# iden3/circom-witnesscalc

Measured on AMD Instinct MI355X. Metric: witnesses/sec, higher is better.
Workload: dtype u32

## Files before the change

### circom-witnesscalc_amd/csrc/fr_gfx950.hpp

```cpp
#pragma once
#include <stdint.h>

#if defined(__HIPCC__)
#define FRD __host__ __device__ __forceinline__
#else
#define FRD inline
#endif

namespace cwc {

struct Fr {
    uint32_t v[8];
};

#define CWC_P0 0xf0000001u
#define CWC_P1 0x43e1f593u
#define CWC_P2 0x79b97091u
#define CWC_P3 0x2833e848u
#define CWC_P4 0x8181585du
#define CWC_P5 0xb85045b6u
#define CWC_P6 0xe131a029u
#define CWC_P7 0x30644e72u
#define CWC_INV32 0xefffffffu

FRD Fr fr_p() { return Fr{{CWC_P0, CWC_P1, CWC_P2, CWC_P3, CWC_P4, CWC_P5, CWC_P6, CWC_P7}}; }
FRD Fr fr_one() { return Fr{{0x4ffffffbu, 0xac96341cu, 0x9f60cd29u, 0x36fc7695u, 0x7879462eu, 0x666ea36fu, 0x9a07df2fu, 0x0e0a77c1u}}; }
FRD Fr fr_r2() { return Fr{{0xae216da7u, 0x1bb8e645u, 0xe35c59e3u, 0x53fe3ab1u, 0x53bb8085u, 0x8c49833du, 0x7f4e44a5u, 0x0216d0b1u}}; }
FRD Fr fr_half() { return Fr{{0xf8000000u, 0xa1f0fac9u, 0x3cdcb848u, 0x9419f424u, 0x40c0ac2eu, 0xdc2822dbu, 0x7098d014u, 0x18322739u}}; }
FRD Fr fr_zero() { return Fr{{0, 0, 0, 0, 0, 0, 0, 0}}; }

FRD bool both(bool a, bool b) { return ((uint32_t)a & (uint32_t)b) != 0u; }
FRD bool either(bool a, bool b) { return ((uint32_t)a | (uint32_t)b) != 0u; }

FRD bool u256_is_zero(const Fr& a) {
    uint32_t o = 0;
#pragma unroll
    for (int i = 0; i < 8; ++i) o |= a.v[i];
    return o == 0;
}
FRD bool u256_eq(const Fr& a, const Fr& b) {
    uint32_t o = 0;
#pragma unroll
    for (int i = 0; i < 8; ++i) o |= a.v[i] ^ b.v[i];
    return o == 0;
}
FRD uint32_t adc32(uint32_t a, uint32_t b, uint32_t& carry) {
#if defined(__clang__)
    unsigned c = carry;
    const uint32_t r = __builtin_addc(a, b, c, &c);
    carry = c;
    return r;
#else
    const uint64_t t = (uint64_t)a + b + carry;
    carry = (uint32_t)(t >> 32);
    return (uint32_t)t;
#endif
}
FRD uint32_t sbb32(uint32_t a, uint32_t b, uint32_t& borrow) {
#if defined(__clang__)
    unsigned c = borrow;
    const uint32_t r = __builtin_subc(a, b, c, &c);
    borrow = c;
    return r;
#else
    const uint64_t t = (uint64_t)a - b - borrow;
    borrow = (uint32_t)(t >> 63);
    return (uint32_t)t;
#endif
}
FRD uint32_t u256_add(Fr& r, const Fr& a, const Fr& b) {
#if defined(__clang__)
    unsigned c = 0;
#pragma unroll
    for (int i = 0; i < 8; ++i) r.v[i] = __builtin_addc(a.v[i], b.v[i], c, &c);
    return c;
#else
    uint64_t c = 0;
#pragma unroll
    for (int i = 0; i < 8; ++i) {
        c += (uint64_t)a.v[i] + b.v[i];
        r.v[i] = (uint32_t)c;
        c >>= 32;
    }
    return (uint32_t)c;
#endif
}
FRD uint32_t u256_sub(Fr& r, const Fr& a, const Fr& b) {
#if defined(__clang__)
    unsigned br = 0;
#pragma unroll
    for (int i = 0; i < 8; ++i) r.v[i] = __builtin_subc(a.v[i], b.v[i], br, &br);
    return br;
#else
    int64_t c = 0;
#pragma unroll
    for (int i = 0; i < 8; ++i) {
        c += (int64_t)a.v[i] - (int64_t)b.v[i];
        r.v[i] = (uint32_t)c;
        c >>= 32;
    }
    return (uint32_t)(c & 1);
#endif
}
FRD bool u256_lt(const Fr& a, const Fr& b) {
    Fr t;
    return u256_sub(t, a, b) != 0;
}
FRD Fr u256_select(bool c, const Fr& a, const Fr& b) {
    Fr r;
#pragma unroll
    for (int i = 0; i < 8; ++i) r.v[i] = c ? a.v[i] : b.v[i];
    return r;
}

FRD Fr fr_add(const Fr& a, const Fr& b) {
    Fr s, t;
    u256_add(s, a, b);
    uint32_t br = u256_sub(t, s, fr_p());
    return u256_select(br != 0, s, t);
}
FRD Fr fr_sub(const Fr& a, const Fr& b) {
    Fr d, t;
    uint32_t br = u256_sub(d, a, b);
    u256_add(t, d, fr_p());
    return u256_select(br != 0, t, d);
}
#if defined(__HIPCC__)
__device__ __forceinline__ Fr fr_add_wave(const Fr& a, const Fr& b, const Fr& pv) {
#if defined(__HIP_DEVICE_COMPILE__)
#include "fr_add_gfx950.inc"
#else
    (void)pv;
    return fr_add(a, b);
#endif
}
__device__ __forceinline__ Fr fr_sub_wave(const Fr& a, const Fr& b, const Fr& pv) {
#if defined(__HIP_DEVICE_COMPILE__)
#include "fr_sub_gfx950.inc"
#else
    (void)pv;
    return fr_sub(a, b);
#endif
}
#endif
FRD Fr fr_neg(const Fr& a) {
    Fr t;
    u256_sub(t, fr_p(), a);
    return u256_select(u256_is_zero(a), a, t);
}

FRD Fr fr_mul(const Fr& a, const Fr& b) {
#if defined(__HIP_DEVICE_COMPILE__) && !defined(CWC_PORTABLE_FR_MUL)
#include "fr_mul_gfx950.inc"
#else
    const uint32_t p[8] = {CWC_P0, CWC_P1, CWC_P2, CWC_P3, CWC_P4, CWC_P5, CWC_P6, CWC_P7};
    uint32_t t[9];
#pragma unroll
    for (int i = 0; i < 9; ++i) t[i] = 0;
#pragma unroll
    for (int i = 0; i < 8; ++i) {
        uint64_t c = 0;
#pragma unroll
        for (int j = 0; j < 8; ++j) {
            c += (uint64_t)a.v[i] * b.v[j] + t[j];
            t[j] = (uint32_t)c;
            c >>= 32;
        }
        t[8] = (uint32_t)c;
        uint32_t m = t[0] * CWC_INV32;
        c = (uint64_t)m * p[0] + t[0];
        c >>= 32;
#pragma unroll
        for (int j = 1; j < 8; ++j) {
            c += (uint64_t)m * p[j] + t[j];
            t[j - 1] = (uint32_t)c;
            c >>= 32;
        }
        c += t[8];
        t[7] = (uint32_t)c;
    }
    Fr r, s;
#pragma unroll
    for (int i = 0; i < 8; ++i) r.v[i] = t[i];
    uint32_t br = u256_sub(s, r, fr_p());
    return u256_select(br != 0, r, s);
#endif
}
#if defined(__HIPCC__)
__device__ __forceinline__ Fr fr_addsub_wave(const Fr& a, const Fr& b, const Fr& pv, uint32_t m, unsigned long long subm,
                                             unsigned long long addm) {
#if defined(__HIP_DEVICE_COMPILE__)
#include "fr_addsub_gfx950.inc"
#else
    (void)pv; (void)subm; (void)addm;
    return m ? fr_sub(a, b) : fr_add(a, b);
#endif
}
__device__ __forceinline__ Fr fr_mul_wave(const Fr& a, const Fr& b, const Fr& pv) {
#if defined(__HIP_DEVICE_COMPILE__)
#include "fr_mul_block_gfx950.inc"
#else
    (void)pv;
    return fr_mul(a, b);
#endif
}
__device__ __forceinline__ void fr_mul_coop4(const Fr& a, uint32_t b0, uint32_t b1, uint32_t n0, uint32_t n1, uint32_t* out) {
#if defined(__HIP_DEVICE_COMPILE__)
#include "fr_mul_coop4_gfx950.inc"
#else
    (void)a; (void)b0; (void)b1; (void)n0; (void)n1;
    out[0] = out[1] = 0;
#endif
}
__device__ __forceinline__ void fr_mul_coop4r(const Fr& a, uint32_t aq0, uint32_t aq1, uint32_t b0, uint32_t b1, uint32_t n0, uint32_t n1, uint32_t sub,
                                              uint32_t* out) {
#if defined(__HIP_DEVICE_COMPILE__)
#include "fr_mul_coop4r_gfx950.inc"
#else
    (void)a; (void)aq0; (void)aq1; (void)b0; (void)b1; (void)n0; (void)n1; (void)sub;
    out[0] = out[1] = 0;
#endif
}
__device__ __forceinline__ void fr_addsub_coop4(uint32_t aq0, uint32_t aq1, uint32_t b0, uint32_t b1, uint32_t n0, uint32_t n1, uint32_t sub, uint32_t* out) {
#if defined(__HIP_DEVICE_COMPILE__)
#include "fr_addsub_coop4_gfx950.inc"
#else
    (void)aq0; (void)aq1; (void)b0; (void)b1; (void)n0; (void)n1; (void)sub;
    out[0] = out[1] = 0;
#endif
}
#endif
FRD Fr fr_sqr(const Fr& a) { return fr_mul(a, a); }

FRD Fr fr_to_mont(const Fr& x) { return fr_mul(x, fr_r2()); }
FRD Fr fr_from_mont(const Fr& x) {
#if defined(__HIP_DEVICE_COMPILE__) && !defined(CWC_PORTABLE_FR_MUL)
#include "fr_from_mont_gfx950.inc"
#else
    const uint32_t p[8] = {CWC_P0, CWC_P1, CWC_P2, CWC_P3, CWC_P4, CWC_P5, CWC_P6, CWC_P7};
    uint32_t t[8];
#pragma unroll
    for (int i = 0; i < 8; ++i) t[i] = x.v[i];
#pragma unroll
    for (int i = 0; i < 8; ++i) {
        uint32_t m = t[0] * CWC_INV32;
        uint64_t c = (uint64_t)m * p[0] + t[0];
        c >>= 32;
#pragma unroll
        for (int j = 1; j < 8; ++j) {
            c += (uint64_t)m * p[j] + t[j];
            t[j - 1] = (uint32_t)c;
            c >>= 32;
        }
        t[7] = (uint32_t)c;
    }
    Fr r, s;
#pragma unroll
    for (int i = 0; i < 8; ++i) r.v[i] = t[i];
    uint32_t br = u256_sub(s, r, fr_p());
    return u256_select(br != 0, r, s);
#endif
}

FRD Fr fr_inv_fermat(const Fr& a) {
    const uint32_t e[8] = {CWC_P7, CWC_P6, CWC_P5, CWC_P4, CWC_P3, CWC_P2, CWC_P1, CWC_P0 - 2u};
    Fr acc = fr_one();
    for (int w = 0; w < 8; ++w) {
        for (int bit = 31; bit >= 0; --bit) {
            acc = fr_sqr(acc);
            if ((e[w] >> bit) & 1u) acc = fr_mul(acc, a);
        }
    }
    return acc;
}

struct S30 {
    int32_t v[9];
};
struct Trans2x2 {
    int32_t u, v, q, r;
};

FRD int32_t sgcd_divsteps_30(int32_t zeta, uint32_t f0, uint32_t g0, Trans2x2& t) {
    uint32_t u = 1, v = 0, q = 0, r = 1;
    uint32_t f = f0, g = g0;
    for (int i = 0; i < 30; ++i) {
        uint32_t c1 = (uint32_t)(zeta >> 31);
        uint32_t c2 = 0u - (g & 1u);
        uint32_t x = (f ^ c1) - c1, y = (u ^ c1) - c1, z = (v ^ c1) - c1;
        g += x & c2;
        q += y & c2;
        r += z & c2;
        c1 &= c2;
        zeta = (int32_t)(((uint32_t)zeta ^ c1) - 1u);
        f += g & c1;
        u += q & c1;
        v += r & c1;
        g >>= 1;
        u <<= 1;
        v <<= 1;
    }
    t.u = (int32_t)u;
    t.v = (int32_t)v;
    t.q = (int32_t)q;
    t.r = (int32_t)r;
    return zeta;
}

FRD int64_t mad_i64(int32_t a, int32_t b, int64_t c) {
#if defined(__HIP_DEVICE_COMPILE__)
    int64_t d;
    unsigned long long cy;
    asm volatile("v_mad_i64_i32 %0, %1, %2, %3, %4" : "=v"(d), "=s"(cy) : "v"(a), "v"(b), "v"(c));
    return d;
#else
    return (int64_t)a * b + c;
#endif
}

FRD void sgcd_update_fg(S30& f, S30& g, const Trans2x2& t) {
    const int32_t M30 = 0x3fffffff;
    int64_t cf = mad_i64(t.u, f.v[0], mad_i64(t.v, g.v[0], 0));
    int64_t cg = mad_i64(t.q, f.v[0], mad_i64(t.r, g.v[0], 0));
    cf >>= 30;
    cg >>= 30;
#pragma unroll
    for (int i = 1; i < 9; ++i) {
        cf = mad_i64(t.u, f.v[i], mad_i64(t.v, g.v[i], cf));
        cg = mad_i64(t.q, f.v[i], mad_i64(t.r, g.v[i], cg));
        f.v[i - 1] = (int32_t)cf & M30;
        cf >>= 30;
        g.v[i - 1] = (int32_t)cg & M30;
        cg >>= 30;
    }
    f.v[8] = (int32_t)cf;
    g.v[8] = (int32_t)cg;
}

FRD void sgcd_update_de(S30& d, S30& e, const Trans2x2& t) {
    const int32_t M30 = 0x3fffffff;
    const int32_t p30[9] = {0x30000001, 0x0f87d64f, 0x1b970914, 0x0cfa121e, 0x01585d28, 0x0116da06, 0x1a029b85, 0x139cb84c, 0x3064};
    const uint32_t pinv30 = 0x10000001u;
    const int32_t sd = d.v[8] >> 31, se = e.v[8] >> 31;
    int32_t md = (t.u & sd) + (t.v & se);
    int32_t me = (t.q & sd) + (t.r & se);
    int64_t cd = mad_i64(t.u, d.v[0], mad_i64(t.v, e.v[0], 0));
    int64_t ce = mad_i64(t.q, d.v[0], mad_i64(t.r, e.v[0], 0));
    md -= (int32_t)((pinv30 * (uint32_t)cd + (uint32_t)md) & (uint32_t)M30);
    me -= (int32_t)((pinv30 * (uint32_t)ce + (uint32_t)me) & (uint32_t)M30);
    cd = mad_i64(p30[0], md, cd);
    ce = mad_i64(p30[0], me, ce);
    cd >>= 30;
    ce >>= 30;
#pragma unroll
    for (int i = 1; i < 9; ++i) {
        cd = mad_i64(t.u, d.v[i], mad_i64(t.v, e.v[i], cd));
        ce = mad_i64(t.q, d.v[i], mad_i64(t.r, e.v[i], ce));
        cd = mad_i64(p30[i], md, cd);
        ce = mad_i64(p30[i], me, ce);
        d.v[i - 1] = (int32_t)cd & M30;
        cd >>= 30;
        e.v[i - 1] = (int32_t)ce & M30;
        ce >>= 30;
    }
    d.v[8] = (int32_t)cd;
    e.v[8] = (int32_t)ce;
}

FRD int64_t sgcd_sar30(int64_t c) {
#if defined(__HIP_DEVICE_COMPILE__) && !defined(CWC_SGCD_SHIFT64)
    const uint32_t lo = (uint32_t)c, hi = (uint32_t)((uint64_t)c >> 32);
    const uint32_t nlo = __builtin_amdgcn_alignbit(hi, lo, 30);
    const int32_t nhi = (int32_t)hi >> 30;
    return (int64_t)(((uint64_t)(uint32_t)nhi << 32) | nlo);
#else
    return c >> 30;
#endif
}
FRD void sgcd_update_all(S30& d, S30& e, S30& f, S30& g, const Trans2x2& t) {
#if defined(__HIP_DEVICE_COMPILE__) && !defined(CWC_SGCD_CXX_UPDATE)
#if defined(CWC_SGCD_UPDATE_INC)
#include CWC_SGCD_UPDATE_INC
#else
#include "sgcd_update_gfx950.inc"
#endif
    return;
#endif
    const int32_t M30 = 0x3fffffff;
    const int32_t p30[9] = {0x30000001, 0x0f87d64f, 0x1b970914, 0x0cfa121e, 0x01585d28, 0x0116da06, 0x1a029b85, 0x139cb84c, 0x3064};
    const uint32_t pinv30 = 0x10000001u;
    const int32_t sd = d.v[8] >> 31, se = e.v[8] >> 31;
    int32_t md = (t.u & sd) + (t.v & se);
    int32_t me = (t.q & sd) + (t.r & se);
    int64_t cd = mad_i64(t.u, d.v[0], 0);
    int64_t ce = mad_i64(t.q, d.v[0], 0);
    int64_t cf = mad_i64(t.u, f.v[0], 0);
    int64_t cg = mad_i64(t.q, f.v[0], 0);
    cd = mad_i64(t.v, e.v[0], cd);
    ce = mad_i64(t.r, e.v[0], ce);
    cf = mad_i64(t.v, g.v[0], cf);
    cg = mad_i64(t.r, g.v[0], cg);
    md -= (int32_t)((pinv30 * (uint32_t)cd + (uint32_t)md) & (uint32_t)M30);
    me -= (int32_t)((pinv30 * (uint32_t)ce + (uint32_t)me) & (uint32_t)M30);
    cf = sgcd_sar30(cf);
    cg = sgcd_sar30(cg);
    cd = mad_i64(p30[0], md, cd);
    ce = mad_i64(p30[0], me, ce);
    cd = sgcd_sar30(cd);
    ce = sgcd_sar30(ce);
#pragma unroll
    for (int i = 1; i < 9; ++i) {
        const int32_t di = d.v[i], ei = e.v[i], fi = f.v[i], gi = g.v[i];
        cd = mad_i64(t.u, di, cd);
        ce = mad_i64(t.q, di, ce);
        cf = mad_i64(t.u, fi, cf);
        cg = mad_i64(t.q, fi, cg);
        cd = mad_i64(t.v, ei, cd);
        ce = mad_i64(t.r, ei, ce);
        cf = mad_i64(t.v, gi, cf);
        cg = mad_i64(t.r, gi, cg);
        cd = mad_i64(p30[i], md, cd);
        ce = mad_i64(p30[i], me, ce);
        f.v[i - 1] = (int32_t)cf & M30;
        g.v[i - 1] = (int32_t)cg & M30;
        cf = sgcd_sar30(cf);
        cg = sgcd_sar30(cg);
        d.v[i - 1] = (int32_t)cd & M30;
        e.v[i - 1] = (int32_t)ce & M30;
        cd = sgcd_sar30(cd);
        ce = sgcd_sar30(ce);
    }
    d.v[8] = (int32_t)cd;
    e.v[8] = (int32_t)ce;
    f.v[8] = (int32_t)cf;
    g.v[8] = (int32_t)cg;
}

FRD uint32_t sgcd_mul24(uint32_t a, uint32_t b) {
#if defined(__HIP_DEVICE_COMPILE__)
    uint32_t d;
    asm("v_mul_u32_u24 %0, %1, %2" : "=v"(d) : "v"(a), "v"(b));
    return d;
#else
    return (a & 0xffffffu) * (b & 0xffffffu);
#endif
}
FRD bool sgcd_any_lane(bool p) {
#if defined(__HIP_DEVICE_COMPILE__)
    return __ballot(p) != 0ull;
#else
    return p;
#endif
}
FRD int32_t sgcd_divsteps_30_var(int32_t eta, uint32_t f0, uint32_t g0, Trans2x2& t) {
    uint32_t u = 1, v = 0, q = 0, r = 1;
    uint32_t f = f0, g = g0;
    int32_t i = 30;
    do {
#pragma unroll
        for (int rep = 0; rep < 2; ++rep) {
            const int32_t zeros = (int32_t)__builtin_ctz(g | (0xffffffffu << i));
            g >>= zeros;
            u <<= zeros;
            v <<= zeros;
            eta -= zeros;
            i -= zeros;
            const bool sw = eta < 0 && i != 0;
            const uint32_t nf = 0u - f, nu = 0u - u, nv = 0u - v;
            eta = sw ? -eta : eta;
            const uint32_t f2 = sw ? g : f, g2 = sw ? nf : g;
            const uint32_t u2 = sw ? q : u, q2 = sw ? nu : q;
            const uint32_t v2 = sw ? r : v, r2 = sw ? nv : r;
            f = f2; g = g2; u = u2; q = q2; v = v2; r = r2;
            int32_t limit = eta + 1 < i ? eta + 1 : i;
            limit = limit < 6 ? limit : 6;
            limit = limit < 0 ? 0 : limit;
            const uint32_t w = sgcd_mul24(sgcd_mul24(g, f), sgcd_mul24(f, f) - 2u) & ((1u << limit) - 1u);
            g += f * w;
            q += u * w;
            r += v * w;
        }
    } while (sgcd_any_lane(i != 0));
    t.u = (int32_t)u;
    t.v = (int32_t)v;
    t.q = (int32_t)q;
    t.r = (int32_t)r;
    return eta;
}

FRD Fr u256_inv_mod_r(const Fr& x) {
    const int32_t M30 = 0x3fffffff;
    const int32_t p30[9] = {0x30000001, 0x0f87d64f, 0x1b970914, 0x0cfa121e, 0x01585d28, 0x0116da06, 0x1a029b85, 0x139cb84c, 0x3064};
    S30 d, e, f, g;
#pragma unroll
    for (int i = 0; i < 9; ++i) {
        d.v[i] = 0;
        e.v[i] = 0;
        f.v[i] = p30[i];
        const int lo = (30 * i) >> 5, sh = (30 * i) & 31;
        uint64_t w = x.v[lo];
        if (lo + 1 < 8) w |= (uint64_t)x.v[lo + 1] << 32;
        g.v[i] = (int32_t)((uint32_t)(w >> sh) & (uint32_t)M30);
    }
    e.v[0] = 1;
#if defined(CWC_CONSTANT_TIME_INVERSE)
    int32_t zeta = -1;
    for (int it = 0; it < 20; ++it) {
        Trans2x2 t;
        zeta = sgcd_divsteps_30(zeta, (uint32_t)f.v[0], (uint32_t)g.v[0], t);
        sgcd_update_de(d, e, t);
        sgcd_update_fg(f, g, t);
    }
#else
    int32_t eta = -1;
    for (int it = 0; it < 25; ++it) {
        Trans2x2 t;
        eta = sgcd_divsteps_30_var(eta, (uint32_t)f.v[0], (uint32_t)g.v[0], t);
        sgcd_update_all(d, e, f, g, t);
        int32_t gz = 0;
#pragma unroll
        for (int i = 0; i < 9; ++i) gz |= g.v[i];
#if defined(__HIP_DEVICE_COMPILE__)
        if (__ballot(gz != 0) == 0ull) break;
#else
        if (gz == 0) break;
#endif
    }
#endif
    const int32_t sign = f.v[8] >> 31;
    int32_t cond_add = d.v[8] >> 31;
#pragma unroll
    for (int i = 0; i < 9; ++i) d.v[i] += p30[i] & cond_add;
#pragma unroll
    for (int i = 0; i < 9; ++i) d.v[i] = (d.v[i] ^ sign) - sign;
#pragma unroll
    for (int i = 0; i < 8; ++i) {
        d.v[i + 1] += d.v[i] >> 30;
        d.v[i] &= M30;
    }
    cond_add = d.v[8] >> 31;
#pragma unroll
    for (int i = 0; i < 9; ++i) d.v[i] += p30[i] & cond_add;
#pragma unroll
    for (int i = 0; i < 8; ++i) {
        d.v[i + 1] += d.v[i] >> 30;
        d.v[i] &= M30;
    }
    Fr out;
#pragma unroll
    for (int k = 0; k < 8; ++k) {
        const int li = (32 * k) / 30, off = (32 * k) % 30;
        uint64_t w = (uint64_t)(uint32_t)d.v[li] >> off;
        w |= (uint64_t)(uint32_t)d.v[li + 1] << (30 - off);
        if (li + 2 < 9) w |= (uint64_t)(uint32_t)d.v[li + 2] << (60 - off);
        out.v[k] = (uint32_t)w;
    }
    return out;
}

FRD Fr fr_inv(const Fr& a) {
    const Fr r3 = Fr{{0xb4bf0040u, 0x5e94d8e1u, 0x1cfbb6b8u, 0x2a489cbeu, 0xa19fcfedu, 0x893cc664u, 0x7fcc657cu, 0x0cf8594bu}};
    return fr_mul(u256_inv_mod_r(a), r3);
}

FRD Fr u256_shr(const Fr& x, uint32_t n) {
    Fr a = x;
    const uint32_t w = n >> 5, s = n & 31;
    const bool w4 = (w & 4u) != 0u, w2 = (w & 2u) != 0u, w1 = (w & 1u) != 0u;
#pragma unroll
    for (int i = 0; i < 8; ++i) a.v[i] = w4 ? ((i + 4 < 8) ? a.v[i + 4 < 8 ? i + 4 : 0] : 0u) : a.v[i];
#pragma unroll
    for (int i = 0; i < 8; ++i) a.v[i] = w2 ? ((i + 2 < 8) ? a.v[i + 2 < 8 ? i + 2 : 0] : 0u) : a.v[i];
#pragma unroll
    for (int i = 0; i < 8; ++i) a.v[i] = w1 ? ((i + 1 < 8) ? a.v[i + 1 < 8 ? i + 1 : 0] : 0u) : a.v[i];
    Fr r;
#pragma unroll
    for (int i = 0; i < 8; ++i) {
        uint64_t pair = ((uint64_t)(i + 1 < 8 ? a.v[i + 1] : 0) << 32) | a.v[i];
        r.v[i] = (uint32_t)(pair >> s);
    }
    return r;
}
FRD Fr u256_shl(const Fr& x, uint32_t n) {
    Fr a = x;
    const uint32_t w = n >> 5, s = n & 31;
    const bool w4 = (w & 4u) != 0u, w2 = (w & 2u) != 0u, w1 = (w & 1u) != 0u;
#pragma unroll
    for (int i = 7; i >= 0; --i) a.v[i] = w4 ? ((i - 4 >= 0) ? a.v[i - 4 >= 0 ? i - 4 : 0] : 0u) : a.v[i];
#pragma unroll
    for (int i = 7; i >= 0; --i) a.v[i] = w2 ? ((i - 2 >= 0) ? a.v[i - 2 >= 0 ? i - 2 : 0] : 0u) : a.v[i];
#pragma unroll
    for (int i = 7; i >= 0; --i) a.v[i] = w1 ? ((i - 1 >= 0) ? a.v[i - 1 >= 0 ? i - 1 : 0] : 0u) : a.v[i];
    Fr r;
#pragma unroll
    for (int i = 7; i >= 0; --i) {
        uint64_t pair = ((uint64_t)a.v[i] << 32) | (i - 1 >= 0 ? a.v[i - 1] : 0);
        r.v[i] = (uint32_t)((pair << s) >> 32);
    }
    return r;
}

#if defined(__HIPCC__)
#endif

FRD uint32_t u256_bitlen(const Fr& a) {
    uint32_t n = 0;
#pragma unroll
    for (int i = 0; i < 8; ++i)
        if (a.v[i]) n = 32u * i + (32u - (uint32_t)__builtin_clz(a.v[i]));
    return n;
}

FRD void u256_divrem(Fr& q, Fr& rem, const Fr& a, const Fr& b, uint32_t top) {
    Fr num = top ? u256_shl(a, 256u - top) : fr_zero();
    rem = top >= 256u ? fr_zero() : u256_shr(a, top);
    q = fr_zero();
    for (uint32_t i = 0; i < top; ++i) {
        uint32_t carry = num.v[7] >> 31;
#pragma unroll
        for (int k = 7; k > 0; --k) num.v[k] = (num.v[k] << 1) | (num.v[k - 1] >> 31);
        num.v[0] <<= 1;
        uint32_t ov = rem.v[7] >> 31;
#pragma unroll
        for (int k = 7; k > 0; --k) rem.v[k] = (rem.v[k] << 1) | (rem.v[k - 1] >> 31);
        rem.v[0] = (rem.v[0] << 1) | carry;
        Fr t;
        uint32_t br = u256_sub(t, rem, b);
        bool ge = (br == 0) || ov;
        rem = u256_select(ge, t, rem);
#pragma unroll
        for (int k = 7; k > 0; --k) q.v[k] = (q.v[k] << 1) | (q.v[k - 1] >> 31);
        q.v[0] = (q.v[0] << 1) | (ge ? 1u : 0u);
    }
}

FRD void u256_divrem_digits(Fr& q, Fr& rem, const Fr& a, const Fr& b, uint32_t digits, uint32_t bitlen_b = 0) {
    const uint32_t L = bitlen_b ? bitlen_b : u256_bitlen(b);
    const uint32_t sh = 256u - L;
    const Fr bn = u256_shl(b, sh);
    Fr lo = u256_shl(a, sh);
    uint32_t R[9];
    {
        const Fr hi = u256_select(sh != 0u, u256_shr(a, L & 255u), fr_zero());
#pragma unroll
        for (int i = 0; i < 8; ++i) R[i] = hi.v[i];
        R[8] = 0;
    }
    q = fr_zero();
#pragma unroll
    for (int j = 7; j >= 0; --j) {
#pragma unroll
        for (int i = 8; i > 0; --i) R[i] = R[i - 1];
        R[0] = lo.v[j];
        if ((uint32_t)j >= digits) continue;
        const uint32_t d = bn.v[7];
        uint32_t qhat;
        {
            const uint64_t n64 = ((uint64_t)R[8] << 32) | R[7];
            const double n = (double)R[8] * 4294967296.0 + (double)R[7];
            double e = n / (double)d;
            e = e < 4294967295.0 ? e : 4294967295.0;
            uint32_t est = (uint32_t)e;
#if defined(CWC_TEST_PERTURB_QHAT)
            if ((CWC_TEST_PERTURB_QHAT) > 0 ? est != 0xffffffffu : est != 0u) est += (uint32_t)(CWC_TEST_PERTURB_QHAT);
#endif
            const int64_t r = (int64_t)(n64 - (uint64_t)est * d);
            est = r < 0 ? est - 1u : ((uint64_t)r >= d ? est + 1u : est);
            qhat = R[8] >= d ? 0xffffffffu : est;
        }
        uint32_t P[9];
        {
            uint64_t c = 0;
#pragma unroll
            for (int i = 0; i < 8; ++i) {
                c += (uint64_t)qhat * bn.v[i];
                P[i] = (uint32_t)c;
                c >>= 32;
            }
            P[8] = (uint32_t)c;
        }
        uint32_t borrow = 0;
#pragma unroll
        for (int i = 0; i < 9; ++i) R[i] = sbb32(R[i], P[i], borrow);
#pragma unroll
        for (int fix = 0; fix < 2; ++fix) {
            const bool neg = borrow != 0;
            uint32_t carry = 0;
#pragma unroll
            for (int i = 0; i < 9; ++i) R[i] = adc32(R[i], neg ? (i < 8 ? bn.v[i] : 0u) : 0u, carry);
            borrow = neg && !carry ? 1u : 0u;
            qhat -= neg ? 1u : 0u;
        }
        q.v[j] = qhat;
    }
    Fr r8;
#pragma unroll
    for (int i = 0; i < 8; ++i) r8.v[i] = R[i];
    rem = u256_shr(r8, sh);
}

FRD void u128_divrem_64(Fr& q, Fr& rem, const Fr& a, const Fr& b) {
    const uint64_t bv = ((uint64_t)b.v[1] << 32) | b.v[0];
    const uint32_t s = (uint32_t)(b.v[1] ? __builtin_clz(b.v[1]) : 32 + __builtin_clz(b.v[0] | 1u));
    const uint64_t bn = bv << s;
    const uint32_t bn1 = (uint32_t)(bn >> 32), bn0 = (uint32_t)bn;
    uint32_t A[6];
    {
        const uint64_t a_lo = ((uint64_t)a.v[1] << 32) | a.v[0], a_hi = ((uint64_t)a.v[3] << 32) | a.v[2];
        const uint64_t w0 = a_lo << s;
        const uint64_t w1 = (a_hi << s) | (s ? a_lo >> (64 - s) : 0);
        const uint64_t w2 = s ? a_hi >> (64 - s) : 0;
        A[0] = (uint32_t)w0; A[1] = (uint32_t)(w0 >> 32); A[2] = (uint32_t)w1; A[3] = (uint32_t)(w1 >> 32);
        A[4] = (uint32_t)w2; A[5] = (uint32_t)(w2 >> 32);
    }
    uint32_t R2 = 0, R1 = A[5], R0 = A[4];
    q = fr_zero();
#pragma unroll
    for (int j = 3; j >= 0; --j) {
        R2 = R1; R1 = R0; R0 = A[j];
        uint32_t qhat;
        {
            const uint64_t n64 = ((uint64_t)R2 << 32) | R1;
            const double n = (double)R2 * 4294967296.0 + (double)R1;
            double e = n / (double)bn1;
            e = e < 4294967295.0 ? e : 4294967295.0;
            uint32_t est = (uint32_t)e;
#if defined(CWC_TEST_PERTURB_QHAT)
            if ((CWC_TEST_PERTURB_QHAT) > 0 ? est != 0xffffffffu : est != 0u) est += (uint32_t)(CWC_TEST_PERTURB_QHAT);
#endif
            const int64_t r = (int64_t)(n64 - (uint64_t)est * bn1);
            est = r < 0 ? est - 1u : ((uint64_t)r >= bn1 ? est + 1u : est);
            qhat = R2 >= bn1 ? 0xffffffffu : est;
        }
        const uint64_t p0 = (uint64_t)qhat * bn0;
        const uint64_t p1 = (uint64_t)qhat * bn1 + (p0 >> 32);
        uint32_t borrow = 0;
        R0 = sbb32(R0, (uint32_t)p0, borrow);
        R1 = sbb32(R1, (uint32_t)p1, borrow);
        R2 = sbb32(R2, (uint32_t)(p1 >> 32), borrow);
#pragma unroll
        for (int fix = 0; fix < 2; ++fix) {
            const bool neg = borrow != 0;
            uint32_t carry = 0;
            R0 = adc32(R0, neg ? bn0 : 0u, carry);
            R1 = adc32(R1, neg ? bn1 : 0u, carry);
            R2 = adc32(R2, 0u, carry);
            borrow = neg && !carry ? 1u : 0u;
            qhat -= neg ? 1u : 0u;
        }
        q.v[j] = qhat;
    }
    const uint64_t r64 = (((uint64_t)R1 << 32) | R0) >> s;
    rem = fr_zero();
    rem.v[0] = (uint32_t)r64;
    rem.v[1] = (uint32_t)(r64 >> 32);
}

FRD uint64_t mulhi64(uint64_t a, uint64_t b) {
#if defined(__HIP_DEVICE_COMPILE__)
    return __umul64hi(a, b);
#else
    return (uint64_t)(((unsigned __int128)a * b) >> 64);
#endif
}
FRD uint32_t clz64_nonzero(uint64_t x) {
    const uint32_t hi = (uint32_t)(x >> 32), lo = (uint32_t)x;
    const uint32_t c_hi = (uint32_t)__builtin_clz(hi | 1u), c_lo = 32u + (uint32_t)__builtin_clz(lo | 1u);
    return hi ? c_hi : c_lo;
}
FRD uint64_t recip64(uint64_t dn) {
    const uint64_t d0 = dn & 1ull, d40 = (dn >> 24) + 1ull, d63 = (dn >> 1) + d0;
    const uint32_t d9 = (uint32_t)(dn >> 55);
    uint32_t v0 = (uint32_t)(523520.0f / (float)d9);
    v0 -= v0 * d9 > 523520u ? 1u : 0u;
    v0 += (v0 + 1u) * d9 <= 523520u ? 1u : 0u;
    const uint64_t v1 = ((uint64_t)v0 << 11) - (((uint64_t)(v0 * v0) * d40) >> 40) - 1ull;
    const uint64_t v2 = (v1 << 13) + ((v1 * ((1ull << 60) - v1 * d40)) >> 47);
    const uint64_t e = (0ull - v2 * d63) + ((v2 >> 1) & (0ull - d0));
    const uint64_t v3 = (v2 << 31) + (mulhi64(v2, e) >> 1);
    const uint64_t lo = v3 * dn, hi = mulhi64(v3, dn);
    const uint64_t lo2 = lo + dn;
    return v3 - (hi + dn + (lo2 < lo ? 1ull : 0ull));
}
FRD void div2by1(uint64_t u1, uint64_t u0, uint64_t dn, uint64_t v, uint64_t& q, uint64_t& r) {
    const uint64_t lo = v * u1, hi = mulhi64(v, u1);
    const uint64_t q0 = lo + u0;
    uint64_t q1 = hi + u1 + (q0 < lo ? 1ull : 0ull) + 1ull;
    uint64_t rr = u0 - q1 * dn;
    if (rr > q0) {
        --q1;
        rr += dn;
    }
    if (rr >= dn) {
        ++q1;
        rr -= dn;
    }
    q = q1;
    r = rr;
}
FRD void u128_divrem_64_recip(uint64_t th, uint64_t tl, uint64_t d, uint32_t s, uint64_t dn, uint64_t v, bool high, uint64_t& qh, uint64_t& ql, uint64_t& rem) {
    uint64_t rh = th;
    qh = 0;
    if (high) {
        uint64_t rn;
        div2by1((th >> 1) >> (63u - s), th << s, dn, v, qh, rn);
        rh = rn >> s;
    }
    (void)d;
    uint64_t rn;
    div2by1((rh << s) | ((tl >> 1) >> (63u - s)), tl << s, dn, v, ql, rn);
    rem = rn >> s;
}

FRD uint64_t recip64_3by2(uint64_t d1, uint64_t d0) {
    uint64_t v = recip64(d1);
    uint64_t p = d1 * v + d0;
    const bool c1 = p < d0, c2 = both(c1, p >= d1);
    v -= (c1 ? 1ull : 0ull) + (c2 ? 1ull : 0ull);
    p -= (c2 ? d1 : 0ull);
    p -= (c1 ? d1 : 0ull);
    const uint64_t t1 = mulhi64(v, d0), t0 = v * d0;
    p += t1;
    const bool c3 = p < t1, c4 = both(c3, either(p > d1, both(p == d1, t0 >= d0)));
    v -= (c3 ? 1ull : 0ull) + (c4 ? 1ull : 0ull);
    return v;
}
FRD void div3by2(uint64_t u2, uint64_t u1, uint64_t u0, uint64_t d1, uint64_t d0, uint64_t v, uint64_t& q, uint64_t& r1, uint64_t& r0) {
    uint64_t q0 = v * u2, q1 = mulhi64(v, u2);
    q0 += u1;
    q1 += u2 + (q0 < u1 ? 1ull : 0ull);
    uint64_t a1 = u1 - q1 * d1;
    const uint64_t t1 = mulhi64(d0, q1), t0 = d0 * q1;
    uint64_t a0 = u0 - t0;
    a1 -= t1 + (u0 < t0 ? 1ull : 0ull);
    const uint64_t b0 = a0 - d0;
    a1 -= d1 + (a0 < d0 ? 1ull : 0ull);
    a0 = b0;
    ++q1;
    {
        const bool f = a1 >= q0;
        q1 -= f ? 1ull : 0ull;
        const uint64_t c0 = a0 + d0, c1 = a1 + d1 + (c0 < a0 ? 1ull : 0ull);
        a1 = f ? c1 : a1;
        a0 = f ? c0 : a0;
    }
    {
        const bool f = either(a1 > d1, both(a1 == d1, a0 >= d0));
        q1 += f ? 1ull : 0ull;
        const uint64_t c0 = a0 - d0, c1 = a1 - (d1 + (a0 < d0 ? 1ull : 0ull));
        a1 = f ? c1 : a1;
        a0 = f ? c0 : a0;
    }
    q = q1;
    r1 = a1;
    r0 = a0;
}
FRD void u256_divrem_128(Fr& q, Fr& rem, const Fr& a, const Fr& b) {
    const uint64_t bh = ((uint64_t)b.v[3] << 32) | b.v[2], bl = ((uint64_t)b.v[1] << 32) | b.v[0];
    const uint32_t s = clz64_nonzero(bh);
    const uint64_t d1 = (bh << s) | ((bl >> 1) >> (63u - s)), d0 = bl << s;
    const uint64_t v = recip64_3by2(d1, d0);
    uint64_t aw[4];
#pragma unroll
    for (int k = 0; k < 4; ++k) aw[k] = ((uint64_t)a.v[2 * k + 1] << 32) | a.v[2 * k];
    uint64_t u[5];
    u[0] = aw[0] << s;
#pragma unroll
    for (int k = 1; k < 4; ++k) u[k] = (aw[k] << s) | ((aw[k - 1] >> 1) >> (63u - s));
    u[4] = (aw[3] >> 1) >> (63u - s);
    uint64_t qw[3];
#pragma unroll
    for (int j = 2; j >= 0; --j) {
        uint64_t r1, r0;
        div3by2(u[j + 2], u[j + 1], u[j], d1, d0, v, qw[j], r1, r0);
        u[j + 1] = r1;
        u[j] = r0;
    }
    q = fr_zero();
    rem = fr_zero();
#pragma unroll
    for (int j = 0; j < 3; ++j) {
        q.v[2 * j] = (uint32_t)qw[j];
        q.v[2 * j + 1] = (uint32_t)(qw[j] >> 32);
    }
    const uint64_t rl = (u[0] >> s) | ((u[1] << 1) << (63u - s)), rh = u[1] >> s;
    rem.v[0] = (uint32_t)rl;
    rem.v[1] = (uint32_t)(rl >> 32);
    rem.v[2] = (uint32_t)rh;
    rem.v[3] = (uint32_t)(rh >> 32);
}

}
```

### circom-witnesscalc_amd/csrc/kernels.hip

```cpp
#include <hip/hip_runtime.h>
#include <stdlib.h>

#include "fr_gfx950.hpp"
#include "scan_gfx950.hpp"
#include "program_dev.h"

namespace cwc {

__device__ __forceinline__ Fr fr_from_u4(const uint4& lo, const uint4& hi) {
    return Fr{{lo.x, lo.y, lo.z, lo.w, hi.x, hi.y, hi.z, hi.w}};
}

__device__ __forceinline__ bool wave_any(bool p) { return __ballot(p) != 0ull; }

struct InterpDims {
    uint32_t n_bundles, n_slots, n_inputs, batch, n_const, n_div_requests, trash_off;
    const uint32_t* div_lanes;
    uint32_t n_streams, stream_first[MAX_STREAMS], stream_count[MAX_STREAMS], stream_div_requests[MAX_STREAMS], stream_cref_first[MAX_STREAMS];
    uint4* pack_out;
    const uint2* pack_entries;
    const uint32_t* pack_ready;
    uint32_t n_inline, pack_mont, n_witness;
};
static const uint32_t ST_DIVIDER_TIMEOUT = 0x80000000u;
static const uint32_t ST_SYNC_TIMEOUT = 0x40000000u;

__device__ __forceinline__ bool mbox_wait(const volatile uint32_t* seq, uint32_t need) {
    for (uint32_t spins = 0; spins < (1u << 22); ++spins) {
        if (*seq >= need) return true;
        __builtin_amdgcn_s_sleep(8);
    }
    return false;
}
__device__ __noinline__ bool post_wait(uint32_t* word, uint32_t need) {
#pragma nounroll
    for (uint32_t spins = 0; spins < (1u << 22); ++spins) {
        if (__hip_atomic_load(word, __ATOMIC_ACQUIRE, __HIP_MEMORY_SCOPE_AGENT) >= need) return true;
        __builtin_amdgcn_s_sleep(8);
    }
    return false;
}
typedef uint32_t u32x4 __attribute__((ext_vector_type(4)));
typedef int i32x4 __attribute__((ext_vector_type(4)));
typedef __attribute__((address_space(3))) char lds_char;

__device__ __forceinline__ void dma16(uint32_t lds_addr, uint32_t voff, const i32x4& rsrc, uint32_t soff) {
    asm volatile("s_mov_b32 m0, %0\n\ts_nop 0\n\tbuffer_load_dwordx4 %1, %2, %3 offen lds"
                 :: "s"(lds_addr), "v"(voff), "s"(rsrc), "s"(soff) : "memory");
}
__device__ __forceinline__ i32x4 make_rsrc_words(const void* base, uint32_t bytes) {
    const uint64_t a = (uint64_t)base;
    return i32x4{(int)(uint32_t)a, (int)((uint32_t)(a >> 32) & 0xffffu), (int)bytes, 0x00020000};
}

template <int T, bool PROF, int W, int PACK, int MODE = 0>
__global__ __launch_bounds__((W > 0 ? (W + 1) * PACK : PACK) * 64) void interp_kernel(const uint32_t* __restrict__ hdr, const uint4* __restrict__ recs,
                                                    const uint32_t* __restrict__ crefs, InterpDims p, WsTable wst,
                                                    const uint4* __restrict__ inputs, uint32_t* __restrict__ status,
                                                    unsigned long long* __restrict__ prof) {
    constexpr int G = 64 / T;
    constexpr bool M2 = MODE == 2 || MODE == 3, WIDE = MODE == 3;
    constexpr uint32_t HI = 16u * T;
    constexpr bool DIVIDER = W > 0;
    constexpr uint32_t NW = (W > 0 ? (uint32_t)W : 1u) * (uint32_t)PACK;
    constexpr uint32_t WD = W > 0 ? (uint32_t)W : 1u;
    constexpr uint32_t AREA = lds_area_bytes((uint32_t)W, LDS_BYTES);
    constexpr uint32_t ML = mbox_lanes((uint32_t)W), MB = mbox_bytes((uint32_t)W);
    const uint32_t batch = p.batch;
    const uint32_t lane = threadIdx.x & 63u;
    const uint32_t wave = (uint32_t)__builtin_amdgcn_readfirstlane((int)(threadIdx.x >> 6));
    const uint32_t n_tiles = (batch + T - 1) / T;
    const uint32_t t = lane % T;
    const uint32_t j = (G == 1) ? 0u : lane / T;
    const uint32_t NS = p.n_streams;
    const uint32_t stream = wave < NW ? wave % NS : 0u;
    const uint32_t tile_raw = blockIdx.x * (NW / NS) + (wave < NW ? wave : 0u) / NS;
    const uint32_t tile = tile_raw < n_tiles ? tile_raw : n_tiles - 1;
    const uint32_t set = tile * T + t;
    const uint32_t set_c = set < batch ? set : batch - 1;
    [[maybe_unused]] auto census_slot = [&]() -> unsigned long long* {
        const uint32_t wv = blockIdx.x * (blockDim.x >> 6) + wave;
        return lane == 0 && wv < CENSUS_MAX_WAVES ? prof + PROF_WORDS + CENSUS_WORDS * wv : nullptr;
    };
    if constexpr (PROF) {
        if (unsigned long long* c = census_slot()) {
            const uint32_t w_of = wave < NW ? wave : (wave - NW) * WD;
            const uint32_t has_tile = blockIdx.x * (NW / NS) + w_of / NS < n_tiles ? 1u : 0u;
            const unsigned long long role = (wave >= NW ? 1u : 0u) | (w_of % NS) << 1 | has_tile << 4 | (blockDim.x >> 6) << 8;
            constexpr int HWREG_HW_ID = 4 | 31 << 11, HWREG_XCC_ID = 20 | 31 << 11;
            c[0] = (unsigned long long)__builtin_amdgcn_s_getreg(HWREG_HW_ID) | (unsigned long long)(__builtin_amdgcn_s_getreg(HWREG_XCC_ID) & 15u) << 32 | role << 40;
            c[1] = __builtin_amdgcn_s_memtime();
        }
    }
    const uint64_t tile_bytes = ws_tile_bytes(p.n_const, p.n_slots, T);
    const uint32_t chunk = tile / wst.tiles_per_chunk, tile_in_chunk = tile % wst.tiles_per_chunk;
    char* tile_base = reinterpret_cast<char*>(wst.base[chunk]) + (uint64_t)tile_in_chunk * tile_bytes;
    const __amdgpu_buffer_rsrc_t rsrc = __builtin_amdgcn_make_buffer_rsrc(tile_base, 0, (int)(uint32_t)tile_bytes, 0x00020000);
    const i32x4 rsrc_rec = make_rsrc_words(recs, (p.n_bundles + REC_AHEAD) * (uint32_t)G * 16u);
    uint32_t* const sync_words = reinterpret_cast<uint32_t*>(tile_base + ws_sync_offset(p.n_const, p.n_slots, T));
    static_assert(NW + PACK <= 16, "sequence words: 64 bytes");
    __shared__ uint4 lds[(NW * AREA + (DIVIDER ? NW * MB + 64u : 0u)) / 16];
    const uint32_t area = wave * AREA;
    const uint32_t lds0 = (uint32_t)(uintptr_t)(lds_char*)(char*)lds + area;
    const uint32_t t16 = 16u * t, lane16 = 16u * lane, j16 = 16u * j;
    char* const ldsb = reinterpret_cast<char*>(lds) + area;
    char* const mbox_all = reinterpret_cast<char*>(lds) + NW * AREA;
    char* const mbox = mbox_all + (wave < NW ? wave : 0u) * MB;
    volatile uint32_t* const seq = reinterpret_cast<volatile uint32_t*>(mbox_all + NW * MB);
    if (DIVIDER || NW > 1) {
        if (DIVIDER && threadIdx.x < NW + (uint32_t)PACK) seq[threadIdx.x] = 0;
        if (NS > 1 && wave < NW && stream == 0 && lane < MAX_STREAMS && tile_raw < n_tiles) {
            __hip_atomic_store(sync_words + lane, 0u, __ATOMIC_RELAXED, __HIP_MEMORY_SCOPE_AGENT);
            __builtin_amdgcn_fence(__ATOMIC_RELEASE, "agent");
        }
        if (wave < NW && stream == 0 && j == 0 && tile_raw < n_tiles && set < batch) status[set] = 0;
        __syncthreads();
    } else {
        if (j == 0 && tile_raw < n_tiles && set < batch) status[set] = 0;
    }
    if (DIVIDER) {
        if (wave >= NW) {
            const uint32_t first_w = (wave - NW) * WD, first_tile = blockIdx.x * (NW / NS) + first_w / NS;
            if (first_tile >= n_tiles) return;
            const uint32_t n_active = NS > 1 ? 1u : n_tiles - first_tile < WD ? n_tiles - first_tile : WD;
            char* const mbox_d = mbox_all + first_w * MB;
            const uint32_t n_requests = NS > 1 ? p.stream_div_requests[first_w % NS] : p.n_div_requests;
            uint32_t div_lanes_base = 0;
            for (uint32_t q = 0; NS > 1 && q < first_w % NS; ++q) div_lanes_base += p.stream_div_requests[q];
            [[maybe_unused]] uint32_t pk_next = 0;
            [[maybe_unused]] uint2 pk_e0 = make_uint2(0u, 0u), pk_e1 = pk_e0;
            [[maybe_unused]] unsigned long long pk_cycles = 0, pk_passes = 0;
            const bool inl = W == 1 && NS == 1 && p.n_inline > 0;
            const char* const pk_tile = reinterpret_cast<const char*>(wst.base[first_tile / wst.tiles_per_chunk]) + (uint64_t)(first_tile % wst.tiles_per_chunk) * tile_bytes;
            const uint32_t pk_set = first_tile * T + t;
            auto pk_load = [&](const uint2& e, uint4& lo, uint4& hi) {
                const uint32_t ref = e.y & ~REF_CANON;
                const uint32_t slot = (ref & REF_CONST) ? (ref & ~REF_CONST) : p.n_const + ref;
                const uint4* q = reinterpret_cast<const uint4*>(pk_tile) + (size_t)slot * (2 * T);
                lo = q[t];
                hi = q[T + t];
            };
            auto pk_store = [&](const uint2& e, const uint4& lo, const uint4& hi, uint32_t limit) {
                const bool valid = pk_next + j < limit && pk_set < batch, canon = (e.y & REF_CANON) != 0;
                const Fr v = fr_from_u4(lo, hi);
                Fr c = v;
                if (p.pack_mont) {
                    if (wave_any(both(valid, canon))) c = u256_select(canon, fr_mul(v, fr_r2()), v);
                } else {
                    if (wave_any(both(valid, !canon))) c = u256_select(canon, v, fr_from_mont(v));
                }
                if (valid) {
                    uint4* o = p.pack_out + ((size_t)pk_set * p.n_witness + e.x) * 2;
                    o[0] = make_uint4(c.v[0], c.v[1], c.v[2], c.v[3]);
                    o[1] = make_uint4(c.v[4], c.v[5], c.v[6], c.v[7]);
                }
            };
            auto pk_run = [&](uint32_t limit, uint32_t need) {
                if (pk_next >= limit) return;
                unsigned long long t0 = 0;
                if (PROF) t0 = __builtin_amdgcn_s_memtime();
                uint4 lo, hi;
                pk_load(pk_e0, lo, hi);
                for (;;) {
                    const uint32_t nb = pk_next + (uint32_t)G;
                    const bool more = nb < limit && seq[first_w] < need;
                    uint4 lo1 = lo, hi1 = hi;
                    if (more) pk_load(pk_e1, lo1, hi1);
                    const uint2 e2 = p.pack_entries[nb + (uint32_t)G + j];
                    pk_store(pk_e0, lo, hi, limit);
                    pk_next = nb;
                    pk_e0 = pk_e1;
                    pk_e1 = e2;
                    if (PROF) ++pk_passes;
                    if (!more) break;
                    lo = lo1;
                    hi = hi1;
                }
                if (PROF) pk_cycles += __builtin_amdgcn_s_memtime() - t0;
            };
            if constexpr (W == 1) {
                if (inl) {
                    pk_e0 = p.pack_entries[j];
                    pk_e1 = p.pack_entries[(uint32_t)G + j];
                }
            }
            for (uint32_t k = 0; k < n_requests; ++k) {
                if constexpr (W == 1) {
                    if (inl) {
                        const uint32_t lim = p.pack_ready[k] < p.n_inline ? p.pack_ready[k] : p.n_inline;
                        pk_run(lim / (uint32_t)G * (uint32_t)G, k + 1);
                    }
                }
                bool ok = true;
                for (uint32_t w = 0; w < n_active; ++w) ok = ok && mbox_wait(seq + first_w + w, k + 1);
                if (!ok) {
                    if (first_tile * T + t < batch) atomicOr(&status[first_tile * T + t], ST_DIVIDER_TIMEOUT);
                    break;
                }
                __builtin_amdgcn_fence(__ATOMIC_ACQUIRE, "workgroup");
                const uint32_t lanes_k = p.div_lanes[div_lanes_base + k];
                const uint32_t total = n_active * lanes_k;
                for (uint32_t g0 = 0; g0 < total; g0 += 64u) {
                    const uint32_t g = g0 + lane;
                    const bool valid = g < total;
                    const uint32_t w = valid ? g / lanes_k : 0u, i = valid ? g % lanes_k : 0u;
                    char* mb = mbox_d + w * MB + 16u * i;
                    const uint4* qa = reinterpret_cast<const uint4*>(mb);
                    const uint4* qb = reinterpret_cast<const uint4*>(mb + 32u * ML);
                    Fr a = fr_from_u4(qa[0], qa[ML]), b = fr_from_u4(qb[0], qb[ML]);
                    if (!valid) b = fr_zero();
                    const Fr inv = fr_inv(b);
                    const Fr r = u256_select(u256_is_zero(b), fr_zero(), fr_mul(a, inv));
                    if (valid) {
                        uint4* qr = reinterpret_cast<uint4*>(mb);
                        qr[0] = make_uint4(r.v[0], r.v[1], r.v[2], r.v[3]);
                        qr[ML] = make_uint4(r.v[4], r.v[5], r.v[6], r.v[7]);
                    }
                }
                __builtin_amdgcn_fence(__ATOMIC_RELEASE, "workgroup");
                if (lane == 0) seq[wave] = k + 1;
            }
            if constexpr (W == 1) {
                if (inl) {
                    pk_run(p.pack_ready[n_requests] < p.n_inline ? p.pack_ready[n_requests] : p.n_inline, 0xffffffffu);
                    if (PROF && lane == 0 && first_tile % 64u == 0) {
                        atomicAdd(&prof[94], pk_cycles);
                        atomicAdd(&prof[95], pk_passes);
                    }
                }
            }
            if constexpr (PROF) {
                if (unsigned long long* c = census_slot()) c[2] = __builtin_amdgcn_s_memtime();
            }
            return;
        }
    }
    if (tile_raw >= n_tiles) return;
    uint32_t div_seq = 0;
    uint32_t n_posts = 0, n_waits = 0;
    uint32_t cref_row = p.stream_cref_first[stream];

    auto ld = [&](uint32_t off) -> Fr {
        const u32x4 lo = __builtin_amdgcn_raw_buffer_load_b128(rsrc, (int)off, 0, 0);
        const u32x4 hi = __builtin_amdgcn_raw_buffer_load_b128(rsrc, (int)off + (int)HI, 0, 0);
        return Fr{{lo.x, lo.y, lo.z, lo.w, hi.x, hi.y, hi.z, hi.w}};
    };
    auto ld_lds = [&](uint32_t addr) -> Fr {
        const uint4* q = reinterpret_cast<const uint4*>(ldsb + addr);
        const uint4 lo = q[0], hi = q[LDS_HALF_BYTES / 16];
        return fr_from_u4(lo, hi);
    };
    auto ld_rec2 = [&](uint32_t bundle, uint32_t half) -> uint2 {
        return *reinterpret_cast<const uint2*>(ldsb + LDS_REC_OFF + (bundle % REC_AHEAD) * REC_BYTES + lane16 + 8u * half);
    };
    const uint32_t B0 = p.stream_first[stream], NBND = B0 + p.stream_count[stream];
    if (NBND == B0) return;
    auto clampb = [&](uint32_t b) { return b < NBND ? b : NBND - 1; };
    auto stage_rec = [&](uint32_t bundle) {
        dma16(lds0 + LDS_REC_OFF + (bundle % REC_AHEAD) * REC_BYTES, j16, rsrc_rec, bundle * (uint32_t)G * 16u);
    };
    constexpr uint32_t DMA_BIAS = 3u * LDS_HALF_BYTES;
    const i32x4 rsrc_dma = make_rsrc_words(tile_base - DMA_BIAS, (uint32_t)tile_bytes + DMA_BIAS);
    const uint32_t dma_soff0 = DMA_BIAS, dma_soff1 = DMA_BIAS + HI - LDS_HALF_BYTES, dma_soff2 = DMA_BIAS - 2u * LDS_HALF_BYTES,
                   dma_soff3 = DMA_BIAS + HI - 3u * LDS_HALF_BYTES;
    static_assert(LDS_HALF_BYTES == 1024, "instruction offsets below are written out");
    auto stage_operands = [&](uint32_t bundle, const uint2& offs) {
        const uint32_t s = lds0 + LDS_STAGE_OFF + (bundle % OPND_AHEAD) * STAGE_BYTES;
        const uint32_t ao = offs.x + t16, bo = offs.y + t16;
        asm volatile("s_mov_b32 m0, %0\n\ts_nop 0\n\t"
                     "buffer_load_dwordx4 %1, %3, %4 offen lds\n\t"
                     "buffer_load_dwordx4 %1, %3, %5 offen offset:1024 lds\n\t"
                     "buffer_load_dwordx4 %2, %3, %6 offen offset:2048 lds\n\t"
                     "buffer_load_dwordx4 %2, %3, %7 offen offset:3072 lds"
                     :: "s"(s), "v"(ao), "v"(bo), "s"(rsrc_dma), "s"(dma_soff0), "s"(dma_soff1), "s"(dma_soff2), "s"(dma_soff3) : "memory");
    };
    uint32_t err_bits = 0;
    Fr pv = fr_p();
#pragma unroll
    for (int i = 0; i < 8; ++i) asm volatile("" : "+v"(pv.v[i]));
    constexpr bool COOP = (uint32_t)T <= COOP_MAX_T;
    const uint32_t cq = lane & 3u, cv = lane >> 2;
    const uint32_t t16c = 16u * (cv % T);
    const uint32_t coop_chunk = (cq >> 1) * LDS_HALF_BYTES + (cq & 1u) * 8u;
    const uint32_t coop_ring_off = 16u * cv + coop_chunk;
    const uint32_t coop_dst_off = t16c + (cq >> 1) * HI + (cq & 1u) * 8u;
    uint32_t nq0 = cq == 0 ? CWC_P0 : cq == 1 ? CWC_P2 : cq == 2 ? CWC_P4 : CWC_P6;
    uint32_t nq1 = cq == 0 ? CWC_P1 : cq == 1 ? CWC_P3 : cq == 2 ? CWC_P5 : CWC_P7;
    asm volatile("" : "+v"(nq0), "+v"(nq1));
    const uint32_t trash_doff = p.trash_off | t16;
    constexpr int C_PROF = 12;
    unsigned long long pf[C_PROF][2], psec[2][7] = {{0, 0, 0, 0, 0, 0, 0}, {0, 0, 0, 0, 0, 0, 0}};
    unsigned long long pf_fused[2] = {0, 0};
    unsigned long long pf_scan[5][2] = {{0, 0}, {0, 0}, {0, 0}, {0, 0}, {0, 0}};
    if (PROF) {
#pragma unroll
        for (int c = 0; c < C_PROF; ++c) pf[c][0] = pf[c][1] = 0;
    }
#define CWC_STAMP(var) unsigned long long var = 0; if (PROF) asm volatile("s_memtime %0\n\ts_waitcnt lgkmcnt(0)" : "=s"(var)::"memory")
#define CWC_SHADOW_ISSUE()                                                                                                                  \
    stage_rec(b + 4);                                                                                                                       \
    __builtin_amdgcn_raw_buffer_store_b128(u32x4{r_prev.v[0], r_prev.v[1], r_prev.v[2], r_prev.v[3]}, rsrc, (int)doff_prev, 0, 0);          \
    __builtin_amdgcn_raw_buffer_store_b128(u32x4{r_prev.v[4], r_prev.v[5], r_prev.v[6], r_prev.v[7]}, rsrc, (int)doff_prev + (int)HI, 0, 0)
#define CWC_NEXT_HEADER(var)                                                                                                                 \
    asm volatile("s_mov_b32 %0, xnack_mask_lo\n\ts_load_dword xnack_mask_lo, %1, %2" : "=&s"(var) : "s"(hdr), "s"(hdr_off_n2) : "memory"); \
    hdr_off_n2 += 4u

    static_assert(OPND_AHEAD == 2 && REC_AHEAD == 4, "the counted waits below are written for this pipeline depth");
#pragma unroll
    for (uint32_t q = 0; q < REC_AHEAD; ++q) stage_rec(B0 + q);
    asm volatile("s_waitcnt vmcnt(0)" ::: "memory");
    stage_operands(B0, ld_rec2(B0, 0));
    stage_operands(B0 + 1, ld_rec2(B0 + 1, 0));
    uint2 rec_hi = ld_rec2(B0, 1);
    uint2 rec_hi_n1 = ld_rec2(B0 + 1, 1);
    uint32_t h_cur = hdr[B0], h_n1 = hdr[clampb(B0 + 1)];
    asm volatile("s_waitcnt vmcnt(0)" ::: "memory");
    const unsigned long long t_wave0 = PROF ? __builtin_amdgcn_s_memtime() : 0ull;
    asm volatile("s_load_dword xnack_mask_lo, %0, %1\n\ts_waitcnt lgkmcnt(0)" :: "s"(hdr), "s"(4u * B0 + 8u) : "memory");
    uint32_t hdr_off_n2 = 4u * B0 + 12u;
    Fr r_prev = fr_zero();
    uint32_t doff_prev = trash_doff;
    for (uint32_t b = B0; b < NBND; ++b) {
        CWC_STAMP(st0);
        const uint32_t h = h_cur;
        asm volatile("s_waitcnt vmcnt(7)" ::: "memory");
        CWC_STAMP(st1);
        if constexpr (COOP) {
            uint32_t cls_q = h & HDR_CLASS_MASK;
            asm volatile("" : "+s"(cls_q));
            static_assert(C_MULQ == 11 && C_SYNC == 12 && C_MULF == 13 && C_SCAN == 14 && C_COUNT == 15, "one compare (class >= C_MULQ) leads to the narrow classes");
            const bool narrow_cls = MODE == 1 ? cls_q >= C_MULQ : cls_q == C_MULQ;
            if (M2 ? __builtin_expect(narrow_cls, 0) : narrow_cls) {
            if (MODE != 1 || cls_q == C_MULQ) {
                const uint32_t la = rec_hi.y + (t16c | (t16c << 16));
                const Fr a_op = ld_lds(la & 0xffffu);
                const uint2 bq = *reinterpret_cast<const uint2*>(ldsb + (la >> 16) + coop_chunk);
                const uint2 aq = *reinterpret_cast<const uint2*>(ldsb + (la & 0xffffu) + coop_chunk);
                const uint4 rec_full_n2 = *reinterpret_cast<const uint4*>(ldsb + LDS_REC_OFF + ((b + 2) % REC_AHEAD) * REC_BYTES + lane16);
                const uint2 rec_n2 = make_uint2(rec_full_n2.x, rec_full_n2.y), rec_hi_n2 = make_uint2(rec_full_n2.z, rec_full_n2.w);
                CWC_SHADOW_ISSUE();
                asm volatile("s_waitcnt lgkmcnt(0)" :: "v"(a_op.v[0]), "v"(a_op.v[4]), "v"(bq.x), "v"(aq.x), "v"(rec_n2.x), "v"(rec_hi_n2.x) : "memory");
                uint32_t h_n2;
                CWC_NEXT_HEADER(h_n2);
                CWC_STAMP(st2);
                stage_operands(b + 2, rec_n2);
                CWC_STAMP(st3);
                uint32_t out[2];
                if (h & (HDR_LIN_ADD | HDR_LIN_SUB)) {
                    fr_mul_coop4r(a_op, aq.x, aq.y, bq.x, bq.y, nq0, nq1, rec_hi.x & CTRL_SUB_MASK, out);
                } else {
                    fr_mul_coop4(a_op, bq.x, bq.y, nq0, nq1, out);
                }
                CWC_STAMP(st4);
                *reinterpret_cast<uint2*>(ldsb + LDS_RING_OFF + (b % RING_BUNDLES) * RING_SLOT_BYTES + coop_ring_off) = make_uint2(out[0], out[1]);
                {
                    typedef uint32_t u32x2 __attribute__((ext_vector_type(2)));
                    __builtin_amdgcn_raw_buffer_store_b64(u32x2{out[0], out[1]}, rsrc, (int)((rec_hi.x & ~CTRL_MASK) + coop_dst_off), 0, 0);
                }
                doff_prev = trash_doff;
                rec_hi = rec_hi_n1;
                rec_hi_n1 = rec_hi_n2;
                h_cur = h_n1;
                h_n1 = h_n2;
                __builtin_amdgcn_fence(__ATOMIC_ACQ_REL, "wavefront");
                if (PROF) {
                    asm volatile("s_waitcnt lgkmcnt(0)" ::: "memory");
                    const unsigned long long t_now = __builtin_amdgcn_s_memtime();
                    pf[C_MULQ][0] += t_now - st0;
                    pf[C_MULQ][1] += 1;
                    (void)st2; (void)st3; (void)st4;
                }
                continue;
            }
            if constexpr (MODE == 1 && (uint32_t)T <= COOP_FUSE_MAX_T) {
            if (cls_q == C_MULF) {
                constexpr int QP_MAIN = T == 1 ? 0xA0  : 0x00 , QP_EXTRA = T == 1 ? 0xF5  : 0xAA ;
                const uint32_t mx = (uint32_t)__builtin_amdgcn_mov_dpp((int)rec_hi.x, QP_MAIN, 0xf, 0xf, false);
                const uint32_t my = (uint32_t)__builtin_amdgcn_mov_dpp((int)rec_hi.y, QP_MAIN, 0xf, 0xf, false);
                const uint32_t xx = (uint32_t)__builtin_amdgcn_mov_dpp((int)rec_hi.x, QP_EXTRA, 0xf, 0xf, false);
                const uint32_t xy = (uint32_t)__builtin_amdgcn_mov_dpp((int)rec_hi.y, QP_EXTRA, 0xf, 0xf, false);
                const uint32_t la = my + (t16c | (t16c << 16)), lx = xy + (t16c | (t16c << 16));
                const Fr a_op = ld_lds(la & 0xffffu);
                const uint2 bq = *reinterpret_cast<const uint2*>(ldsb + (la >> 16) + coop_chunk);
                const Fr x2_full = ld_lds(lx & 0xffffu);
                const uint2 x2q = *reinterpret_cast<const uint2*>(ldsb + (lx & 0xffffu) + coop_chunk);
                const uint2 x3q = *reinterpret_cast<const uint2*>(ldsb + (lx >> 16) + coop_chunk);
                const uint4 rec_full_n2 = *reinterpret_cast<const uint4*>(ldsb + LDS_REC_OFF + ((b + 2) % REC_AHEAD) * REC_BYTES + lane16);
                const uint2 rec_n2 = make_uint2(rec_full_n2.x, rec_full_n2.y), rec_hi_n2 = make_uint2(rec_full_n2.z, rec_full_n2.w);
                CWC_SHADOW_ISSUE();
                asm volatile("s_waitcnt lgkmcnt(0)" :: "v"(a_op.v[0]), "v"(a_op.v[4]), "v"(bq.x), "v"(x2_full.v[0]), "v"(x2_full.v[4]), "v"(x2q.x), "v"(x3q.x), "v"(rec_n2.x), "v"(rec_hi_n2.x) : "memory");
                uint32_t h_n2;
                CWC_NEXT_HEADER(h_n2);
                stage_operands(b + 2, rec_n2);
                uint32_t out[2];
                fr_mul_coop4(a_op, bq.x, bq.y, nq0, nq1, out);
                const uint32_t op2 = mx & CTRL_SUB_MASK, op3 = xx & CTRL_SUB_MASK;
                if (h & HDR_F_S2MUL) {
                    uint32_t o2[2];
                    fr_mul_coop4(x2_full, out[0], out[1], nq0, nq1, o2);
                    out[0] = op2 == FOP_MUL ? o2[0] : out[0];
                    out[1] = op2 == FOP_MUL ? o2[1] : out[1];
                }
                auto lin_stage = [&](uint32_t op, const uint2& xq) {
                    const bool rs = op == FOP_RSUB;
                    uint32_t o[2];
                    fr_addsub_coop4(rs ? xq.x : out[0], rs ? xq.y : out[1], rs ? out[0] : xq.x, rs ? out[1] : xq.y, nq0, nq1, op == FOP_ADD ? 0u : 1u, o);
                    out[0] = op >= FOP_ADD ? o[0] : out[0];
                    out[1] = op >= FOP_ADD ? o[1] : out[1];
                };
                if (h & HDR_F_S2LIN) lin_stage(op2, x2q);
                if (h & HDR_F_S3LIN) lin_stage(op3, x3q);
                *reinterpret_cast<uint2*>(ldsb + LDS_RING_OFF + (b % RING_BUNDLES) * RING_SLOT_BYTES + coop_ring_off) = make_uint2(out[0], out[1]);
                {
                    typedef uint32_t u32x2 __attribute__((ext_vector_type(2)));
                    __builtin_amdgcn_raw_buffer_store_b64(u32x2{out[0], out[1]}, rsrc, (int)((mx & ~CTRL_MASK) + coop_dst_off), 0, 0);
                }
                doff_prev = trash_doff;
                rec_hi = rec_hi_n1;
                rec_hi_n1 = rec_hi_n2;
                h_cur = h_n1;
                h_n1 = h_n2;
                __builtin_amdgcn_fence(__ATOMIC_ACQ_REL, "wavefront");
                if (PROF) {
                    asm volatile("s_waitcnt lgkmcnt(0)" ::: "memory");
                    const unsigned long long t_now = __builtin_amdgcn_s_memtime();
                    pf_fused[0] += t_now - st0;
                    pf_fused[1] += 1;
                }
                continue;
            }
            }
            }
        }
        const uint32_t ctrl = rec_hi.x & CTRL_MASK;
        const uint32_t doff = (rec_hi.x & ~CTRL_MASK) | t16;
        const uint32_t la = rec_hi.y + (t16 | (t16 << 16));
        const Fr a_op = ld_lds(la & 0xffffu), b_op = ld_lds(la >> 16);
        const uint4 rec_full_n2 = *reinterpret_cast<const uint4*>(ldsb + LDS_REC_OFF + ((b + 2) % REC_AHEAD) * REC_BYTES + lane16);
        const uint2 rec_n2 = make_uint2(rec_full_n2.x, rec_full_n2.y), rec_hi_n2 = make_uint2(rec_full_n2.z, rec_full_n2.w);
        CWC_SHADOW_ISSUE();
        unsigned long long st_iss = 0;
        if (PROF) st_iss = __builtin_amdgcn_s_memtime();
        uint32_t h_n2;
        unsigned long long st2 = 0, st3 = 0;
        auto wait_and_stage = [&]() {
            asm volatile("s_waitcnt lgkmcnt(0)" :: "v"(a_op.v[0]), "v"(a_op.v[4]), "v"(b_op.v[0]), "v"(b_op.v[4]), "v"(rec_n2.x), "v"(rec_hi_n2.x) : "memory");
            CWC_NEXT_HEADER(h_n2);
            if (PROF) asm volatile("s_memtime %0\n\ts_waitcnt lgkmcnt(0)" : "=s"(st2)::"memory");
            stage_operands(b + 2, rec_n2);
            if (PROF) asm volatile("s_memtime %0\n\ts_waitcnt lgkmcnt(0)" : "=s"(st3)::"memory");
        };

        const uint32_t cls = h & HDR_CLASS_MASK;
        uint32_t cls_hot = cls, cls_hot2 = cls;
        asm volatile("" : "+s"(cls_hot));
        asm volatile("" : "+s"(cls_hot2));
        const bool active = (ctrl & CTRL_ACTIVE) != 0;
        const uint32_t sub = ctrl & CTRL_SUB_MASK;
        auto finish = [&](const Fr& r) {
            CWC_STAMP(st4);
            r_prev = r;
            doff_prev = doff;
            {
                uint4* q = reinterpret_cast<uint4*>(ldsb + LDS_RING_OFF + (b % RING_BUNDLES) * RING_SLOT_BYTES + lane16);
                q[0] = make_uint4(r.v[0], r.v[1], r.v[2], r.v[3]);
                q[LDS_HALF_BYTES / 16] = make_uint4(r.v[4], r.v[5], r.v[6], r.v[7]);
            }
            rec_hi = rec_hi_n1;
            rec_hi_n1 = rec_hi_n2;
            h_cur = h_n1;
            h_n1 = h_n2;
            __builtin_amdgcn_fence(__ATOMIC_ACQ_REL, "wavefront");
            if (PROF) {
                asm volatile("s_waitcnt lgkmcnt(0)" ::: "memory");
                const unsigned long long t_now = __builtin_amdgcn_s_memtime();
    #pragma unroll
                for (int c = 0; c < C_PROF; ++c)
                    if (cls == (uint32_t)c) {
                        pf[c][0] += t_now - st0;
                        pf[c][1] += 1;
                    }
                if (M2 && cls == C_SCAN) {
                    pf_fused[0] += t_now - st0;
                    pf_fused[1] += 1;
                    const int kind = (h & HDR_SCAN_CONV) ? 2 : (h & HDR_SCAN_BORROW) ? 3 : (h & HDR_SCAN_LEX) ? 4 : (h & HDR_SCAN_DIV) ? 1 : 0;
#pragma unroll
                    for (int q = 0; q < 5; ++q)
                        if (kind == q) {
                            pf_scan[q][0] += t_now - st0;
                            pf_scan[q][1] += 1;
                        }
                }
                if (cls == C_MUL || cls == C_LIN) {
                    unsigned long long* q = psec[cls == C_MUL ? 0 : 1];
                    q[0] += st1 - st0;
                    q[1] += st2 - st1;
                    q[2] += st3 - st2;
                    q[3] += st4 - st3;
                    q[4] += t_now - st4;
                    q[5] += 1;
                    q[6] += st_iss - st1;
                }
            }
        };
        Fr r;
        auto one_out = [&]() -> Fr { return (h & HDR_OUT_CANON) ? Fr{{1u, 0u, 0u, 0u, 0u, 0u, 0u, 0u}} : fr_one(); };
        if (cls_hot2 == C_LIN) {
            wait_and_stage();
            if (!(h & HDR_LIN_SUB)) {
                r = fr_add_wave(a_op, b_op, pv);
            } else if (!(h & HDR_LIN_ADD)) {
                r = fr_sub_wave(a_op, b_op, pv);
            } else {
                const unsigned long long subm = __ballot(sub == SUB_SUB);
                r = fr_addsub_wave(a_op, b_op, pv, sub == SUB_SUB ? ~0u : 0u, subm, ~subm);
            }
            finish(r);
            continue;
        }
        wait_and_stage();
        if (__builtin_expect(cls_hot == C_MUL, WIDE ? 0 : 1)) {
            if constexpr (M2) {
                if (h & HDR_MUL_CC) {
                    auto limb_product = [&](const Fr& x, const Fr& y) -> Fr {
                        const uint64_t p00 = (uint64_t)x.v[0] * y.v[0], p01 = (uint64_t)x.v[0] * y.v[1], p10 = (uint64_t)x.v[1] * y.v[0], p11 = (uint64_t)x.v[1] * y.v[1];
                        const uint64_t m1 = (p00 >> 32) + (uint32_t)p01 + (uint32_t)p10;
                        const uint64_t m2 = (m1 >> 32) + (p01 >> 32) + (p10 >> 32) + (uint32_t)p11;
                        Fr z = fr_zero();
                        z.v[0] = (uint32_t)p00;
                        z.v[1] = (uint32_t)m1;
                        z.v[2] = (uint32_t)m2;
                        z.v[3] = (uint32_t)((m2 >> 32) + (p11 >> 32));
                        return z;
                    };
                    const uint32_t hi_a = a_op.v[2] | a_op.v[3] | a_op.v[4] | a_op.v[5] | a_op.v[6] | a_op.v[7], hi_b = b_op.v[2] | b_op.v[3] | b_op.v[4] | b_op.v[5] | b_op.v[6] | b_op.v[7];
                    if (!wave_any((hi_a | hi_b) != 0u)) {
                        r = limb_product(a_op, b_op);
                    } else if (WIDE && !wave_any(((a_op.v[3] | b_op.v[3]) >> 30 | a_op.v[4] | a_op.v[5] | a_op.v[6] | a_op.v[7] | b_op.v[4] | b_op.v[5] | b_op.v[6] | b_op.v[7]) != 0u)) {
                        uint32_t z[8] = {0, 0, 0, 0, 0, 0, 0, 0};
#pragma unroll
                        for (int i = 0; i < 4; ++i) {
                            uint32_t carry = 0;
#pragma unroll
                            for (int jj = 0; jj < 4; ++jj) {
                                const uint64_t t = (uint64_t)a_op.v[i] * b_op.v[jj] + z[i + jj] + carry;
                                z[i + jj] = (uint32_t)t;
                                carry = (uint32_t)(t >> 32);
                            }
                            z[i + 4] = carry;
                        }
#pragma unroll
                        for (int k = 0; k < 8; ++k) r.v[k] = z[k];
                    } else {
                        Fr na, nb;
                        (void)u256_sub(na, fr_p(), a_op);
                        (void)u256_sub(nb, fr_p(), b_op);
                        const bool a_neg = hi_a != 0u, b_neg = hi_b != 0u;
                        const Fr ma = u256_select(a_neg, na, a_op), mb = u256_select(b_neg, nb, b_op);
                        if (!wave_any((ma.v[2] | ma.v[3] | ma.v[4] | ma.v[5] | ma.v[6] | ma.v[7] | mb.v[2] | mb.v[3] | mb.v[4] | mb.v[5] | mb.v[6] | mb.v[7]) != 0u)) {
                            const Fr z = limb_product(ma, mb);
                            Fr nz;
                            (void)u256_sub(nz, fr_p(), z);
                            r = u256_select(both(a_neg != b_neg, !u256_is_zero(z)), nz, z);
                        } else {
                            r = fr_mul_wave(fr_mul_wave(a_op, fr_r2(), pv), b_op, pv);
                        }
                    }
                    finish(r);
                    continue;
                }
            }
            r = fr_mul_wave(a_op, b_op, pv);
            if ((h & (HDR_LIN_ADD | HDR_LIN_SUB)) == (HDR_LIN_ADD | HDR_LIN_SUB)) {
                const unsigned long long subm = __ballot(sub == SUB_SUB);
                r = u256_select(sub <= SUB_SUB, fr_addsub_wave(a_op, b_op, pv, sub == SUB_SUB ? ~0u : 0u, subm, ~subm), r);
            } else if (h & HDR_LIN_ADD) {
                r = u256_select(sub == SUB_ADD, fr_add_wave(a_op, b_op, pv), r);
            } else if (h & HDR_LIN_SUB) {
                r = u256_select(sub == SUB_SUB, fr_sub_wave(a_op, b_op, pv), r);
            }
            finish(r);
            continue;
        }
        if constexpr (M2 && (uint32_t)T <= SCAN_MAX_T) {
            uint32_t cls_scan = cls;
            asm volatile("" : "+s"(cls_scan));
            if (WIDE ? __builtin_expect(cls_scan == C_SCAN, 1) : (cls_scan == C_SCAN)) {
                r = fr_zero();
                if constexpr (M2 && (uint32_t)T <= SCAN_MAX_T) {
                    if (h & HDR_SCAN_CONV) {
                        const uint32_t k = (h >> HDR_SCAN_ITER_SHIFT) + 1u;
                        const bool holds_y = active && lane < k * (uint32_t)T;
                        if (!wave_any(both(active, (a_op.v[2] | a_op.v[3] | a_op.v[4] | a_op.v[5] | a_op.v[6] | a_op.v[7] | b_op.v[2] | b_op.v[3] | b_op.v[4] | b_op.v[5] | b_op.v[6] | b_op.v[7]) != 0u))) {
                            uint32_t col[5];
                            conv_limb_columns<T>(k, lane, ((uint64_t)a_op.v[1] << 32) | a_op.v[0], holds_y ? (((uint64_t)b_op.v[1] << 32) | b_op.v[0]) : 0ull, col);
#pragma unroll
                            for (int w = 0; w < 5; ++w) r.v[w] = col[w];
                        } else {
                            Fr yy = u256_select(holds_y, b_op, fr_zero());
                            for (uint32_t i = 0; i < k; ++i) {
                                Fr xi;
#pragma unroll
                                for (int w = 0; w < 8; ++w) {
                                    if constexpr (T == 1) {
                                        xi.v[w] = (uint32_t)__builtin_amdgcn_readlane((int)a_op.v[w], (int)i);
                                    } else {
                                        const uint32_t e = (uint32_t)__builtin_amdgcn_readlane((int)a_op.v[w], (int)(2 * i)), o = (uint32_t)__builtin_amdgcn_readlane((int)a_op.v[w], (int)(2 * i + 1));
                                        xi.v[w] = (lane & 1u) ? o : e;
                                    }
                                }
                                r = fr_add_wave(r, fr_mul_wave(fr_mul_wave(xi, fr_r2(), pv), yy, pv), pv);
#pragma unroll
                                for (int w = 0; w < 8; ++w) yy.v[w] = wave_shr_lanes<T>(yy.v[w]);
                            }
                        }
                        finish(r);
                        continue;
                    }
                    constexpr int QP_OUT = T == 1 ? 0xA0  : 0x44 , QP_ACC = T == 1 ? 0xF5  : 0xEE ;
                    constexpr int D = 2 * T;
                    const uint32_t sh = (h >> HDR_SCAN_SHIFT_SHIFT) & 0xffu, iters = (h >> HDR_SCAN_ITER_SHIFT) + 1u;
                    const bool start = (sub & SCAN_START) != 0, role_acc = (sub & SCAN_ROLE_ACC) != 0;
                    const Fr x = fr_quad_perm<QP_OUT>(a_op), acc0 = fr_quad_perm<QP_OUT>(b_op);
                    if (WIDE && (h & (HDR_SCAN_BORROW | HDR_SCAN_LEX))) {
                        const Fr y = fr_quad_perm<QP_ACC>(a_op);
                        const bool seg = start || !active;
                        const uint32_t a0 = both(both(start, active), !u256_is_zero(acc0)) ? 1u : 0u;
                        auto less = [](const Fr& a, const Fr& b) {
                            Fr t;
                            const uint32_t borrow = u256_sub(t, a, b);
                            asm volatile("" ::"v"(t.v[7]));
                            return borrow != 0;
                        };
                        auto signed_lt = [&](const Fr& a, const Fr& b) {
                            const bool an = less(fr_half(), a), bn = less(fr_half(), b), ab = less(a, b);
                            return an == bn ? ab : an;
                        };
                        auto compare = [&](const Fr& a, const Fr& b, bool& lt, bool& gt) {
                            if (!wave_any(both(active, (a.v[4] | a.v[5] | a.v[6] | a.v[7] | b.v[4] | b.v[5] | b.v[6] | b.v[7]) != 0u))) {
                                uint32_t d[4], bw = 0;
#pragma unroll
                                for (int k = 0; k < 4; ++k) d[k] = sbb32(a.v[k], b.v[k], bw);
                                lt = bw != 0u;
                                gt = bw == 0u && (d[0] | d[1] | d[2] | d[3]) != 0u;
                            } else {
                                lt = signed_lt(a, b);
                                gt = signed_lt(b, a);
                            }
                        };
                        if ((h & (HDR_SCAN_BORROW | HDR_SCAN_LEX)) == (HDR_SCAN_BORROW | HDR_SCAN_LEX)) {
                            const Fr q_arm = fr_quad_perm<QP_ACC>(b_op);
                            const uint32_t code = sh & 7u;
                            bool cond;
                            if (code == SEL_NEZ) {
                                cond = !u256_is_zero(x);
                            } else {
                                bool lt, gt;
                                compare(x, acc0, lt, gt);
                                cond = code == SEL_LT ? lt : code == SEL_GT ? gt : code == SEL_LEQ ? !gt : !lt;
                            }
                            const Fr one_out = (sh & SEL_OUT_MONT) ? fr_one() : Fr{{1u, 0u, 0u, 0u, 0u, 0u, 0u, 0u}};
                            r = u256_select(cond, u256_select(role_acc, y, one_out), u256_select(role_acc, q_arm, fr_zero()));
                        } else if (h & HDR_SCAN_LEX) {
                            const uint32_t kg = (h & HDR_SCAN_KG) ? 1u : 0u, kl = (h & HDR_SCAN_KL) ? 1u : 0u;
                            bool lt, gt;
                            compare(x, y, lt, gt);
                            lt = both(lt, active);
                            gt = both(gt, active);
                            const bool gen = either(both(gt, kg != 0u), both(lt, kl != 0u)), prop = both(active, !either(gt, lt));
                            const uint32_t cin = scan_bit_lookahead<T>(seg, either(gen, both(both(seg, prop), a0 != 0u)), prop, lane);
                            const uint32_t bin = seg ? a0 : cin;
                            const bool res = role_acc ? either(gen, both(prop, bin != 0u)) : bin != 0u;
                            r = u256_select(res, sh ? fr_one() : Fr{{1u, 0u, 0u, 0u, 0u, 0u, 0u, 0u}}, fr_zero());
                        } else {
                            const uint32_t m[4] = {mask_word(sh, 0), mask_word(sh, 1), mask_word(sh, 2), mask_word(sh, 3)};
                            const uint32_t above = (x.v[0] & ~m[0]) | (x.v[1] & ~m[1]) | (x.v[2] & ~m[2]) | (x.v[3] & ~m[3]) | x.v[4] | x.v[5] | x.v[6] | x.v[7] |
                                                   (y.v[0] & ~m[0]) | (y.v[1] & ~m[1]) | (y.v[2] & ~m[2]) | (y.v[3] & ~m[3]) | y.v[4] | y.v[5] | y.v[6] | y.v[7];
                            if (sh <= 126u && !wave_any(both(active, above != 0u))) {
                                uint32_t d[4], bw = 0;
#pragma unroll
                                for (int k = 0; k < 4; ++k) d[k] = sbb32(x.v[k], y.v[k], bw);
                                const bool gen = both(active, bw != 0u), prop = both(active, (d[0] | d[1] | d[2] | d[3]) == 0u);
                                const uint32_t cin = scan_bit_lookahead<T>(seg, either(gen, both(both(seg, prop), a0 != 0u)), prop, lane);
                                const uint32_t bin = seg ? a0 : cin;
                                const bool bout = either(gen, both(prop, bin != 0u));
                                uint32_t e[4], b2 = 0;
                                e[0] = sbb32(d[0], bin, b2);
#pragma unroll
                                for (int k = 1; k < 4; ++k) e[k] = sbb32(d[k], 0u, b2);
                                uint32_t cy = 0;
#pragma unroll
                                for (int k = 0; k < 4; ++k) {
                                    const uint32_t add = (bout && (sh >> 5) == (uint32_t)k) ? (1u << (sh & 31u)) : 0u;
                                    e[k] = adc32(e[k], add, cy);
                                }
#pragma unroll
                                for (int k = 0; k < 4; ++k) r.v[k] = role_acc ? (k == 0 && bout ? 1u : 0u) : e[k];
                            } else {
                                Fr pw = fr_zero();
#pragma unroll
                                for (int k = 0; k < 8; ++k) pw.v[k] = (sh >> 5) == (uint32_t)k ? (1u << (sh & 31u)) : 0u;
                                uint32_t bo = 0;
                                Fr diff = fr_zero();
                                const Fr xy = fr_sub_wave(x, y, pv);
                                for (uint32_t it = 0; it < iters; ++it) {
                                    const uint32_t sft = wave_shr_lanes<D>(bo);
                                    Fr in = fr_zero();
                                    in.v[0] = start ? a0 : sft;
                                    const bool c = !signed_lt(x, fr_add_wave(y, in, pv));
                                    const Fr d0 = fr_sub_wave(xy, in, pv);
                                    diff = u256_select(c, d0, fr_add_wave(d0, pw, pv));
                                    bo = c ? 0u : 1u;
                                }
                                r = u256_select(role_acc, Fr{{bo, 0u, 0u, 0u, 0u, 0u, 0u, 0u}}, diff);
                            }
                        }
                    } else if (!(h & HDR_SCAN_DIV)) {
                        const bool small = !wave_any((x.v[4] | x.v[5] | x.v[6] | x.v[7] | acc0.v[4] | acc0.v[5] | acc0.v[6] | acc0.v[7]) != 0u) && sh >= 1u && sh <= 128u;
                        const bool seg = start || !active;
                        uint32_t xp[8];
                        {
                            uint32_t cy = 0;
#pragma unroll
                            for (int k = 0; k < 8; ++k) xp[k] = adc32(active ? x.v[k] : 0u, start && active ? acc0.v[k] : 0u, cy);
                            xp[7] |= cy << 31;
                        }
                        bool wide_ok = WIDE && sh != 64u && sh >= 32u && sh <= 126u && iters > 2u;
                        if (wide_ok) {
                            const Fr xpf = Fr{{xp[0], xp[1], xp[2], xp[3], xp[4], xp[5], xp[6], xp[7]}};
                            if (3u * sh >= 252u) {
                                wide_ok = !wave_any((xp[7] >> 28) != 0u);
                            } else {
                                const uint32_t top = 3u * sh;
                                uint32_t hi_or = 0;
#pragma unroll
                                for (int k = 0; k < 8; ++k) hi_or |= xp[k] & ~(top >= 32u * (k + 1) ? 0xffffffffu : top > 32u * k ? (1u << (top - 32u * k)) - 1u : 0u);
                                wide_ok = !wave_any(hi_or != 0u);
                            }
                            if (wide_ok) {
                                Fr limb, carry;
                                if (sh >= 96u) scan_carry_parallel_wide<T, 3>(seg, lane, sh, xpf, limb, carry);
                                else if (sh >= 64u) scan_carry_parallel_wide<T, 2>(seg, lane, sh, xpf, limb, carry);
                                else scan_carry_parallel_wide<T, 1>(seg, lane, sh, xpf, limb, carry);
                                r = u256_select(role_acc, carry, limb);
                            }
                        }
                        if (wide_ok) {
                        } else if (sh == 64u && iters > 2u && !wave_any((xp[6] | xp[7]) != 0u)) {
                            const uint32_t xw[6] = {xp[0], xp[1], xp[2], xp[3], xp[4], xp[5]};
                            uint32_t limb[2], carry[6];
                            scan_carry_parallel<T>(seg, lane, xw, limb, carry);
#pragma unroll
                            for (int k = 0; k < 6; ++k) r.v[k] = role_acc ? carry[k] : (k < 2 ? limb[k] : 0u);
                        } else if (small) {
                            const uint32_t m[4] = {mask_word(sh, 0), mask_word(sh, 1), mask_word(sh, 2), mask_word(sh, 3)};
                            const uint32_t xs[4] = {x.v[0], x.v[1], x.v[2], x.v[3]}, as[4] = {acc0.v[0], acc0.v[1], acc0.v[2], acc0.v[3]};
                            uint32_t limb[4], carry[4];
                            const uint32_t bs = sh & 31u;
                            switch (sh >> 5) {
                                case 0: scan_carry_rounds<0, D>(iters, bs, m, start, xs, as, limb, carry); break;
                                case 1: scan_carry_rounds<1, D>(iters, bs, m, start, xs, as, limb, carry); break;
                                case 2: scan_carry_rounds<2, D>(iters, bs, m, start, xs, as, limb, carry); break;
                                case 3: scan_carry_rounds<3, D>(iters, bs, m, start, xs, as, limb, carry); break;
                                default: scan_carry_rounds<4, D>(iters, bs, m, start, xs, as, limb, carry); break;
                            }
#pragma unroll
                            for (int k = 0; k < 4; ++k) r.v[k] = role_acc ? carry[k] : limb[k];
                        } else {
                            Fr c = fr_zero(), limb = fr_zero();
                            for (uint32_t it = 0; it < iters; ++it) {
                                Fr in;
#pragma unroll
                                for (int k = 0; k < 8; ++k) {
                                    const uint32_t sft = wave_shr_lanes<D>(c.v[k]);
                                    in.v[k] = start ? acc0.v[k] : sft;
                                }
                                const Fr t = fr_add_wave(x, in, pv);
#pragma unroll
                                for (int k = 0; k < 8; ++k) limb.v[k] = t.v[k] & mask_word(sh, (uint32_t)k);
                                c = u256_shr(t, sh);
                            }
                            r = u256_select(role_acc, c, limb);
                        }
                    } else {
                        const Fr d = fr_quad_perm<QP_ACC>(a_op), bm = fr_quad_perm<QP_ACC>(b_op);
                        const bool dz = u256_is_zero(d);
                        Fr ds = d;
                        ds.v[0] |= dz ? 1u : 0u;
                        const bool small = !wave_any((x.v[2] | x.v[3] | x.v[4] | x.v[5] | x.v[6] | x.v[7] | acc0.v[2] | acc0.v[3] | acc0.v[4] | acc0.v[5] | acc0.v[6] | acc0.v[7] |
                                                      d.v[2] | d.v[3] | d.v[4] | d.v[5] | d.v[6] | d.v[7]) != 0u) && sh >= 1u && sh <= 64u;
                        Fr quo = fr_zero(), rem = fr_zero();
                        if (small) {
                            const uint64_t dv = ((uint64_t)ds.v[1] << 32) | ds.v[0];
                            const uint32_t s = clz64_nonzero(dv);
                            const uint64_t dn = dv << s, rv = recip64(dn);
                            const uint64_t xl = ((uint64_t)x.v[1] << 32) | x.v[0];
                            const uint64_t a0 = ((uint64_t)acc0.v[1] << 32) | acc0.v[0];
                            uint64_t r64 = 0, qh = 0, ql = 0;
                            const bool seg = start || !active;
                            const uint64_t d_prev = ((uint64_t)wave_shr_lanes<D>((uint32_t)(dv >> 32)) << 32) | wave_shr_lanes<D>((uint32_t)dv);
                            if (sh == 64u && iters > 2u && !wave_any(both(active, either(dz, start ? a0 >= dv : dv != d_prev)))) {
                                scan_div_parallel<T>(seg, lane, iters, active ? dv : 1ull, active ? xl : 0ull, active ? a0 : 0ull, ql, r64);
                            } else if (sh == 64u) {
                                const uint64_t xn = xl << s, xh = (xl >> 1) >> (63u - s);
                                for (uint32_t it = 0; it < iters; ++it) {
                                    const uint32_t s0 = wave_shr_lanes<D>((uint32_t)r64), s1 = wave_shr_lanes<D>((uint32_t)(r64 >> 32));
                                    const uint64_t in = start ? a0 : (((uint64_t)s1 << 32) | s0);
                                    uint64_t q_h = 0, q_l, rr;
                                    if (wave_any(in >= dv)) {
                                        u128_divrem_64_recip(in, xl, dv, s, dn, rv, true, q_h, q_l, rr);
                                    } else {
                                        uint64_t rn;
                                        div2by1((in << s) | xh, xn, dn, rv, q_l, rn);
                                        rr = rn >> s;
                                    }
                                    qh = dz ? 0ull : q_h;
                                    ql = dz ? 0ull : q_l;
                                    r64 = dz ? 0ull : rr;
                                }
                            } else {
                                for (uint32_t it = 0; it < iters; ++it) {
                                    const uint32_t s0 = wave_shr_lanes<D>((uint32_t)r64), s1 = wave_shr_lanes<D>((uint32_t)(r64 >> 32));
                                    const uint64_t in = start ? a0 : (((uint64_t)s1 << 32) | s0);
                                    const uint64_t lo = in << sh, hi = (in >> 1) >> (63u - sh);
                                    const uint64_t tl = lo + xl, th = hi + (tl < lo ? 1ull : 0ull);
                                    uint64_t q_h, q_l, rr;
                                    u128_divrem_64_recip(th, tl, dv, s, dn, rv, wave_any(th >= dv), q_h, q_l, rr);
                                    qh = dz ? 0ull : q_h;
                                    ql = dz ? 0ull : q_l;
                                    r64 = dz ? 0ull : rr;
                                }
                            }
                            quo.v[0] = (uint32_t)ql; quo.v[1] = (uint32_t)(ql >> 32); quo.v[2] = (uint32_t)qh; quo.v[3] = (uint32_t)(qh >> 32);
                            rem.v[0] = (uint32_t)r64; rem.v[1] = (uint32_t)(r64 >> 32);
                        } else {
                            for (uint32_t it = 0; it < iters; ++it) {
                                Fr in;
#pragma unroll
                                for (int k = 0; k < 8; ++k) {
                                    const uint32_t sft = wave_shr_lanes<D>(rem.v[k]);
                                    in.v[k] = start ? acc0.v[k] : sft;
                                }
                                const Fr t = fr_add_wave(fr_mul_wave(in, bm, pv), x, pv);
                                const uint32_t lx = u256_bitlen(t), ly = u256_bitlen(ds);
                                const uint32_t my_dig = lx >= ly ? (lx - ly + 32u) >> 5 : 0u;
                                uint32_t dig = 0;
#pragma unroll
                                for (uint32_t dd = 1; dd <= 8; ++dd) dig = wave_any(my_dig >= dd) ? dd : dig;
                                Fr q1, r1;
                                u256_divrem_digits(q1, r1, t, ds, dig, ly);
                                quo = u256_select(dz, fr_zero(), q1);
                                rem = u256_select(dz, fr_zero(), r1);
                            }
                        }
                        r = u256_select(role_acc, rem, quo);
                    }
                }
                finish(r);
                continue;
            }
        }
        switch (cls) {
            case C_INPUT: {
                const uint32_t idx = crefs[(size_t)cref_row * G + j];
                ++cref_row;
                const uint4* q = inputs + ((size_t)set_c * p.n_inputs + idx) * 2;
                r = fr_mul_wave(fr_from_u4(q[0], q[1]), (h & HDR_OUT_CANON) ? fr_one() : fr_r2(), pv);
                break;
            }
            case C_DIVREQ: {
                if (DIVIDER) {
                    if (lane < ML) {
                        uint4* qa = reinterpret_cast<uint4*>(mbox + lane16);
                        uint4* qb = reinterpret_cast<uint4*>(mbox + 32u * ML + lane16);
                        qa[0] = make_uint4(a_op.v[0], a_op.v[1], a_op.v[2], a_op.v[3]);
                        qa[ML] = make_uint4(a_op.v[4], a_op.v[5], a_op.v[6], a_op.v[7]);
                        qb[0] = make_uint4(b_op.v[0], b_op.v[1], b_op.v[2], b_op.v[3]);
                        qb[ML] = make_uint4(b_op.v[4], b_op.v[5], b_op.v[6], b_op.v[7]);
                    }
                    __builtin_amdgcn_fence(__ATOMIC_RELEASE, "workgroup");
                    if (lane == 0) seq[wave] = div_seq + 1;
                }
                r = fr_zero();
                break;
            }
            case C_DIVGET: {
                r = fr_zero();
                if (DIVIDER) {
                    ++div_seq;
                    if (!mbox_wait(seq + NW + wave / WD, div_seq)) err_bits |= ST_DIVIDER_TIMEOUT;
                    __builtin_amdgcn_fence(__ATOMIC_ACQUIRE, "workgroup");
                    if (lane < ML) {
                        const uint4* qr = reinterpret_cast<const uint4*>(mbox + lane16);
                        r = fr_from_u4(qr[0], qr[ML]);
                    }
                }
                break;
            }
            case C_DIV: {
                const Fr inv = fr_inv(b_op);
                r = u256_select(u256_is_zero(b_op), fr_zero(), fr_mul(a_op, inv));
                break;
            }
            case C_CMPZ: {
                const bool az = u256_is_zero(a_op), cz = u256_is_zero(b_op), eq = u256_eq(a_op, b_op);
                const bool v = either(either(both(sub == SUB_EQ, eq), both(sub == SUB_NEQ, !eq)), either(both(sub == SUB_LAND, !either(az, cz)), both(both(sub != SUB_EQ, both(sub != SUB_NEQ, sub != SUB_LAND)), !both(az, cz))));
                r = u256_select(v, one_out(), fr_zero());
                break;
            }
            case C_CMPS: {
                const Fr x = (h & HDR_A_CANON) ? a_op : fr_from_mont(a_op), y = (h & HDR_B_CANON) ? b_op : fr_from_mont(b_op);
                auto less = [](const Fr& a, const Fr& b) {
                    Fr t;
                    const uint32_t borrow = u256_sub(t, a, b);
                    if constexpr (M2) asm volatile("" ::"v"(t.v[7]));
                    return borrow != 0;
                };
                bool lt, gt;
                bool limb_sized = false;
                if constexpr (M2) limb_sized = !wave_any(both(active, (x.v[4] | x.v[5] | x.v[6] | x.v[7] | y.v[4] | y.v[5] | y.v[6] | y.v[7]) != 0u));
                if (M2 && limb_sized) {
                    uint32_t d[4], bw = 0;
#pragma unroll
                    for (int k = 0; k < 4; ++k) d[k] = sbb32(x.v[k], y.v[k], bw);
                    lt = bw != 0u;
                    gt = both(bw == 0u, (d[0] | d[1] | d[2] | d[3]) != 0u);
                } else {
                    const bool xn = less(fr_half(), x), yn = less(fr_half(), y);
                    const bool same = xn == yn, xy = less(x, y), yx = less(y, x);
                    lt = same ? xy : xn;
                    gt = same ? yx : yn;
                }
                const bool v = either(either(both(sub == SUB_LT, lt), both(sub == SUB_GT, gt)), either(both(sub == SUB_LEQ, !gt), both(both(sub != SUB_LT, both(sub != SUB_GT, sub != SUB_LEQ)), !lt)));
                r = u256_select(v, one_out(), fr_zero());
                break;
            }
            case C_BIT: {
                const Fr x = (h & HDR_A_CANON) ? a_op : fr_from_mont(a_op);
                const uint32_t kx = rec_hi.y >> 20;
                const bool is_x = sub == SUB_BITX;
                if (h & HDR_BITX_ALL) {
                    const Fr e = u256_shr(x, kx);
                    r = u256_select((e.v[0] & 1u) != 0u, one_out(), fr_zero());
                    break;
                }
                const Fr y = (h & HDR_B_CANON) ? b_op : fr_from_mont(b_op);
                auto bit_result = [&](const Fr& d) -> Fr {
                    if (h & HDR_OUT_CANON) return d;
                    const bool small = both(d.v[0] < 2u, (d.v[1] | d.v[2] | d.v[3] | d.v[4] | d.v[5] | d.v[6] | d.v[7]) == 0u);
                    if (wave_any(!small)) return fr_mul_wave(d, fr_r2(), pv);
                    return u256_select(d.v[0] != 0u, fr_one(), fr_zero());
                };
                if (h & (HDR_BIT_ALL_SHR | HDR_BIT_ALL_BAND)) {
                    Fr d;
#pragma unroll
                    for (int i = 0; i < 8; ++i) d.v[i] = x.v[i] & y.v[i];
                    if (h & HDR_BIT_ALL_SHR) {
                        const bool big = either((y.v[1] | y.v[2] | y.v[3] | y.v[4] | y.v[5] | y.v[6] | y.v[7]) != 0u, y.v[0] >= 254u);
                        const Fr sh = u256_select(big, fr_zero(), u256_shr(x, big ? 0u : y.v[0]));
                        d = u256_select(sub == SUB_SHR, sh, d);
                    }
                    r = bit_result(d);
                    break;
                }
                uint32_t hi_or = 0;
#pragma unroll
                for (int i = 1; i < 8; ++i) hi_or |= y.v[i];
                const bool big = either(hi_or != 0u, y.v[0] >= 254u);
                const uint32_t n = is_x ? kx : big ? 0u : y.v[0];
                const bool shifts = either(either(sub == SUB_SHL, sub == SUB_SHR), is_x);
                Fr d = u256_shr(x, n);
                if (wave_any(sub == SUB_SHL)) d = u256_select(sub == SUB_SHL, u256_shl(x, n), d);
                d = u256_select(both(big, !is_x), fr_zero(), d);
                d.v[0] &= is_x ? 1u : 0xffffffffu;
#pragma unroll
                for (int i = 1; i < 8; ++i) d.v[i] = is_x ? 0u : d.v[i];
                {
                    const bool over = both(sub == SUB_SHL, !u256_lt(d, fr_p()));
                    err_bits |= both(over, active) ? ST_SHL_OVERFLOW : 0u;
                    d = u256_select(over, fr_zero(), d);
                }
                {
                    const uint32_t m_and = sub == SUB_BAND ? 0xffffffffu : 0u, m_or = sub == SUB_BAND ? 0u : 0xffffffffu, m_xor = (sub == SUB_BAND || sub == SUB_BOR) ? 0u : 0xffffffffu;
                    Fr e;
#pragma unroll
                    for (int i = 0; i < 8; ++i) {
                        const uint32_t a = x.v[i] & y.v[i], o = x.v[i] | y.v[i];
                        e.v[i] = (a & m_and) | ((o & m_or) & ~(a & m_xor));
                    }
                    Fr em;
                    const uint32_t br = u256_sub(em, e, fr_p());
                    err_bits |= both(both(br == 0u, u256_is_zero(em)), both(active, !shifts)) ? ST_BITOP_EQ_R : 0u;
                    e = u256_select(br == 0u, em, e);
                    d = u256_select(shifts, d, e);
                }
                r = bit_result(d);
                break;
            }
            case C_IDIVMOD: {
                const Fr x = (h & HDR_A_CANON) ? a_op : fr_from_mont(a_op), y = (h & HDR_B_CANON) ? b_op : fr_from_mont(b_op);
                const bool yz = u256_is_zero(y);
                Fr ys = y;
                ys.v[0] |= yz ? 1u : 0u;
                Fr q, rem;
                bool two_words = false;
                if constexpr (WIDE) two_words = !wave_any(both(both(active, !yz), either((ys.v[2] | ys.v[3]) == 0u, (ys.v[4] | ys.v[5] | ys.v[6] | ys.v[7]) != 0u)));
                if (!wave_any((x.v[4] | x.v[5] | x.v[6] | x.v[7] | ys.v[2] | ys.v[3] | ys.v[4] | ys.v[5] | ys.v[6] | ys.v[7]) != 0u)) {
                    u128_divrem_64(q, rem, x, ys);
                } else if (WIDE && two_words) {
                    const bool sub = either(yz, !active);
                    Fr yy = ys;
                    yy.v[0] = sub ? 0u : ys.v[0];
                    yy.v[1] = sub ? 0u : ys.v[1];
                    yy.v[2] = sub ? 1u : ys.v[2];
                    yy.v[3] = sub ? 0u : ys.v[3];
#pragma unroll
                    for (int k = 4; k < 8; ++k) yy.v[k] = 0u;
                    u256_divrem_128(q, rem, x, yy);
                } else {
                    const uint32_t lx = u256_bitlen(x), ly = u256_bitlen(ys);
                    const uint32_t my_dig = lx >= ly ? (lx - ly + 32u) >> 5 : 0u;
                    uint32_t dig = 0;
#pragma unroll
                    for (uint32_t dd = 1; dd <= 8; ++dd) dig = wave_any(my_dig >= dd) ? dd : dig;
                    u256_divrem_digits(q, rem, x, ys, dig, ly);
                }
                const Fr d = u256_select(yz, fr_zero(), u256_select(sub == SUB_IDIV, q, rem));
                r = (h & HDR_OUT_CANON) ? d : fr_mul_wave(d, fr_r2(), pv);
                break;
            }
            case C_TERN: {
                const uint32_t cr = crefs[(size_t)cref_row * G + j];
                ++cref_row;
                const Fr y = ld(cr + t16);
                r = u256_select(u256_is_zero(a_op), y, b_op);
                break;
            }
            case C_SYNC: {
                r = fr_zero();
                if (h & HDR_POST) {
                    asm volatile("s_waitcnt vmcnt(0)" ::: "memory");
                    ++n_posts;
                    if (lane == 0) __hip_atomic_store(sync_words + stream, n_posts, __ATOMIC_RELEASE, __HIP_MEMORY_SCOPE_AGENT);
                }
                if (h & HDR_WAIT) {
                    ++n_waits;
                    if (!post_wait(sync_words, n_waits)) err_bits |= ST_SYNC_TIMEOUT;
                }
                break;
            }
            case C_SCAN: r = fr_zero(); break;
            default: r = fr_zero(); break;
        }
        finish(r);
    }
    __builtin_amdgcn_raw_buffer_store_b128(u32x4{r_prev.v[0], r_prev.v[1], r_prev.v[2], r_prev.v[3]}, rsrc, (int)doff_prev, 0, 0);
    __builtin_amdgcn_raw_buffer_store_b128(u32x4{r_prev.v[4], r_prev.v[5], r_prev.v[6], r_prev.v[7]}, rsrc, (int)doff_prev + (int)HI, 0, 0);
    if (PROF && lane == 0) {
        const unsigned long long cyc = __builtin_amdgcn_s_memtime() - t_wave0;
        atomicMax(&prof[54], cyc);
        atomicMax(&prof[55], (1ull << 40) - cyc);
        atomicAdd(&prof[62], cyc);
        atomicAdd(&prof[63], 1ull);
    }
    if constexpr (PROF) {
        if (unsigned long long* c = census_slot()) c[2] = __builtin_amdgcn_s_memtime();
    }
    if (PROF && lane == 0 && (tile % 64u) == 0u) {
#pragma unroll
        for (int c = 0; c < C_PROF; ++c) {
            atomicAdd(&prof[c * 4 + 0], pf[c][0]);
            atomicAdd(&prof[c * 4 + 3], pf[c][1]);
        }
        atomicAdd(&prof[M2 ? 68 : 64], pf_fused[0]);
        atomicAdd(&prof[M2 ? 71 : 67], pf_fused[1]);
        if (M2) {
#pragma unroll
            for (int q = 0; q < 5; ++q) {
                atomicAdd(&prof[72 + 4 * q], pf_scan[q][0]);
                atomicAdd(&prof[75 + 4 * q], pf_scan[q][1]);
            }
        }
#pragma unroll
        for (int k = 0; k < 2; ++k)
#pragma unroll
            for (int q = 0; q < 6; ++q) atomicAdd(&prof[48 + 8 * k + q], psec[k][q]);
        atomicAdd(&prof[92], psec[0][6]);
        atomicAdd(&prof[93], psec[1][6]);
    }
    if (err_bits && set < batch) atomicOr(&status[set], err_bits);
}

__global__ __launch_bounds__(256) void fill_consts_kernel(ProgramDev p, WsTable wst, uint32_t n_tiles, uint32_t T) {
    const uint32_t e = blockIdx.x * 256u + threadIdx.x;
    const uint32_t pieces = p.n_const * 2u * T;
    if (e >= pieces) return;
    const uint4 v = reinterpret_cast<const uint4*>(p.consts)[(size_t)(e / (2u * T)) * 2u + (e / T) % 2u];
    const uint64_t tile_bytes = ws_tile_bytes(p.n_const, p.n_slots, T);
    for (uint32_t tile = blockIdx.y; tile < n_tiles; tile += gridDim.y) {
        char* tb = reinterpret_cast<char*>(wst.base[tile / wst.tiles_per_chunk]) + (uint64_t)(tile % wst.tiles_per_chunk) * tile_bytes;
        reinterpret_cast<uint4*>(tb)[e] = v;
    }
}

template <bool MONT>
__device__ __forceinline__ Fr pack_form(const Fr& v, bool canon) {
    if (MONT) return canon ? fr_mul(v, fr_r2()) : v;
    return canon ? v : fr_from_mont(v);
}

template <bool MONT, int TT>
__global__ __launch_bounds__(256) void pack_kernel(ProgramDev p, WsTable wst, uint4* __restrict__ out, uint32_t batch, uint32_t T_, uint32_t first) {
    const uint32_t T = TT ? (uint32_t)TT : T_;
    const uint32_t wi = first + blockIdx.x * 256u + threadIdx.x;
    if (wi >= p.n_witness) return;
    const uint32_t w = first ? p.pack_order[wi] : wi;
    const uint32_t ref_raw = p.witness_refs[w];
    const bool canon = (ref_raw & REF_CANON) != 0;
    const uint32_t ref = ref_raw & ~REF_CANON;
    const uint32_t n_tiles = (batch + T - 1) / T;
    const uint64_t tile_bytes = ws_tile_bytes(p.n_const, p.n_slots, T);
    const uint32_t slot = (ref & REF_CONST) ? (ref & ~REF_CONST) : p.n_const + ref;
    for (uint32_t tile = blockIdx.y; tile < n_tiles; tile += gridDim.y) {
        const char* tb = reinterpret_cast<const char*>(wst.base[tile / wst.tiles_per_chunk]) + (uint64_t)(tile % wst.tiles_per_chunk) * tile_bytes;
        const uint4* q = reinterpret_cast<const uint4*>(tb) + (size_t)slot * (2 * T);
        if (TT != 0 && TT <= 4) {
            uint4 lo[TT ? TT : 1], hi[TT ? TT : 1];
#pragma unroll
            for (int t = 0; t < TT; ++t) {
                lo[t] = q[t];
                hi[t] = q[TT + t];
            }
#pragma unroll
            for (int t = 0; t < TT; ++t) {
                const uint32_t set = tile * TT + t;
                if (set >= batch) break;
                const Fr c = pack_form<MONT>(fr_from_u4(lo[t], hi[t]), canon);
                uint4* o = out + ((size_t)set * p.n_witness + w) * 2;
                o[0] = make_uint4(c.v[0], c.v[1], c.v[2], c.v[3]);
                o[1] = make_uint4(c.v[4], c.v[5], c.v[6], c.v[7]);
            }
        } else {
            for (uint32_t t = 0; t < T; ++t) {
                const uint32_t set = tile * T + t;
                if (set >= batch) break;
                const Fr c = pack_form<MONT>(fr_from_u4(q[t], q[T + t]), canon);
                uint4* o = out + ((size_t)set * p.n_witness + w) * 2;
                o[0] = make_uint4(c.v[0], c.v[1], c.v[2], c.v[3]);
                o[1] = make_uint4(c.v[4], c.v[5], c.v[6], c.v[7]);
            }
        }
    }
}

template <bool MONT, int TT>
__global__ __launch_bounds__(256) void pack_kernel_v3(ProgramDev p, WsTable wst, uint4* __restrict__ out, uint32_t batch, uint32_t first) {
    constexpr uint32_t T = TT, WPB = 256u / T;
    const uint32_t t = threadIdx.x % T, wi = first + blockIdx.x * WPB + threadIdx.x / T;
    if (wi >= p.n_witness) return;
    const uint32_t w = first ? p.pack_order[wi] : wi;
    const uint32_t ref_raw = p.witness_refs[w];
    const bool canon = (ref_raw & REF_CANON) != 0;
    const uint32_t ref = ref_raw & ~REF_CANON;
    const uint32_t n_tiles = (batch + T - 1) / T;
    const uint64_t tile_bytes = ws_tile_bytes(p.n_const, p.n_slots, T);
    const uint32_t slot = (ref & REF_CONST) ? (ref & ~REF_CONST) : p.n_const + ref;
    for (uint32_t tile = blockIdx.y; tile < n_tiles; tile += gridDim.y) {
        const uint32_t set = tile * T + t;
        if (set >= batch) continue;
        const char* tb = reinterpret_cast<const char*>(wst.base[tile / wst.tiles_per_chunk]) + (uint64_t)(tile % wst.tiles_per_chunk) * tile_bytes;
        const uint4* q = reinterpret_cast<const uint4*>(tb) + (size_t)slot * (2 * T);
        const Fr c = pack_form<MONT>(fr_from_u4(q[t], q[T + t]), canon);
        uint4* o = out + ((size_t)set * p.n_witness + w) * 2;
        o[0] = make_uint4(c.v[0], c.v[1], c.v[2], c.v[3]);
        o[1] = make_uint4(c.v[4], c.v[5], c.v[6], c.v[7]);
    }
}

template <bool MONT>
__global__ __launch_bounds__(256) void pack_kernel_v1(ProgramDev p, WsTable wst, uint4* __restrict__ out, uint32_t batch, uint32_t T, uint32_t first) {
    const uint32_t wi = first + blockIdx.x * 64u + threadIdx.x;
    if (wi >= p.n_witness) return;
    const uint32_t w = first ? p.pack_order[wi] : wi;
    const uint32_t ref_raw = p.witness_refs[w];
    const bool canon = (ref_raw & REF_CANON) != 0;
    const uint32_t ref = ref_raw & ~REF_CANON;
    const uint32_t n_tiles = (batch + T - 1) / T;
    const uint64_t tile_bytes = ws_tile_bytes(p.n_const, p.n_slots, T);
    const uint32_t slot = (ref & REF_CONST) ? (ref & ~REF_CONST) : p.n_const + ref;
    for (uint32_t tile = blockIdx.y; tile < n_tiles; tile += gridDim.y) {
        const char* tb = reinterpret_cast<const char*>(wst.base[tile / wst.tiles_per_chunk]) + (uint64_t)(tile % wst.tiles_per_chunk) * tile_bytes;
        const uint4* q0 = reinterpret_cast<const uint4*>(tb) + (size_t)slot * (2 * T);
        for (uint32_t t = threadIdx.y; t < T; t += blockDim.y) {
            const uint32_t set = tile * T + t;
            if (set >= batch) break;
            const uint4* q = q0 + t;
            const Fr c = pack_form<MONT>(fr_from_u4(q[0], q[T]), canon);
            uint4* o = out + ((size_t)set * p.n_witness + w) * 2;
            o[0] = make_uint4(c.v[0], c.v[1], c.v[2], c.v[3]);
            o[1] = make_uint4(c.v[4], c.v[5], c.v[6], c.v[7]);
        }
    }
}

hipError_t launch_interp(uint32_t T, uint32_t W, uint32_t pack, uint32_t n_div_requests, const uint32_t* div_lanes, const ProgramDev& p,
                         const WsTable& wst, const void* inputs, uint32_t* status, uint32_t batch, hipStream_t stream, unsigned long long* prof,
                         void* out, uint32_t n_inline, bool montgomery) {
    const uint32_t tiles = (batch + T - 1) / T, nw = (W ? W : 1u) * pack, ns = p.n_streams ? p.n_streams : 1u;
    if (nw == 0 || nw % ns != 0 || (ns > 1 && W > 1)) return hipErrorInvalidValue;
    const uint32_t tiles_per_wg = nw / ns;
    dim3 grid((tiles + tiles_per_wg - 1) / tiles_per_wg), block((W ? (W + 1) * pack : pack) * 64);
    const uint4* in = (const uint4*)inputs;
    InterpDims dims{p.n_bundles, p.n_slots, p.n_inputs, batch, p.n_const, n_div_requests, p.trash_off, div_lanes, ns, {0, 0, 0, 0}, {0, 0, 0, 0}, {0, 0, 0, 0}, {0, 0, 0, 0},
                    (uint4*)out, reinterpret_cast<const uint2*>(p.pack_entries), p.pack_ready, 0u, montgomery ? 1u : 0u, p.n_witness};
    if (W == 1 && ns == 1 && out && p.pack_entries && p.pack_ready) dims.n_inline = n_inline < p.n_ready_last ? n_inline : p.n_ready_last;
    for (uint32_t s = 0; s < MAX_STREAMS; ++s) {
        dims.stream_first[s] = p.stream_first[s];
        dims.stream_count[s] = p.stream_count[s];
        dims.stream_div_requests[s] = p.stream_div_requests[s];
        dims.stream_cref_first[s] = p.stream_cref_first[s];
    }
    if (ns == 1) {
        dims.stream_first[0] = 0;
        dims.stream_count[0] = p.n_bundles;
        dims.stream_div_requests[0] = n_div_requests;
    }
    const uint4* recs = reinterpret_cast<const uint4*>(p.recs);
    const uint32_t mode = p.has_fused;
    static_assert(SCAN_MAX_T == COOP_FUSE_MAX_T, "the instances with a MODE are made for tile widths up to COOP_FUSE_MAX_T");
    if (mode > 3 || (mode && (T > COOP_FUSE_MAX_T || W > 1))) return hipErrorInvalidValue;
#define CWC_LAUNCH3(TT, PP, WW, KK)                                                                                                     \
    do {                                                                                                                                \
        if constexpr ((uint32_t)(TT) <= COOP_FUSE_MAX_T && (WW) <= 1) {                                                                 \
            if (mode == 3) interp_kernel<TT, PP, WW, KK, 3><<<grid, block, 0, stream>>>(p.hdr, recs, p.crefs, dims, wst, in, status, prof); \
            else if (mode == 2) interp_kernel<TT, PP, WW, KK, 2><<<grid, block, 0, stream>>>(p.hdr, recs, p.crefs, dims, wst, in, status, prof); \
            else if (mode == 1) interp_kernel<TT, PP, WW, KK, 1><<<grid, block, 0, stream>>>(p.hdr, recs, p.crefs, dims, wst, in, status, prof); \
            else interp_kernel<TT, PP, WW, KK, 0><<<grid, block, 0, stream>>>(p.hdr, recs, p.crefs, dims, wst, in, status, prof);     \
        } else {                                                                                                                        \
            interp_kernel<TT, PP, WW, KK, 0><<<grid, block, 0, stream>>>(p.hdr, recs, p.crefs, dims, wst, in, status, prof);          \
        }                                                                                                                               \
    } while (0)
#define CWC_LAUNCH2(TT, PP)                                  \
    if (W == 0 && pack == 1) CWC_LAUNCH3(TT, PP, 0, 1);      \
    else if (W == 0 && pack == 4) CWC_LAUNCH3(TT, PP, 0, 4); \
    else if (W == 1 && pack == 1) CWC_LAUNCH3(TT, PP, 1, 1); \
    else if (W == 1 && pack == 2) CWC_LAUNCH3(TT, PP, 1, 2); \
    else if (W == 1 && pack == 4) CWC_LAUNCH3(TT, PP, 1, 4); \
    else if (W == 3 && pack == 1) CWC_LAUNCH3(TT, PP, 3, 1); \
    else if (W == 4 && pack == 1) CWC_LAUNCH3(TT, PP, 4, 1); \
    else return hipErrorInvalidValue;
#ifdef CWC_DIAG
#define CWC_LAUNCH_PROF(TT, WW, KK) CWC_LAUNCH3(TT, true, WW, KK)
#define CWC_LAUNCH2_PROF(TT) CWC_LAUNCH2(TT, true)
#else
#define CWC_LAUNCH_PROF(TT, WW, KK) return hipErrorNotSupported
#define CWC_LAUNCH2_PROF(TT) return hipErrorNotSupported;
#endif
#define CWC_LAUNCH(TT)                                    \
    case TT:                                              \
        if (prof) { CWC_LAUNCH2_PROF(TT) } else { CWC_LAUNCH2(TT, false) } \
        break;
    switch (T) {
        CWC_LAUNCH(1) CWC_LAUNCH(2) CWC_LAUNCH(4) CWC_LAUNCH(8) CWC_LAUNCH(16) CWC_LAUNCH(32)
        case 64:
            if (W != 0) return hipErrorInvalidValue;
            if (pack == 4) { if (prof) { CWC_LAUNCH_PROF(64, 0, 4); } else CWC_LAUNCH3(64, false, 0, 4); }
            else if (pack == 1) { if (prof) { CWC_LAUNCH_PROF(64, 0, 1); } else CWC_LAUNCH3(64, false, 0, 1); }
            else return hipErrorInvalidValue;
            break;
        default: return hipErrorInvalidValue;
    }
#undef CWC_LAUNCH_PROF
#undef CWC_LAUNCH2_PROF
#undef CWC_LAUNCH
#undef CWC_LAUNCH2
#undef CWC_LAUNCH3
    return hipGetLastError();
}

#ifndef CWC_KSRC_HASH
#define CWC_KSRC_HASH "unstamped"
#endif
extern "C" const char* gwb_kernel_source_hash() { return CWC_KSRC_HASH; }
extern "C" int gwb_kernels_have_diagnostics() {
#ifdef CWC_DIAG
    return 1;
#else
    return 0;
#endif
}

__global__ void warm_kernel() {}
hipError_t launch_warm(hipStream_t stream) {
    warm_kernel<<<1, 64, 0, stream>>>();
    return hipGetLastError();
}

hipError_t launch_fill_consts(uint32_t T, const ProgramDev& p, const WsTable& wst, uint32_t n_tiles, hipStream_t stream) {
    if (n_tiles == 0 || p.n_const == 0) return hipSuccess;
    dim3 grid((p.n_const * 2u * T + 255u) / 256u, n_tiles < 16384u ? n_tiles : 16384u), block(256);
    fill_consts_kernel<<<grid, block, 0, stream>>>(p, wst, n_tiles, T);
    return hipGetLastError();
}

hipError_t launch_pack(uint32_t T, const ProgramDev& p, const WsTable& wst, void* out, uint32_t batch, hipStream_t stream, bool montgomery, int pack_shape, uint32_t first) {
    if (p.n_witness == 0 || batch == 0 || first >= p.n_witness) return hipSuccess;
    const uint32_t count = p.n_witness - first;
    const uint32_t n_tiles = (batch + T - 1) / T;
    if (pack_shape == 1 || T > 4) {
        dim3 grid((count + 63) / 64, n_tiles < 32768u ? n_tiles : 32768u), block(64, T < 4 ? T : 4);
        if (montgomery) pack_kernel_v1<true><<<grid, block, 0, stream>>>(p, wst, (uint4*)out, batch, T, first);
        else pack_kernel_v1<false><<<grid, block, 0, stream>>>(p, wst, (uint4*)out, batch, T, first);
        return hipGetLastError();
    }
    if (pack_shape == 3 && T >= 2) {
        dim3 grid3((count + 256 / T - 1) / (256 / T), n_tiles < 32768u ? n_tiles : 32768u), block3(256);
#define CWC_PACK3(MM, TT) pack_kernel_v3<MM, TT><<<grid3, block3, 0, stream>>>(p, wst, (uint4*)out, batch, first)
        if (montgomery) {
            if (T == 2) CWC_PACK3(true, 2); else CWC_PACK3(true, 4);
        } else {
            if (T == 2) CWC_PACK3(false, 2); else CWC_PACK3(false, 4);
        }
#undef CWC_PACK3
        return hipGetLastError();
    }
    dim3 grid((count + 255) / 256, n_tiles < 32768u ? n_tiles : 32768u), block(256);
#define CWC_PACK(MM, TT) pack_kernel<MM, TT><<<grid, block, 0, stream>>>(p, wst, (uint4*)out, batch, T, first)
    if (montgomery) {
        if (T == 1) CWC_PACK(true, 1); else if (T == 2) CWC_PACK(true, 2); else CWC_PACK(true, 4);
    } else {
        if (T == 1) CWC_PACK(false, 1); else if (T == 2) CWC_PACK(false, 2); else CWC_PACK(false, 4);
    }
#undef CWC_PACK
    return hipGetLastError();
}

__global__ __launch_bounds__(1024) void modmul_ubench_kernel(uint32_t* sink, uint32_t iters) {
    Fr a = fr_r2(), b = fr_one();
    a.v[0] ^= threadIdx.x + blockIdx.x * 977u;
    for (uint32_t it = 0; it < iters; ++it) {
        a = fr_mul(a, b);
        b = fr_mul(b, a);
    }
    if (a.v[0] == 0x1234567u && b.v[3] == 7u) sink[0] = a.v[1];
}
__global__ __launch_bounds__(512) void modmul_block_ubench_kernel(uint32_t* sink, uint32_t iters) {
    Fr a = fr_r2(), b = fr_one(), pv = fr_p();
#pragma unroll
    for (int i = 0; i < 8; ++i) asm volatile("" : "+v"(pv.v[i]));
    a.v[0] ^= threadIdx.x + blockIdx.x * 977u;
    for (uint32_t it = 0; it < iters; ++it) {
        a = fr_mul_wave(a, b, pv);
        b = fr_mul_wave(b, a, pv);
    }
    if (a.v[0] == 0x1234567u && b.v[3] == 7u) sink[0] = a.v[1];
}
hipError_t launch_modmul_ubench(uint32_t n_cus, uint32_t waves_per_simd, uint32_t iters, uint32_t* sink, hipStream_t stream, bool block_multiplier) {
    if (block_multiplier) {
        if (waves_per_simd > 2) return hipErrorInvalidValue;
        modmul_block_ubench_kernel<<<n_cus, 256 * waves_per_simd, 0, stream>>>(sink, iters);
    } else {
        modmul_ubench_kernel<<<n_cus, 256 * waves_per_simd, 0, stream>>>(sink, iters);
    }
    return hipGetLastError();
}

}
```

Baseline: 94330.

## Use lazy Montgomery reduction in [0,2p) and canonicalize only at consumers

```diff
diff --git a/circom-witnesscalc_amd/csrc/fr_gfx950.hpp b/circom-witnesscalc_amd/csrc/fr_gfx950.hpp
--- a/circom-witnesscalc_amd/csrc/fr_gfx950.hpp
+++ b/circom-witnesscalc_amd/csrc/fr_gfx950.hpp
@@ -229,7 +229,38 @@
     out[0] = out[1] = 0;
 #endif
 }
-#endif
+__device__ __forceinline__ Fr fr_mul_wave_lazy(const Fr& a, const Fr& b) {
+#if defined(__HIP_DEVICE_COMPILE__)
+#include "fr_mul_block_lazy_gfx950.inc"
+#else
+    (void)a; (void)b;
+    return fr_zero();
+#endif
+}
+__device__ __forceinline__ void fr_mul_coop4_lazy(const Fr& a, uint32_t b0, uint32_t b1, uint32_t n0, uint32_t n1, uint32_t* out) {
+#if defined(__HIP_DEVICE_COMPILE__)
+#include "fr_mul_coop4_lazy_gfx950.inc"
+#else
+    (void)a; (void)b0; (void)b1; (void)n0; (void)n1;
+    out[0] = out[1] = 0;
+#endif
+}
+__device__ __forceinline__ void fr_mul_coop4r_lazy(const Fr& a, uint32_t aq0, uint32_t aq1, uint32_t b0, uint32_t b1, uint32_t n0, uint32_t n1,
+                                                   uint32_t nn0, uint32_t nn1, uint32_t sub, uint32_t* out) {
+#if defined(__HIP_DEVICE_COMPILE__)
+#include "fr_mul_coop4r_lazy_gfx950.inc"
+#else
+    (void)a; (void)aq0; (void)aq1; (void)b0; (void)b1; (void)n0; (void)n1; (void)nn0; (void)nn1; (void)sub;
+    out[0] = out[1] = 0;
+#endif
+}
+#endif
+FRD Fr fr_2p() { return Fr{{0xe0000002u, 0x87c3eb27u, 0xf372e122u, 0x5067d090u, 0x0302b0bau, 0x70a08b6du, 0xc2634053u, 0x60c89ce5u}}; }
+FRD Fr fr_canon(const Fr& v) {
+    Fr t;
+    const uint32_t br = u256_sub(t, v, fr_p());
+    return u256_select(br != 0, v, t);
+}
 FRD Fr fr_sqr(const Fr& a) { return fr_mul(a, a); }
 
 FRD Fr fr_to_mont(const Fr& x) { return fr_mul(x, fr_r2()); }
diff --git a/circom-witnesscalc_amd/csrc/fr_mul_block_lazy_gfx950.inc b/circom-witnesscalc_amd/csrc/fr_mul_block_lazy_gfx950.inc
--- /dev/null
+++ b/circom-witnesscalc_amd/csrc/fr_mul_block_lazy_gfx950.inc
@@ -0,0 +1,18 @@
+{
+    unsigned int t0, t1, t2, t3, t4, t5, t6, t7, m0, m1, m2, m3, m4, m5, m6, m7;
+    unsigned long long cA, cB, cC;
+    const unsigned int p0 = 0xf0000001u;
+    const unsigned int p1 = 0x43e1f593u;
+    const unsigned int p2 = 0x79b97091u;
+    const unsigned int p3 = 0x2833e848u;
+    const unsigned int p4 = 0x8181585du;
+    const unsigned int p5 = 0xb85045b6u;
+    const unsigned int p6 = 0xe131a029u;
+    const unsigned int p7 = 0x30644e72u;
+    const unsigned int inv32 = 0xefffffffu;
+    asm volatile("v_mad_u64_u32 v[160:161], %[cA], %[a0], %[b0], 0\n\ts_nop 1\n\ts_nop 0\n\tv_addc_co_u32_e64 v162, %[cA], 0, 0, %[cA]\n\tv_mul_lo_u32 %[m0], v160, %[inv]\n\tv_mad_u64_u32 v[160:161], %[cB], %[m0], %[p0], v[160:161]\n\ts_nop 1\n\ts_nop 0\n\tv_addc_co_u32_e64 v162, %[cB], 0, v162, %[cB]\n\tv_pk_mov_b32 v[164:165], v[160:161], v[162:163] op_sel:[1,0]\n\tv_mad_u64_u32 v[164:165], %[cA], %[a0], %[b1], v[164:165]\n\tv_mad_u64_u32 v[164:165], %[cB], %[a1], %[b0], v[164:165]\n\tv_mad_u64_u32 v[164:165], %[cC], %[m0], %[p1], v[164:165]\n\tv_addc_co_u32_e64 v166, %[cA], 0, 0, %[cA]\n\tv_addc_co_u32_e64 v166, %[cB], 0, v166, %[cB]\n\tv_addc_co_u32_e64 v166, %[cC], 0, v166, %[cC]\n\tv_mul_lo_u32 %[m1], v164, %[inv]\n\tv_mad_u64_u32 v[164:165], %[cA], %[m1], %[p0], v[164:165]\n\ts_nop 1\n\ts_nop 0\n\tv_addc_co_u32_e64 v166, %[cA], 0, v166, %[cA]\n\tv_pk_mov_b32 v[160:161], v[164:165], v[166:167] op_sel:[1,0]\n\tv_mad_u64_u32 v[160:161], %[cA], %[a0], %[b2], v[160:161]\n\tv_mad_u64_u32 v[160:161], %[cB], %[a1], %[b1], v[160:161]\n\tv_mad_u64_u32 v[160:161], %[cC], %[a2], %[b0], v[160:161]\n\tv_addc_co_u32_e64 v162, %[cA], 0, 0, %[cA]\n\tv_mad_u64_u32 v[160:161], %[cA], %[m0], %[p2], v[160:161]\n\tv_addc_co_u32_e64 v162, %[cB], 0, v162, %[cB]\n\tv_mad_u64_u32 v[160:161], %[cB], %[m1], %[p1], v[160:161]\n\tv_addc_co_u32_e64 v162, %[cC], 0, v162, %[cC]\n\tv_addc_co_u32_e64 v162, %[cA], 0, v162, %[cA]\n\tv_addc_co_u32_e64 v162, %[cB], 0, v162, %[cB]\n\tv_mul_lo_u32 %[m2], v160, %[inv]\n\tv_mad_u64_u32 v[160:161], %[cC], %[m2], %[p0], v[160:161]\n\ts_nop 1\n\ts_nop 0\n\tv_addc_co_u32_e64 v162, %[cC], 0, v162, %[cC]\n\tv_pk_mov_b32 v[164:165], v[160:161], v[162:163] op_sel:[1,0]\n\tv_mad_u64_u32 v[164:165], %[cA], %[a0], %[b3], v[164:165]\n\tv_mad_u64_u32 v[164:165], %[cB], %[a1], %[b2], v[164:165]\n\tv_mad_u64_u32 v[164:165], %[cC], %[a2], %[b1], v[164:165]\n\tv_addc_co_u32_e64 v166, %[cA], 0, 0, %[cA]\n\tv_mad_u64_u32 v[164:165], %[cA], %[a3], %[b0], v[164:165]\n\tv_addc_co_u32_e64 v166, %[cB], 0, v166, %[cB]\n\tv_mad_u64_u32 v[164:165], %[cB], %[m0], %[p3], v[164:165]\n\tv_addc_co_u32_e64 v166, %[cC], 0, v166, %[cC]\n\tv_mad_u64_u32 v[164:165], %[cC], %[m1], %[p2], v[164:165]\n\tv_addc_co_u32_e64 v166, %[cA], 0, v166, %[cA]\n\tv_mad_u64_u32 v[164:165], %[cA], %[m2], %[p1], v[164:165]\n\tv_addc_co_u32_e64 v166, %[cB], 0, v166, %[cB]\n\tv_addc_co_u32_e64 v166, %[cC], 0, v166, %[cC]\n\tv_addc_co_u32_e64 v166, %[cA], 0, v166, %[cA]\n\tv_mul_lo_u32 %[m3], v164, %[inv]\n\tv_mad_u64_u32 v[164:165], %[cB], %[m3], %[p0], v[164:165]\n\ts_nop 1\n\ts_nop 0\n\tv_addc_co_u32_e64 v166, %[cB], 0, v166, %[cB]\n\tv_pk_mov_b32 v[160:161], v[164:165], v[166:167] op_sel:[1,0]\n\tv_mad_u64_u32 v[160:161], %[cA], %[a0], %[b4], v[160:161]\n\tv_mad_u64_u32 v[160:161], %[cB], %[a1], %[b3], v[160:161]\n\tv_mad_u64_u32 v[160:161], %[cC], %[a2], %[b2], v[160:161]\n\tv_addc_co_u32_e64 v162, %[cA], 0, 0, %[cA]\n\tv_mad_u64_u32 v[160:161], %[cA], %[a3], %[b1], v[160:161]\n\tv_addc_co_u32_e64 v162, %[cB], 0, v162, %[cB]\n\tv_mad_u64_u32 v[160:161], %[cB], %[a4], %[b0], v[160:161]\n\tv_addc_co_u32_e64 v162, %[cC], 0, v162, %[cC]\n\tv_mad_u64_u32 v[160:161], %[cC], %[m0], %[p4], v[160:161]\n\tv_addc_co_u32_e64 v162, %[cA], 0, v162, %[cA]\n\tv_mad_u64_u32 v[160:161], %[cA], %[m1], %[p3], v[160:161]\n\tv_addc_co_u32_e64 v162, %[cB], 0, v162, %[cB]\n\tv_mad_u64_u32 v[160:161], %[cB], %[m2], %[p2], v[160:161]\n\tv_addc_co_u32_e64 v162, %[cC], 0, v162, %[cC]\n\tv_mad_u64_u32 v[160:161], %[cC], %[m3], %[p1], v[160:161]\n\tv_addc_co_u32_e64 v162, %[cA], 0, v162, %[cA]\n\tv_addc_co_u32_e64 v162, %[cB], 0, v162, %[cB]\n\tv_addc_co_u32_e64 v162, %[cC], 0, v162, %[cC]\n\tv_mul_lo_u32 %[m4], v160, %[inv]\n\tv_mad_u64_u32 v[160:161], %[cA], %[m4], %[p0], v[160:161]\n\ts_nop 1\n\ts_nop 0\n\tv_addc_co_u32_e64 v162, %[cA], 0, v162, %[cA]\n\tv_pk_mov_b32 v[164:165], v[160:161], v[162:163] op_sel:[1,0]\n\tv_mad_u64_u32 v[164:165], %[cA], %[a0], %[b5], v[164:165]\n\tv_mad_u64_u32 v[164:165], %[cB], %[a1], %[b4], v[164:165]\n\tv_mad_u64_u32 v[164:165], %[cC], %[a2], %[b3], v[164:165]\n\tv_addc_co_u32_e64 v166, %[cA], 0, 0, %[cA]\n\tv_mad_u64_u32 v[164:165], %[cA], %[a3], %[b2], v[164:165]\n\tv_addc_co_u32_e64 v166, %[cB], 0, v166, %[cB]\n\tv_mad_u64_u32 v[164:165], %[cB], %[a4], %[b1], v[164:165]\n\tv_addc_co_u32_e64 v166, %[cC], 0, v166, %[cC]\n\tv_mad_u64_u32 v[164:165], %[cC], %[a5], %[b0], v[164:165]\n\tv_addc_co_u32_e64 v166, %[cA], 0, v166, %[cA]\n\tv_mad_u64_u32 v[164:165], %[cA], %[m0], %[p5], v[164:165]\n\tv_addc_co_u32_e64 v166, %[cB], 0, v166, %[cB]\n\tv_mad_u64_u32 v[164:165], %[cB], %[m1], %[p4], v[164:165]\n\tv_addc_co_u32_e64 v166, %[cC], 0, v166, %[cC]\n\tv_mad_u64_u32 v[164:165], %[cC], %[m2], %[p3], v[164:165]\n\tv_addc_co_u32_e64 v166, %[cA], 0, v166, %[cA]\n\tv_mad_u64_u32 v[164:165], %[cA], %[m3], %[p2], v[164:165]\n\tv_addc_co_u32_e64 v166, %[cB], 0, v166, %[cB]\n\tv_mad_u64_u32 v[164:165], %[cB], %[m4], %[p1], v[164:165]\n\tv_addc_co_u32_e64 v166, %[cC], 0, v166, %[cC]\n\tv_addc_co_u32_e64 v166, %[cA], 0, v166, %[cA]\n\tv_addc_co_u32_e64 v166, %[cB], 0, v166, %[cB]\n\tv_mul_lo_u32 %[m5], v164, %[inv]\n\tv_mad_u64_u32 v[164:165], %[cC], %[m5], %[p0], v[164:165]\n\ts_nop 1\n\ts_nop 0\n\tv_addc_co_u32_e64 v166, %[cC], 0, v166, %[cC]\n\tv_pk_mov_b32 v[160:161], v[164:165], v[166:167] op_sel:[1,0]\n\tv_mad_u64_u32 v[160:161], %[cA], %[a0], %[b6], v[160:161]\n\tv_mad_u64_u32 v[160:161], %[cB], %[a1], %[b5], v[160:161]\n\tv_mad_u64_u32 v[160:161], %[cC], %[a2], %[b4], v[160:161]\n\tv_addc_co_u32_e64 v162, %[cA], 0, 0, %[cA]\n\tv_mad_u64_u32 v[160:161], %[cA], %[a3], %[b3], v[160:161]\n\tv_addc_co_u32_e64 v162, %[cB], 0, v162, %[cB]\n\tv_mad_u64_u32 v[160:161], %[cB], %[a4], %[b2], v[160:161]\n\tv_addc_co_u32_e64 v162, %[cC], 0, v162, %[cC]\n\tv_mad_u64_u32 v[160:161], %[cC], %[a5], %[b1], v[160:161]\n\tv_addc_co_u32_e64 v162, %[cA], 0, v162, %[cA]\n\tv_mad_u64_u32 v[160:161], %[cA], %[a6], %[b0], v[160:161]\n\tv_addc_co_u32_e64 v162, %[cB], 0, v162, %[cB]\n\tv_mad_u64_u32 v[160:161], %[cB], %[m0], %[p6], v[160:161]\n\tv_addc_co_u32_e64 v162, %[cC], 0, v162, %[cC]\n\tv_mad_u64_u32 v[160:161], %[cC], %[m1], %[p5], v[160:161]\n\tv_addc_co_u32_e64 v162, %[cA], 0, v162, %[cA]\n\tv_mad_u64_u32 v[160:161], %[cA], %[m2], %[p4], v[160:161]\n\tv_addc_co_u32_e64 v162, %[cB], 0, v162, %[cB]\n\tv_mad_u64_u32 v[160:161], %[cB], %[m3], %[p3], v[160:161]\n\tv_addc_co_u32_e64 v162, %[cC], 0, v162, %[cC]\n\tv_mad_u64_u32 v[160:161], %[cC], %[m4], %[p2], v[160:161]\n\tv_addc_co_u32_e64 v162, %[cA], 0, v162, %[cA]\n\tv_mad_u64_u32 v[160:161], %[cA], %[m5], %[p1], v[160:161]\n\tv_addc_co_u32_e64 v162, %[cB], 0, v162, %[cB]\n\tv_addc_co_u32_e64 v162, %[cC], 0, v162, %[cC]\n\tv_addc_co_u32_e64 v162, %[cA], 0, v162, %[cA]\n\tv_mul_lo_u32 %[m6], v160, %[inv]\n\tv_mad_u64_u32 v[160:161], %[cB], %[m6], %[p0], v[160:161]\n\ts_nop 1\n\ts_nop 0\n\tv_addc_co_u32_e64 v162, %[cB], 0, v162, %[cB]\n\tv_pk_mov_b32 v[164:165], v[160:161], v[162:163] op_sel:[1,0]\n\tv_mad_u64_u32 v[164:165], %[cA], %[a0], %[b7], v[164:165]\n\tv_mad_u64_u32 v[164:165], %[cB], %[a1], %[b6], v[164:165]\n\tv_mad_u64_u32 v[164:165], %[cC], %[a2], %[b5], v[164:165]\n\tv_addc_co_u32_e64 v166, %[cA], 0, 0, %[cA]\n\tv_mad_u64_u32 v[164:165], %[cA], %[a3], %[b4], v[164:165]\n\tv_addc_co_u32_e64 v166, %[cB], 0, v166, %[cB]\n\tv_mad_u64_u32 v[164:165], %[cB], %[a4], %[b3], v[164:165]\n\tv_addc_co_u32_e64 v166, %[cC], 0, v166, %[cC]\n\tv_mad_u64_u32 v[164:165], %[cC], %[a5], %[b2], v[164:165]\n\tv_addc_co_u32_e64 v166, %[cA], 0, v166, %[cA]\n\tv_mad_u64_u32 v[164:165], %[cA], %[a6], %[b1], v[164:165]\n\tv_addc_co_u32_e64 v166, %[cB], 0, v166, %[cB]\n\tv_mad_u64_u32 v[164:165], %[cB], %[a7], %[b0], v[164:165]\n\tv_addc_co_u32_e64 v166, %[cC], 0, v166, %[cC]\n\tv_mad_u64_u32 v[164:165], %[cC], %[m0], %[p7], v[164:165]\n\tv_addc_co_u32_e64 v166, %[cA], 0, v166, %[cA]\n\tv_mad_u64_u32 v[164:165], %[cA], %[m1], %[p6], v[164:165]\n\tv_addc_co_u32_e64 v166, %[cB], 0, v166, %[cB]\n\tv_mad_u64_u32 v[164:165], %[cB], %[m2], %[p5], v[164:165]\n\tv_addc_co_u32_e64 v166, %[cC], 0, v166, %[cC]\n\tv_mad_u64_u32 v[164:165], %[cC], %[m3], %[p4], v[164:165]\n\tv_addc_co_u32_e64 v166, %[cA], 0, v166, %[cA]\n\tv_mad_u64_u32 v[164:165], %[cA], %[m4], %[p3], v[164:165]\n\tv_addc_co_u32_e64 v166, %[cB], 0, v166, %[cB]\n\tv_mad_u64_u32 v[164:165], %[cB], %[m5], %[p2], v[164:165]\n\tv_addc_co_u32_e64 v166, %[cC], 0, v166, %[cC]\n\tv_mad_u64_u32 v[164:165], %[cC], %[m6], %[p1], v[164:165]\n\tv_addc_co_u32_e64 v166, %[cA], 0, v166, %[cA]\n\tv_addc_co_u32_e64 v166, %[cB], 0, v166, %[cB]\n\tv_addc_co_u32_e64 v166, %[cC], 0, v166, %[cC]\n\tv_mul_lo_u32 %[m7], v164, %[inv]\n\tv_mad_u64_u32 v[164:165], %[cA], %[m7], %[p0], v[164:165]\n\ts_nop 1\n\ts_nop 0\n\tv_addc_co_u32_e64 v166, %[cA], 0, v166, %[cA]\n\tv_pk_mov_b32 v[160:161], v[164:165], v[166:167] op_sel:[1,0]\n\tv_mad_u64_u32 v[160:161], %[cA], %[a1], %[b7], v[160:161]\n\tv_mad_u64_u32 v[160:161], %[cB], %[a2], %[b6], v[160:161]\n\tv_mad_u64_u32 v[160:161], %[cC], %[a3], %[b5], v[160:161]\n\tv_addc_co_u32_e64 v162, %[cA], 0, 0, %[cA]\n\tv_mad_u64_u32 v[160:161], %[cA], %[a4], %[b4], v[160:161]\n\tv_addc_co_u32_e64 v162, %[cB], 0, v162, %[cB]\n\tv_mad_u64_u32 v[160:161], %[cB], %[a5], %[b3], v[160:161]\n\tv_addc_co_u32_e64 v162, %[cC], 0, v162, %[cC]\n\tv_mad_u64_u32 v[160:161], %[cC], %[a6], %[b2], v[160:161]\n\tv_addc_co_u32_e64 v162, %[cA], 0, v162, %[cA]\n\tv_mad_u64_u32 v[160:161], %[cA], %[a7], %[b1], v[160:161]\n\tv_addc_co_u32_e64 v162, %[cB], 0, v162, %[cB]\n\tv_mad_u64_u32 v[160:161], %[cB], %[m1], %[p7], v[160:161]\n\tv_addc_co_u32_e64 v162, %[cC], 0, v162, %[cC]\n\tv_mad_u64_u32 v[160:161], %[cC], %[m2], %[p6], v[160:161]\n\tv_addc_co_u32_e64 v162, %[cA], 0, v162, %[cA]\n\tv_mad_u64_u32 v[160:161], %[cA], %[m3], %[p5], v[160:161]\n\tv_addc_co_u32_e64 v162, %[cB], 0, v162, %[cB]\n\tv_mad_u64_u32 v[160:161], %[cB], %[m4], %[p4], v[160:161]\n\tv_addc_co_u32_e64 v162, %[cC], 0, v162, %[cC]\n\tv_mad_u64_u32 v[160:161], %[cC], %[m5], %[p3], v[160:161]\n\tv_addc_co_u32_e64 v162, %[cA], 0, v162, %[cA]\n\tv_mad_u64_u32 v[160:161], %[cA], %[m6], %[p2], v[160:161]\n\tv_addc_co_u32_e64 v162, %[cB], 0, v162, %[cB]\n\tv_mad_u64_u32 v[160:161], %[cB], %[m7], %[p1], v[160:161]\n\tv_addc_co_u32_e64 v162, %[cC], 0, v162, %[cC]\n\tv_addc_co_u32_e64 v162, %[cA], 0, v162, %[cA]\n\tv_addc_co_u32_e64 v162, %[cB], 0, v162, %[cB]\n\tv_mov_b32 %[t0], v160\n\tv_pk_mov_b32 v[164:165], v[160:161], v[162:163] op_sel:[1,0]\n\tv_mad_u64_u32 v[164:165], %[cA], %[a2], %[b7], v[164:165]\n\tv_mad_u64_u32 v[164:165], %[cB], %[a3], %[b6], v[164:165]\n\tv_mad_u64_u32 v[164:165], %[cC], %[a4], %[b5], v[164:165]\n\tv_addc_co_u32_e64 v166, %[cA], 0, 0, %[cA]\n\tv_mad_u64_u32 v[164:165], %[cA], %[a5], %[b4], v[164:165]\n\tv_addc_co_u32_e64 v166, %[cB], 0, v166, %[cB]\n\tv_mad_u64_u32 v[164:165], %[cB], %[a6], %[b3], v[164:165]\n\tv_addc_co_u32_e64 v166, %[cC], 0, v166, %[cC]\n\tv_mad_u64_u32 v[164:165], %[cC], %[a7], %[b2], v[164:165]\n\tv_addc_co_u32_e64 v166, %[cA], 0, v166, %[cA]\n\tv_mad_u64_u32 v[164:165], %[cA], %[m2], %[p7], v[164:165]\n\tv_addc_co_u32_e64 v166, %[cB], 0, v166, %[cB]\n\tv_mad_u64_u32 v[164:165], %[cB], %[m3], %[p6], v[164:165]\n\tv_addc_co_u32_e64 v166, %[cC], 0, v166, %[cC]\n\tv_mad_u64_u32 v[164:165], %[cC], %[m4], %[p5], v[164:165]\n\tv_addc_co_u32_e64 v166, %[cA], 0, v166, %[cA]\n\tv_mad_u64_u32 v[164:165], %[cA], %[m5], %[p4], v[164:165]\n\tv_addc_co_u32_e64 v166, %[cB], 0, v166, %[cB]\n\tv_mad_u64_u32 v[164:165], %[cB], %[m6], %[p3], v[164:165]\n\tv_addc_co_u32_e64 v166, %[cC], 0, v166, %[cC]\n\tv_mad_u64_u32 v[164:165], %[cC], %[m7], %[p2], v[164:165]\n\tv_addc_co_u32_e64 v166, %[cA], 0, v166, %[cA]\n\tv_addc_co_u32_e64 v166, %[cB], 0, v166, %[cB]\n\tv_addc_co_u32_e64 v166, %[cC], 0, v166, %[cC]\n\tv_mov_b32 %[t1], v164\n\tv_pk_mov_b32 v[160:161], v[164:165], v[166:167] op_sel:[1,0]\n\tv_mad_u64_u32 v[160:161], %[cA], %[a3], %[b7], v[160:161]\n\tv_mad_u64_u32 v[160:161], %[cB], %[a4], %[b6], v[160:161]\n\tv_mad_u64_u32 v[160:161], %[cC], %[a5], %[b5], v[160:161]\n\tv_addc_co_u32_e64 v162, %[cA], 0, 0, %[cA]\n\tv_mad_u64_u32 v[160:161], %[cA], %[a6], %[b4], v[160:161]\n\tv_addc_co_u32_e64 v162, %[cB], 0, v162, %[cB]\n\tv_mad_u64_u32 v[160:161], %[cB], %[a7], %[b3], v[160:161]\n\tv_addc_co_u32_e64 v162, %[cC], 0, v162, %[cC]\n\tv_mad_u64_u32 v[160:161], %[cC], %[m3], %[p7], v[160:161]\n\tv_addc_co_u32_e64 v162, %[cA], 0, v162, %[cA]\n\tv_mad_u64_u32 v[160:161], %[cA], %[m4], %[p6], v[160:161]\n\tv_addc_co_u32_e64 v162, %[cB], 0, v162, %[cB]\n\tv_mad_u64_u32 v[160:161], %[cB], %[m5], %[p5], v[160:161]\n\tv_addc_co_u32_e64 v162, %[cC], 0, v162, %[cC]\n\tv_mad_u64_u32 v[160:161], %[cC], %[m6], %[p4], v[160:161]\n\tv_addc_co_u32_e64 v162, %[cA], 0, v162, %[cA]\n\tv_mad_u64_u32 v[160:161], %[cA], %[m7], %[p3], v[160:161]\n\tv_addc_co_u32_e64 v162, %[cB], 0, v162, %[cB]\n\tv_addc_co_u32_e64 v162, %[cC], 0, v162, %[cC]\n\tv_addc_co_u32_e64 v162, %[cA], 0, v162, %[cA]\n\tv_mov_b32 %[t2], v160\n\tv_pk_mov_b32 v[164:165], v[160:161], v[162:163] op_sel:[1,0]\n\tv_mad_u64_u32 v[164:165], %[cA], %[a4], %[b7], v[164:165]\n\tv_mad_u64_u32 v[164:165], %[cB], %[a5], %[b6], v[164:165]\n\tv_mad_u64_u32 v[164:165], %[cC], %[a6], %[b5], v[164:165]\n\tv_addc_co_u32_e64 v166, %[cA], 0, 0, %[cA]\n\tv_mad_u64_u32 v[164:165], %[cA], %[a7], %[b4], v[164:165]\n\tv_addc_co_u32_e64 v166, %[cB], 0, v166, %[cB]\n\tv_mad_u64_u32 v[164:165], %[cB], %[m4], %[p7], v[164:165]\n\tv_addc_co_u32_e64 v166, %[cC], 0, v166, %[cC]\n\tv_mad_u64_u32 v[164:165], %[cC], %[m5], %[p6], v[164:165]\n\tv_addc_co_u32_e64 v166, %[cA], 0, v166, %[cA]\n\tv_mad_u64_u32 v[164:165], %[cA], %[m6], %[p5], v[164:165]\n\tv_addc_co_u32_e64 v166, %[cB], 0, v166, %[cB]\n\tv_mad_u64_u32 v[164:165], %[cB], %[m7], %[p4], v[164:165]\n\tv_addc_co_u32_e64 v166, %[cC], 0, v166, %[cC]\n\tv_addc_co_u32_e64 v166, %[cA], 0, v166, %[cA]\n\tv_addc_co_u32_e64 v166, %[cB], 0, v166, %[cB]\n\tv_mov_b32 %[t3], v164\n\tv_pk_mov_b32 v[160:161], v[164:165], v[166:167] op_sel:[1,0]\n\tv_mad_u64_u32 v[160:161], %[cA], %[a5], %[b7], v[160:161]\n\tv_mad_u64_u32 v[160:161], %[cB], %[a6], %[b6], v[160:161]\n\tv_mad_u64_u32 v[160:161], %[cC], %[a7], %[b5], v[160:161]\n\tv_addc_co_u32_e64 v162, %[cA], 0, 0, %[cA]\n\tv_mad_u64_u32 v[160:161], %[cA], %[m5], %[p7], v[160:161]\n\tv_addc_co_u32_e64 v162, %[cB], 0, v162, %[cB]\n\tv_mad_u64_u32 v[160:161], %[cB], %[m6], %[p6], v[160:161]\n\tv_addc_co_u32_e64 v162, %[cC], 0, v162, %[cC]\n\tv_mad_u64_u32 v[160:161], %[cC], %[m7], %[p5], v[160:161]\n\tv_addc_co_u32_e64 v162, %[cA], 0, v162, %[cA]\n\tv_addc_co_u32_e64 v162, %[cB], 0, v162, %[cB]\n\tv_addc_co_u32_e64 v162, %[cC], 0, v162, %[cC]\n\tv_mov_b32 %[t4], v160\n\tv_pk_mov_b32 v[164:165], v[160:161], v[162:163] op_sel:[1,0]\n\tv_mad_u64_u32 v[164:165], %[cA], %[a6], %[b7], v[164:165]\n\tv_mad_u64_u32 v[164:165], %[cB], %[a7], %[b6], v[164:165]\n\tv_mad_u64_u32 v[164:165], %[cC], %[m6], %[p7], v[164:165]\n\tv_addc_co_u32_e64 v166, %[cA], 0, 0, %[cA]\n\tv_mad_u64_u32 v[164:165], %[cA], %[m7], %[p6], v[164:165]\n\tv_addc_co_u32_e64 v166, %[cB], 0, v166, %[cB]\n\tv_addc_co_u32_e64 v166, %[cC], 0, v166, %[cC]\n\tv_addc_co_u32_e64 v166, %[cA], 0, v166, %[cA]\n\tv_mov_b32 %[t5], v164\n\tv_pk_mov_b32 v[160:161], v[164:165], v[166:167] op_sel:[1,0]\n\tv_mad_u64_u32 v[160:161], %[cA], %[a7], %[b7], v[160:161]\n\tv_mad_u64_u32 v[160:161], %[cB], %[m7], %[p7], v[160:161]\n\tv_mov_b32 %[t6], v160\n\tv_addc_co_u32_e64 v162, %[cA], 0, 0, %[cA]\n\tv_addc_co_u32_e64 v162, %[cB], 0, v162, %[cB]\n\tv_pk_mov_b32 v[164:165], v[160:161], v[162:163] op_sel:[1,0]\n\tv_mov_b32 %[t7], v164"
+                 : [t0] "=&v"(t0), [t1] "=&v"(t1), [t2] "=&v"(t2), [t3] "=&v"(t3), [t4] "=&v"(t4), [t5] "=&v"(t5), [t6] "=&v"(t6), [t7] "=&v"(t7), [m0] "=&v"(m0), [m1] "=&v"(m1), [m2] "=&v"(m2), [m3] "=&v"(m3), [m4] "=&v"(m4), [m5] "=&v"(m5), [m6] "=&v"(m6), [m7] "=&v"(m7), [cA] "=&s"(cA), [cB] "=&s"(cB), [cC] "=&s"(cC)
+                 : [a0] "v"(a.v[0]), [a1] "v"(a.v[1]), [a2] "v"(a.v[2]), [a3] "v"(a.v[3]), [a4] "v"(a.v[4]), [a5] "v"(a.v[5]), [a6] "v"(a.v[6]), [a7] "v"(a.v[7]), [b0] "v"(b.v[0]), [b1] "v"(b.v[1]), [b2] "v"(b.v[2]), [b3] "v"(b.v[3]), [b4] "v"(b.v[4]), [b5] "v"(b.v[5]), [b6] "v"(b.v[6]), [b7] "v"(b.v[7]), [p0] "s"(p0), [p1] "s"(p1), [p2] "s"(p2), [p3] "s"(p3), [p4] "s"(p4), [p5] "s"(p5), [p6] "s"(p6), [p7] "s"(p7), [inv] "s"(inv32)
+                 : "v160", "v161", "v162", "v163", "v164", "v165", "v166", "v167");
+    return Fr{{t0, t1, t2, t3, t4, t5, t6, t7}};
+}
diff --git a/circom-witnesscalc_amd/csrc/fr_mul_coop4_lazy_gfx950.inc b/circom-witnesscalc_amd/csrc/fr_mul_coop4_lazy_gfx950.inc
--- /dev/null
+++ b/circom-witnesscalc_amd/csrc/fr_mul_coop4_lazy_gfx950.inc
@@ -0,0 +1,12 @@
+{
+    unsigned int r0, r1;
+    unsigned long long sc0, sc1, sc2, sc3, sp;
+    const unsigned int inv32 = 0xefffffffu;
+    const unsigned long long top = 0x8888888888888888ull, lane0 = 0x1111111111111111ull;
+    asm volatile("v_mad_u64_u32 v[172:173], %[sc0], %[a0], %[b0], 0\n\tv_mul_lo_u32 v170, v172, %[inv]\n\tv_mad_u64_u32 v[176:177], %[sc1], %[a0], %[b1], 0\n\tv_mov_b32_e32 v169, 0\n\tv_mov_b32_dpp v171, v170 quad_perm:[0,0,0,0] row_mask:0xf bank_mask:0xf bound_ctrl:0\n\tv_mad_u64_u32 v[172:173], %[sc2], v171, %[n0], v[172:173]\n\tv_mad_u64_u32 v[176:177], %[sc3], v171, %[n1], v[176:177]\n\tv_add_co_u32_e64 v176, %[sc0], v176, v173\n\tv_addc_co_u32_e64 v174, %[sc2], 0, 0, %[sc2]\n\tv_addc_co_u32_e64 v178, %[sc3], 0, 0, %[sc3]\n\tv_addc_co_u32_e64 v177, %[sc0], v177, v174, %[sc0]\n\tv_mad_u64_u32 v[176:177], %[sc1], %[a1], %[b0], v[176:177]\n\tv_mul_lo_u32 v170, v176, %[inv]\n\tv_mov_b32_dpp v168, v172 quad_perm:[1,2,3,0] row_mask:0xf bank_mask:0xf bound_ctrl:0\n\tv_addc_co_u32_e64 v178, %[sc0], v178, 0, %[sc0]\n\tv_mad_u64_u32 v[172:173], %[sc2], %[a1], %[b1], v[168:169]\n\tv_mov_b32_dpp v171, v170 quad_perm:[0,0,0,0] row_mask:0xf bank_mask:0xf bound_ctrl:0\n\tv_addc_co_u32_e64 v178, %[sc1], v178, 0, %[sc1]\n\tv_mad_u64_u32 v[176:177], %[sc3], v171, %[n0], v[176:177]\n\tv_mad_u64_u32 v[172:173], %[sc0], v171, %[n1], v[172:173]\n\tv_add_co_u32_e64 v172, %[sc1], v172, v177\n\tv_addc_co_u32_e64 v178, %[sc3], v178, 0, %[sc3]\n\tv_addc_co_u32_e64 v174, %[sc0], 0, 0, %[sc0]\n\tv_addc_co_u32_e64 v173, %[sc1], v173, v178, %[sc1]\n\tv_mad_u64_u32 v[172:173], %[sc2], %[a2], %[b0], v[172:173]\n\tv_mul_lo_u32 v170, v172, %[inv]\n\tv_mov_b32_dpp v168, v176 quad_perm:[1,2,3,0] row_mask:0xf bank_mask:0xf bound_ctrl:0\n\tv_addc_co_u32_e64 v174, %[sc1], v174, 0, %[sc1]\n\tv_mad_u64_u32 v[176:177], %[sc3], %[a2], %[b1], v[168:169]\n\tv_mov_b32_dpp v171, v170 quad_perm:[0,0,0,0] row_mask:0xf bank_mask:0xf bound_ctrl:0\n\tv_addc_co_u32_e64 v174, %[sc2], v174, 0, %[sc2]\n\tv_mad_u64_u32 v[172:173], %[sc0], v171, %[n0], v[172:173]\n\tv_mad_u64_u32 v[176:177], %[sc1], v171, %[n1], v[176:177]\n\tv_add_co_u32_e64 v176, %[sc2], v176, v173\n\tv_addc_co_u32_e64 v174, %[sc0], v174, 0, %[sc0]\n\tv_addc_co_u32_e64 v178, %[sc1], 0, 0, %[sc1]\n\tv_addc_co_u32_e64 v177, %[sc2], v177, v174, %[sc2]\n\tv_mad_u64_u32 v[176:177], %[sc3], %[a3], %[b0], v[176:177]\n\tv_mul_lo_u32 v170, v176, %[inv]\n\tv_mov_b32_dpp v168, v172 quad_perm:[1,2,3,0] row_mask:0xf bank_mask:0xf bound_ctrl:0\n\tv_addc_co_u32_e64 v178, %[sc2], v178, 0, %[sc2]\n\tv_mad_u64_u32 v[172:173], %[sc0], %[a3], %[b1], v[168:169]\n\tv_mov_b32_dpp v171, v170 quad_perm:[0,0,0,0] row_mask:0xf bank_mask:0xf bound_ctrl:0\n\tv_addc_co_u32_e64 v178, %[sc3], v178, 0, %[sc3]\n\tv_mad_u64_u32 v[176:177], %[sc1], v171, %[n0], v[176:177]\n\tv_mad_u64_u32 v[172:173], %[sc2], v171, %[n1], v[172:173]\n\tv_add_co_u32_e64 v172, %[sc3], v172, v177\n\tv_addc_co_u32_e64 v178, %[sc1], v178, 0, %[sc1]\n\tv_addc_co_u32_e64 v174, %[sc2], 0, 0, %[sc2]\n\tv_addc_co_u32_e64 v173, %[sc3], v173, v178, %[sc3]\n\tv_mad_u64_u32 v[172:173], %[sc0], %[a4], %[b0], v[172:173]\n\tv_mul_lo_u32 v170, v172, %[inv]\n\tv_mov_b32_dpp v168, v176 quad_perm:[1,2,3,0] row_mask:0xf bank_mask:0xf bound_ctrl:0\n\tv_addc_co_u32_e64 v174, %[sc3], v174, 0, %[sc3]\n\tv_mad_u64_u32 v[176:177], %[sc1], %[a4], %[b1], v[168:169]\n\tv_mov_b32_dpp v171, v170 quad_perm:[0,0,0,0] row_mask:0xf bank_mask:0xf bound_ctrl:0\n\tv_addc_co_u32_e64 v174, %[sc0], v174, 0, %[sc0]\n\tv_mad_u64_u32 v[172:173], %[sc2], v171, %[n0], v[172:173]\n\tv_mad_u64_u32 v[176:177], %[sc3], v171, %[n1], v[176:177]\n\tv_add_co_u32_e64 v176, %[sc0], v176, v173\n\tv_addc_co_u32_e64 v174, %[sc2], v174, 0, %[sc2]\n\tv_addc_co_u32_e64 v178, %[sc3], 0, 0, %[sc3]\n\tv_addc_co_u32_e64 v177, %[sc0], v177, v174, %[sc0]\n\tv_mad_u64_u32 v[176:177], %[sc1], %[a5], %[b0], v[176:177]\n\tv_mul_lo_u32 v170, v176, %[inv]\n\tv_mov_b32_dpp v168, v172 quad_perm:[1,2,3,0] row_mask:0xf bank_mask:0xf bound_ctrl:0\n\tv_addc_co_u32_e64 v178, %[sc0], v178, 0, %[sc0]\n\tv_mad_u64_u32 v[172:173], %[sc2], %[a5], %[b1], v[168:169]\n\tv_mov_b32_dpp v171, v170 quad_perm:[0,0,0,0] row_mask:0xf bank_mask:0xf bound_ctrl:0\n\tv_addc_co_u32_e64 v178, %[sc1], v178, 0, %[sc1]\n\tv_mad_u64_u32 v[176:177], %[sc3], v171, %[n0], v[176:177]\n\tv_mad_u64_u32 v[172:173], %[sc0], v171, %[n1], v[172:173]\n\tv_add_co_u32_e64 v172, %[sc1], v172, v177\n\tv_addc_co_u32_e64 v178, %[sc3], v178, 0, %[sc3]\n\tv_addc_co_u32_e64 v174, %[sc0], 0, 0, %[sc0]\n\tv_addc_co_u32_e64 v173, %[sc1], v173, v178, %[sc1]\n\tv_mad_u64_u32 v[172:173], %[sc2], %[a6], %[b0], v[172:173]\n\tv_mul_lo_u32 v170, v172, %[inv]\n\tv_mov_b32_dpp v168, v176 quad_perm:[1,2,3,0] row_mask:0xf bank_mask:0xf bound_ctrl:0\n\tv_addc_co_u32_e64 v174, %[sc1], v174, 0, %[sc1]\n\tv_mad_u64_u32 v[176:177], %[sc3], %[a6], %[b1], v[168:169]\n\tv_mov_b32_dpp v171, v170 quad_perm:[0,0,0,0] row_mask:0xf bank_mask:0xf bound_ctrl:0\n\tv_addc_co_u32_e64 v174, %[sc2], v174, 0, %[sc2]\n\tv_mad_u64_u32 v[172:173], %[sc0], v171, %[n0], v[172:173]\n\tv_mad_u64_u32 v[176:177], %[sc1], v171, %[n1], v[176:177]\n\tv_add_co_u32_e64 v176, %[sc2], v176, v173\n\tv_addc_co_u32_e64 v174, %[sc0], v174, 0, %[sc0]\n\tv_addc_co_u32_e64 v178, %[sc1], 0, 0, %[sc1]\n\tv_addc_co_u32_e64 v177, %[sc2], v177, v174, %[sc2]\n\tv_mad_u64_u32 v[176:177], %[sc3], %[a7], %[b0], v[176:177]\n\tv_mul_lo_u32 v170, v176, %[inv]\n\tv_mov_b32_dpp v168, v172 quad_perm:[1,2,3,0] row_mask:0xf bank_mask:0xf bound_ctrl:0\n\tv_addc_co_u32_e64 v178, %[sc2], v178, 0, %[sc2]\n\tv_mad_u64_u32 v[172:173], %[sc0], %[a7], %[b1], v[168:169]\n\tv_mov_b32_dpp v171, v170 quad_perm:[0,0,0,0] row_mask:0xf bank_mask:0xf bound_ctrl:0\n\tv_addc_co_u32_e64 v178, %[sc3], v178, 0, %[sc3]\n\tv_mad_u64_u32 v[176:177], %[sc1], v171, %[n0], v[176:177]\n\tv_mad_u64_u32 v[172:173], %[sc2], v171, %[n1], v[172:173]\n\tv_add_co_u32_e64 v172, %[sc3], v172, v177\n\tv_addc_co_u32_e64 v178, %[sc1], v178, 0, %[sc1]\n\tv_mov_b32_dpp v168, v176 quad_perm:[1,2,3,0] row_mask:0xf bank_mask:0xf bound_ctrl:0\n\tv_addc_co_u32_e64 v173, %[sc3], v173, v178, %[sc3]\n\tv_add_co_u32_e64 v173, %[sc0], v173, v168\n\tv_addc_co_u32_e64 v174, %[sc2], 0, 0, %[sc2]\n\tv_addc_co_u32_e64 v174, %[sc3], v174, 0, %[sc3]\n\tv_addc_co_u32_e64 v174, %[sc0], v174, 0, %[sc0]\n\ts_nop 1\n\tv_mov_b32_dpp v179, v174 quad_perm:[3,0,1,2] row_mask:0xf bank_mask:0xf bound_ctrl:0\n\tv_add_co_u32_e64 v172, s[94:95], v172, v179\n\ts_nop 1\n\tv_addc_co_u32_e64 v173, s[94:95], v173, 0, s[94:95]\n\tv_and_b32_e32 v180, v172, v173\n\tv_cmp_eq_u32_e64 %[sp], v180, -1\n\ts_andn2_b64 s[90:91], s[94:95], %[top]\n\ts_andn2_b64 %[sp], %[sp], %[top]\n\ts_or_b64 s[88:89], s[90:91], %[sp]\n\ts_add_u32 s88, s88, s90\n\ts_addc_u32 s89, s89, s91\n\ts_xor_b64 s[90:91], s[88:89], %[sp]\n\tv_addc_co_u32_e64 %[r0], s[94:95], v172, 0, s[90:91]\n\ts_nop 1\n\tv_addc_co_u32_e64 %[r1], s[94:95], v173, 0, s[94:95]"
+                 : [r0] "=&v"(r0), [r1] "=&v"(r1), [sc0] "=&s"(sc0), [sc1] "=&s"(sc1), [sc2] "=&s"(sc2), [sc3] "=&s"(sc3), [sp] "=&s"(sp)
+                 : [a0] "v"(a.v[0]), [a1] "v"(a.v[1]), [a2] "v"(a.v[2]), [a3] "v"(a.v[3]), [a4] "v"(a.v[4]), [a5] "v"(a.v[5]), [a6] "v"(a.v[6]), [a7] "v"(a.v[7]), [b0] "v"(b0), [b1] "v"(b1), [n0] "v"(n0), [n1] "v"(n1), [inv] "s"(inv32), [top] "s"(top)
+                 : "v168", "v169", "v170", "v171", "v172", "v173", "v174", "v175", "v176", "v177", "v178", "v179", "v180", "s88", "s89", "s90", "s91", "s92", "s93", "s94", "s95", "vcc", "scc");
+    out[0] = r0;
+    out[1] = r1;
+}
diff --git a/circom-witnesscalc_amd/csrc/fr_mul_coop4r_lazy_gfx950.inc b/circom-witnesscalc_amd/csrc/fr_mul_coop4r_lazy_gfx950.inc
--- /dev/null
+++ b/circom-witnesscalc_amd/csrc/fr_mul_coop4r_lazy_gfx950.inc
@@ -0,0 +1,12 @@
+{
+    unsigned int r0, r1;
+    unsigned long long sc0, sc1, sc2, sc3, sp, sb, sma, sms;
+    const unsigned int inv32 = 0xefffffffu;
+    const unsigned long long top = 0x8888888888888888ull, lane0 = 0x1111111111111111ull;
+    asm volatile("v_mad_u64_u32 v[172:173], %[sc0], %[a0], %[b0], 0\n\tv_mul_lo_u32 v170, v172, %[inv]\n\tv_mad_u64_u32 v[176:177], %[sc1], %[a0], %[b1], 0\n\tv_mov_b32_e32 v169, 0\n\tv_mov_b32_dpp v171, v170 quad_perm:[0,0,0,0] row_mask:0xf bank_mask:0xf bound_ctrl:0\n\tv_mad_u64_u32 v[172:173], %[sc2], v171, %[n0], v[172:173]\n\tv_mad_u64_u32 v[176:177], %[sc3], v171, %[n1], v[176:177]\n\tv_add_co_u32_e64 v176, %[sc0], v176, v173\n\tv_addc_co_u32_e64 v174, %[sc2], 0, 0, %[sc2]\n\tv_addc_co_u32_e64 v178, %[sc3], 0, 0, %[sc3]\n\tv_addc_co_u32_e64 v177, %[sc0], v177, v174, %[sc0]\n\tv_mad_u64_u32 v[176:177], %[sc1], %[a1], %[b0], v[176:177]\n\tv_mul_lo_u32 v170, v176, %[inv]\n\tv_mov_b32_dpp v168, v172 quad_perm:[1,2,3,0] row_mask:0xf bank_mask:0xf bound_ctrl:0\n\tv_addc_co_u32_e64 v178, %[sc0], v178, 0, %[sc0]\n\tv_mad_u64_u32 v[172:173], %[sc2], %[a1], %[b1], v[168:169]\n\tv_mov_b32_dpp v171, v170 quad_perm:[0,0,0,0] row_mask:0xf bank_mask:0xf bound_ctrl:0\n\tv_addc_co_u32_e64 v178, %[sc1], v178, 0, %[sc1]\n\tv_mad_u64_u32 v[176:177], %[sc3], v171, %[n0], v[176:177]\n\tv_mad_u64_u32 v[172:173], %[sc0], v171, %[n1], v[172:173]\n\tv_add_co_u32_e64 v172, %[sc1], v172, v177\n\tv_addc_co_u32_e64 v178, %[sc3], v178, 0, %[sc3]\n\tv_addc_co_u32_e64 v174, %[sc0], 0, 0, %[sc0]\n\tv_addc_co_u32_e64 v173, %[sc1], v173, v178, %[sc1]\n\tv_mad_u64_u32 v[172:173], %[sc2], %[a2], %[b0], v[172:173]\n\tv_mul_lo_u32 v170, v172, %[inv]\n\tv_mov_b32_dpp v168, v176 quad_perm:[1,2,3,0] row_mask:0xf bank_mask:0xf bound_ctrl:0\n\tv_addc_co_u32_e64 v174, %[sc1], v174, 0, %[sc1]\n\tv_mad_u64_u32 v[176:177], %[sc3], %[a2], %[b1], v[168:169]\n\tv_mov_b32_dpp v171, v170 quad_perm:[0,0,0,0] row_mask:0xf bank_mask:0xf bound_ctrl:0\n\tv_addc_co_u32_e64 v174, %[sc2], v174, 0, %[sc2]\n\tv_mad_u64_u32 v[172:173], %[sc0], v171, %[n0], v[172:173]\n\tv_mad_u64_u32 v[176:177], %[sc1], v171, %[n1], v[176:177]\n\tv_add_co_u32_e64 v176, %[sc2], v176, v173\n\tv_addc_co_u32_e64 v174, %[sc0], v174, 0, %[sc0]\n\tv_addc_co_u32_e64 v178, %[sc1], 0, 0, %[sc1]\n\tv_addc_co_u32_e64 v177, %[sc2], v177, v174, %[sc2]\n\tv_mad_u64_u32 v[176:177], %[sc3], %[a3], %[b0], v[176:177]\n\tv_mul_lo_u32 v170, v176, %[inv]\n\tv_mov_b32_dpp v168, v172 quad_perm:[1,2,3,0] row_mask:0xf bank_mask:0xf bound_ctrl:0\n\tv_addc_co_u32_e64 v178, %[sc2], v178, 0, %[sc2]\n\tv_mad_u64_u32 v[172:173], %[sc0], %[a3], %[b1], v[168:169]\n\tv_mov_b32_dpp v171, v170 quad_perm:[0,0,0,0] row_mask:0xf bank_mask:0xf bound_ctrl:0\n\tv_addc_co_u32_e64 v178, %[sc3], v178, 0, %[sc3]\n\tv_mad_u64_u32 v[176:177], %[sc1], v171, %[n0], v[176:177]\n\tv_mad_u64_u32 v[172:173], %[sc2], v171, %[n1], v[172:173]\n\tv_add_co_u32_e64 v172, %[sc3], v172, v177\n\tv_addc_co_u32_e64 v178, %[sc1], v178, 0, %[sc1]\n\tv_addc_co_u32_e64 v174, %[sc2], 0, 0, %[sc2]\n\tv_addc_co_u32_e64 v173, %[sc3], v173, v178, %[sc3]\n\tv_mad_u64_u32 v[172:173], %[sc0], %[a4], %[b0], v[172:173]\n\tv_mul_lo_u32 v170, v172, %[inv]\n\tv_mov_b32_dpp v168, v176 quad_perm:[1,2,3,0] row_mask:0xf bank_mask:0xf bound_ctrl:0\n\tv_addc_co_u32_e64 v174, %[sc3], v174, 0, %[sc3]\n\tv_mad_u64_u32 v[176:177], %[sc1], %[a4], %[b1], v[168:169]\n\tv_mov_b32_dpp v171, v170 quad_perm:[0,0,0,0] row_mask:0xf bank_mask:0xf bound_ctrl:0\n\tv_addc_co_u32_e64 v174, %[sc0], v174, 0, %[sc0]\n\tv_mad_u64_u32 v[172:173], %[sc2], v171, %[n0], v[172:173]\n\tv_mad_u64_u32 v[176:177], %[sc3], v171, %[n1], v[176:177]\n\tv_add_co_u32_e64 v176, %[sc0], v176, v173\n\tv_addc_co_u32_e64 v174, %[sc2], v174, 0, %[sc2]\n\tv_addc_co_u32_e64 v178, %[sc3], 0, 0, %[sc3]\n\tv_addc_co_u32_e64 v177, %[sc0], v177, v174, %[sc0]\n\tv_mad_u64_u32 v[176:177], %[sc1], %[a5], %[b0], v[176:177]\n\tv_mul_lo_u32 v170, v176, %[inv]\n\tv_mov_b32_dpp v168, v172 quad_perm:[1,2,3,0] row_mask:0xf bank_mask:0xf bound_ctrl:0\n\tv_addc_co_u32_e64 v178, %[sc0], v178, 0, %[sc0]\n\tv_mad_u64_u32 v[172:173], %[sc2], %[a5], %[b1], v[168:169]\n\tv_mov_b32_dpp v171, v170 quad_perm:[0,0,0,0] row_mask:0xf bank_mask:0xf bound_ctrl:0\n\tv_addc_co_u32_e64 v178, %[sc1], v178, 0, %[sc1]\n\tv_mad_u64_u32 v[176:177], %[sc3], v171, %[n0], v[176:177]\n\tv_mad_u64_u32 v[172:173], %[sc0], v171, %[n1], v[172:173]\n\tv_add_co_u32_e64 v172, %[sc1], v172, v177\n\tv_addc_co_u32_e64 v178, %[sc3], v178, 0, %[sc3]\n\tv_addc_co_u32_e64 v174, %[sc0], 0, 0, %[sc0]\n\tv_addc_co_u32_e64 v173, %[sc1], v173, v178, %[sc1]\n\tv_mad_u64_u32 v[172:173], %[sc2], %[a6], %[b0], v[172:173]\n\tv_mul_lo_u32 v170, v172, %[inv]\n\tv_mov_b32_dpp v168, v176 quad_perm:[1,2,3,0] row_mask:0xf bank_mask:0xf bound_ctrl:0\n\tv_addc_co_u32_e64 v174, %[sc1], v174, 0, %[sc1]\n\tv_mad_u64_u32 v[176:177], %[sc3], %[a6], %[b1], v[168:169]\n\tv_mov_b32_dpp v171, v170 quad_perm:[0,0,0,0] row_mask:0xf bank_mask:0xf bound_ctrl:0\n\tv_addc_co_u32_e64 v174, %[sc2], v174, 0, %[sc2]\n\tv_mad_u64_u32 v[172:173], %[sc0], v171, %[n0], v[172:173]\n\tv_mad_u64_u32 v[176:177], %[sc1], v171, %[n1], v[176:177]\n\tv_add_co_u32_e64 v176, %[sc2], v176, v173\n\tv_addc_co_u32_e64 v174, %[sc0], v174, 0, %[sc0]\n\tv_addc_co_u32_e64 v178, %[sc1], 0, 0, %[sc1]\n\tv_addc_co_u32_e64 v177, %[sc2], v177, v174, %[sc2]\n\tv_mad_u64_u32 v[176:177], %[sc3], %[a7], %[b0], v[176:177]\n\tv_mul_lo_u32 v170, v176, %[inv]\n\tv_mov_b32_dpp v168, v172 quad_perm:[1,2,3,0] row_mask:0xf bank_mask:0xf bound_ctrl:0\n\tv_cmp_eq_u32_e64 %[sms], %[sub], 1\n\tv_mov_b32_dpp v171, v170 quad_perm:[0,0,0,0] row_mask:0xf bank_mask:0xf bound_ctrl:0\n\tv_addc_co_u32_e64 v178, %[sc2], v178, 0, %[sc2]\n\tv_mad_u64_u32 v[172:173], %[sc0], %[a7], %[b1], v[168:169]\n\tv_mad_u64_u32 v[176:177], %[sc1], v171, %[n0], v[176:177]\n\tv_mad_u64_u32 v[172:173], %[sc2], v171, %[n1], v[172:173]\n\tv_addc_co_u32_e64 v178, %[sc3], v178, 0, %[sc3]\n\tv_cndmask_b32_e64 v179, 0, -1, %[sms]\n\tv_addc_co_u32_e64 v178, %[sc1], v178, 0, %[sc1]\n\tv_and_b32_e32 v182, v179, %[nn0]\n\tv_addc_co_u32_e64 v174, %[sc2], 0, 0, %[sc2]\n\tv_add_co_u32_e64 v172, %[sc3], v172, v177\n\tv_xor_b32_e32 v180, v179, %[b0]\n\ts_and_b64 s[90:91], %[sms], %[lane0]\n\tv_add_co_u32_e64 v184, %[sc1], %[aq0], v182\n\tv_addc_co_u32_e64 v184, %[sc2], v184, v180, s[90:91]\n\tv_and_b32_e32 v183, v179, %[nn1]\n\tv_mov_b32_dpp v168, v176 quad_perm:[1,2,3,0] row_mask:0xf bank_mask:0xf bound_ctrl:0\n\tv_addc_co_u32_e64 v173, %[sc3], v173, v178, %[sc3]\n\tv_xor_b32_e32 v181, v179, %[b1]\n\tv_addc_co_u32_e64 v185, %[sc1], %[aq1], v183, %[sc1]\n\tv_add_co_u32_e64 v173, %[sc0], v173, v168\n\tv_addc_co_u32_e64 v185, %[sc2], v185, v181, %[sc2]\n\tv_addc_co_u32_e64 v174, %[sc3], v174, 0, %[sc3]\n\tv_cmp_eq_u32_e64 %[sma], %[sub], 0\n\tv_addc_co_u32_e64 v186, %[sc1], 0, 0, %[sc1]\n\tv_addc_co_u32_e64 v174, %[sc0], v174, 0, %[sc0]\n\tv_addc_co_u32_e64 v186, %[sc2], v186, 0, %[sc2]\n\ts_or_b64 %[sma], %[sma], %[sms]\n\tv_cndmask_b32_e64 v174, v174, v186, %[sma]\n\tv_cndmask_b32_e64 v174, v174, 0, %[top]\n\tv_cndmask_b32_e64 v172, v172, v184, %[sma]\n\tv_cndmask_b32_e64 v173, v173, v185, %[sma]\n\tv_mov_b32_dpp v187, v174 quad_perm:[3,0,1,2] row_mask:0xf bank_mask:0xf bound_ctrl:0\n\tv_add_co_u32_e64 v172, s[94:95], v172, v187\n\ts_nop 1\n\tv_addc_co_u32_e64 v173, s[94:95], v173, 0, s[94:95]\n\tv_and_b32_e32 v188, v172, v173\n\tv_cmp_eq_u32_e64 %[sp], v188, -1\n\ts_andn2_b64 s[90:91], s[94:95], %[top]\n\ts_andn2_b64 %[sp], %[sp], %[top]\n\ts_or_b64 s[88:89], s[90:91], %[sp]\n\ts_add_u32 s88, s88, s90\n\ts_addc_u32 s89, s89, s91\n\ts_xor_b64 s[90:91], s[88:89], %[sp]\n\tv_addc_co_u32_e64 v172, s[94:95], v172, 0, s[90:91]\n\ts_nop 1\n\tv_addc_co_u32_e64 v173, s[94:95], v173, 0, s[94:95]\n\tv_sub_co_u32_e64 v189, s[94:95], v172, %[nn0]\n\ts_nop 1\n\tv_subb_co_u32_e64 v190, s[94:95], v173, %[nn1], s[94:95]\n\tv_or_b32_e32 v191, v189, v190\n\ts_or_b64 %[sb], s[94:95], s[94:95]\n\tv_cmp_eq_u32_e64 %[sp], v191, 0\n\ts_andn2_b64 s[90:91], s[94:95], %[top]\n\ts_andn2_b64 %[sp], %[sp], %[top]\n\ts_or_b64 s[88:89], s[90:91], %[sp]\n\ts_add_u32 s88, s88, s90\n\ts_addc_u32 s89, s89, s91\n\ts_xor_b64 s[90:91], s[88:89], %[sp]\n\tv_subb_co_u32_e64 v189, s[94:95], v189, 0, s[90:91]\n\ts_nop 1\n\tv_subb_co_u32_e64 v190, s[94:95], v190, 0, s[94:95]\n\ts_or_b64 s[92:93], s[94:95], %[sb]\n\ts_lshr_b64 s[92:93], s[92:93], 3\n\ts_and_b32 s92, s92, 0x11111111\n\ts_and_b32 s93, s93, 0x11111111\n\ts_mul_i32 s92, s92, 0xf\n\ts_mul_i32 s93, s93, 0xf\n\tv_cndmask_b32_e64 %[r0], v189, v172, s[92:93]\n\tv_cndmask_b32_e64 %[r1], v190, v173, s[92:93]"
+                 : [r0] "=&v"(r0), [r1] "=&v"(r1), [sc0] "=&s"(sc0), [sc1] "=&s"(sc1), [sc2] "=&s"(sc2), [sc3] "=&s"(sc3), [sp] "=&s"(sp), [sb] "=&s"(sb), [sma] "=&s"(sma), [sms] "=&s"(sms)
+                 : [a0] "v"(a.v[0]), [a1] "v"(a.v[1]), [a2] "v"(a.v[2]), [a3] "v"(a.v[3]), [a4] "v"(a.v[4]), [a5] "v"(a.v[5]), [a6] "v"(a.v[6]), [a7] "v"(a.v[7]), [b0] "v"(b0), [b1] "v"(b1), [n0] "v"(n0), [n1] "v"(n1), [nn0] "v"(nn0), [nn1] "v"(nn1), [inv] "s"(inv32), [top] "s"(top), [aq0] "v"(aq0), [aq1] "v"(aq1), [sub] "v"(sub), [lane0] "s"(lane0)
+                 : "v168", "v169", "v170", "v171", "v172", "v173", "v174", "v175", "v176", "v177", "v178", "v179", "v180", "v181", "v182", "v183", "v184", "v185", "v186", "v187", "v188", "v189", "v190", "v191", "s88", "s89", "s90", "s91", "s92", "s93", "s94", "s95", "vcc", "scc");
+    out[0] = r0;
+    out[1] = r1;
+}
diff --git a/circom-witnesscalc_amd/csrc/kernels.hip b/circom-witnesscalc_amd/csrc/kernels.hip
--- a/circom-witnesscalc_amd/csrc/kernels.hip
+++ b/circom-witnesscalc_amd/csrc/kernels.hip
@@ -53,6 +53,17 @@
     return i32x4{(int)(uint32_t)a, (int)((uint32_t)(a >> 32) & 0xffffu), (int)bytes, 0x00020000};
 }
 
+template <bool LAZY>
+__device__ __forceinline__ Fr lazy_canon(const Fr& x) {
+    if constexpr (LAZY) return fr_canon(x);
+    else return x;
+}
+template <bool LAZY>
+__device__ __forceinline__ Fr lazy_mul_wave(const Fr& x, const Fr& y, const Fr& pv) {
+    if constexpr (LAZY) return fr_mul_wave_lazy(x, y);
+    else return fr_mul_wave(x, y, pv);
+}
+
 template <int T, bool PROF, int W, int PACK, int MODE = 0>
 __global__ __launch_bounds__((W > 0 ? (W + 1) * PACK : PACK) * 64) void interp_kernel(const uint32_t* __restrict__ hdr, const uint4* __restrict__ recs,
                                                     const uint32_t* __restrict__ crefs, InterpDims p, WsTable wst,
@@ -60,6 +71,7 @@
                                                     unsigned long long* __restrict__ prof) {
     constexpr int G = 64 / T;
     constexpr bool M2 = MODE == 2 || MODE == 3, WIDE = MODE == 3;
+    constexpr bool LAZY = MODE == 0;
     constexpr uint32_t HI = 16u * T;
     constexpr bool DIVIDER = W > 0;
     constexpr uint32_t NW = (W > 0 ? (uint32_t)W : 1u) * (uint32_t)PACK;
@@ -144,7 +156,15 @@
                 const bool valid = pk_next + j < limit && pk_set < batch, canon = (e.y & REF_CANON) != 0;
                 const Fr v = fr_from_u4(lo, hi);
                 Fr c = v;
-                if (p.pack_mont) {
+                if constexpr (LAZY) {
+                    if (p.pack_mont) {
+                        c = fr_canon(v);
+                        if (wave_any(both(valid, canon))) c = u256_select(canon, fr_mul(v, fr_r2()), c);
+                    } else {
+                        if (wave_any(both(valid, canon))) c = fr_canon(v);
+                        if (wave_any(both(valid, !canon))) c = u256_select(canon, c, fr_from_mont(v));
+                    }
+                } else if (p.pack_mont) {
                     if (wave_any(both(valid, canon))) c = u256_select(canon, fr_mul(v, fr_r2()), v);
                 } else {
                     if (wave_any(both(valid, !canon))) c = u256_select(canon, v, fr_from_mont(v));
@@ -208,6 +228,10 @@
                     const uint4* qa = reinterpret_cast<const uint4*>(mb);
                     const uint4* qb = reinterpret_cast<const uint4*>(mb + 32u * ML);
                     Fr a = fr_from_u4(qa[0], qa[ML]), b = fr_from_u4(qb[0], qb[ML]);
+                    if constexpr (LAZY) {
+                        a = fr_canon(a);
+                        b = fr_canon(b);
+                    }
                     if (!valid) b = fr_zero();
                     const Fr inv = fr_inv(b);
                     const Fr r = u256_select(u256_is_zero(b), fr_zero(), fr_mul(a, inv));
@@ -275,7 +299,7 @@
                      :: "s"(s), "v"(ao), "v"(bo), "s"(rsrc_dma), "s"(dma_soff0), "s"(dma_soff1), "s"(dma_soff2), "s"(dma_soff3) : "memory");
     };
     uint32_t err_bits = 0;
-    Fr pv = fr_p();
+    Fr pv = LAZY ? fr_2p() : fr_p();
 #pragma unroll
     for (int i = 0; i < 8; ++i) asm volatile("" : "+v"(pv.v[i]));
     constexpr bool COOP = (uint32_t)T <= COOP_MAX_T;
@@ -287,6 +311,13 @@
     uint32_t nq0 = cq == 0 ? CWC_P0 : cq == 1 ? CWC_P2 : cq == 2 ? CWC_P4 : CWC_P6;
     uint32_t nq1 = cq == 0 ? CWC_P1 : cq == 1 ? CWC_P3 : cq == 2 ? CWC_P5 : CWC_P7;
     asm volatile("" : "+v"(nq0), "+v"(nq1));
+    [[maybe_unused]] uint32_t nnq0 = 0, nnq1 = 0;
+    if constexpr (LAZY) {
+        const Fr p2 = fr_2p();
+        nnq0 = cq == 0 ? p2.v[0] : cq == 1 ? p2.v[2] : cq == 2 ? p2.v[4] : p2.v[6];
+        nnq1 = cq == 0 ? p2.v[1] : cq == 1 ? p2.v[3] : cq == 2 ? p2.v[5] : p2.v[7];
+        asm volatile("" : "+v"(nnq0), "+v"(nnq1));
+    }
     const uint32_t trash_doff = p.trash_off | t16;
     constexpr int C_PROF = 12;
     unsigned long long pf[C_PROF][2], psec[2][7] = {{0, 0, 0, 0, 0, 0, 0}, {0, 0, 0, 0, 0, 0, 0}};
@@ -347,9 +378,11 @@
                 CWC_STAMP(st3);
                 uint32_t out[2];
                 if (h & (HDR_LIN_ADD | HDR_LIN_SUB)) {
-                    fr_mul_coop4r(a_op, aq.x, aq.y, bq.x, bq.y, nq0, nq1, rec_hi.x & CTRL_SUB_MASK, out);
+                    if constexpr (LAZY) fr_mul_coop4r_lazy(a_op, aq.x, aq.y, bq.x, bq.y, nq0, nq1, nnq0, nnq1, rec_hi.x & CTRL_SUB_MASK, out);
+                    else fr_mul_coop4r(a_op, aq.x, aq.y, bq.x, bq.y, nq0, nq1, rec_hi.x & CTRL_SUB_MASK, out);
                 } else {
-                    fr_mul_coop4(a_op, bq.x, bq.y, nq0, nq1, out);
+                    if constexpr (LAZY) fr_mul_coop4_lazy(a_op, bq.x, bq.y, nq0, nq1, out);
+                    else fr_mul_coop4(a_op, bq.x, bq.y, nq0, nq1, out);
                 }
                 CWC_STAMP(st4);
                 *reinterpret_cast<uint2*>(ldsb + LDS_RING_OFF + (b % RING_BUNDLES) * RING_SLOT_BYTES + coop_ring_off) = make_uint2(out[0], out[1]);
@@ -570,7 +603,8 @@
                     continue;
                 }
             }
-            r = fr_mul_wave(a_op, b_op, pv);
+            if constexpr (LAZY) r = fr_mul_wave_lazy(a_op, b_op);
+            else r = fr_mul_wave(a_op, b_op, pv);
             if ((h & (HDR_LIN_ADD | HDR_LIN_SUB)) == (HDR_LIN_ADD | HDR_LIN_SUB)) {
                 const unsigned long long subm = __ballot(sub == SUB_SUB);
                 r = u256_select(sub <= SUB_SUB, fr_addsub_wave(a_op, b_op, pv, sub == SUB_SUB ? ~0u : 0u, subm, ~subm), r);
@@ -865,7 +899,7 @@
                 const uint32_t idx = crefs[(size_t)cref_row * G + j];
                 ++cref_row;
                 const uint4* q = inputs + ((size_t)set_c * p.n_inputs + idx) * 2;
-                r = fr_mul_wave(fr_from_u4(q[0], q[1]), (h & HDR_OUT_CANON) ? fr_one() : fr_r2(), pv);
+                r = lazy_mul_wave<LAZY>(fr_from_u4(q[0], q[1]), (h & HDR_OUT_CANON) ? fr_one() : fr_r2(), pv);
                 break;
             }
             case C_DIVREQ: {
@@ -898,18 +932,21 @@
                 break;
             }
             case C_DIV: {
-                const Fr inv = fr_inv(b_op);
-                r = u256_select(u256_is_zero(b_op), fr_zero(), fr_mul(a_op, inv));
+                const Fr ac = lazy_canon<LAZY>(a_op), bc = lazy_canon<LAZY>(b_op);
+                const Fr inv = fr_inv(bc);
+                r = u256_select(u256_is_zero(bc), fr_zero(), fr_mul(ac, inv));
                 break;
             }
             case C_CMPZ: {
-                const bool az = u256_is_zero(a_op), cz = u256_is_zero(b_op), eq = u256_eq(a_op, b_op);
+                const Fr ac = lazy_canon<LAZY>(a_op), bc = lazy_canon<LAZY>(b_op);
+                const bool az = u256_is_zero(ac), cz = u256_is_zero(bc), eq = u256_eq(ac, bc);
                 const bool v = either(either(both(sub == SUB_EQ, eq), both(sub == SUB_NEQ, !eq)), either(both(sub == SUB_LAND, !either(az, cz)), both(both(sub != SUB_EQ, both(sub != SUB_NEQ, sub != SUB_LAND)), !both(az, cz))));
                 r = u256_select(v, one_out(), fr_zero());
                 break;
             }
             case C_CMPS: {
-                const Fr x = (h & HDR_A_CANON) ? a_op : fr_from_mont(a_op), y = (h & HDR_B_CANON) ? b_op : fr_from_mont(b_op);
+                const Fr ac = lazy_canon<LAZY>(a_op), bc = lazy_canon<LAZY>(b_op);
+                const Fr x = (h & HDR_A_CANON) ? ac : fr_from_mont(ac), y = (h & HDR_B_CANON) ? bc : fr_from_mont(bc);
                 auto less = [](const Fr& a, const Fr& b) {
                     Fr t;
                     const uint32_t borrow = u256_sub(t, a, b);
@@ -936,7 +973,8 @@
                 break;
             }
             case C_BIT: {
-                const Fr x = (h & HDR_A_CANON) ? a_op : fr_from_mont(a_op);
+                const Fr ac = lazy_canon<LAZY>(a_op), bc = lazy_canon<LAZY>(b_op);
+                const Fr x = (h & HDR_A_CANON) ? ac : fr_from_mont(ac);
                 const uint32_t kx = rec_hi.y >> 20;
                 const bool is_x = sub == SUB_BITX;
                 if (h & HDR_BITX_ALL) {
@@ -944,11 +982,11 @@
                     r = u256_select((e.v[0] & 1u) != 0u, one_out(), fr_zero());
                     break;
                 }
-                const Fr y = (h & HDR_B_CANON) ? b_op : fr_from_mont(b_op);
+                const Fr y = (h & HDR_B_CANON) ? bc : fr_from_mont(bc);
                 auto bit_result = [&](const Fr& d) -> Fr {
                     if (h & HDR_OUT_CANON) return d;
                     const bool small = both(d.v[0] < 2u, (d.v[1] | d.v[2] | d.v[3] | d.v[4] | d.v[5] | d.v[6] | d.v[7]) == 0u);
-                    if (wave_any(!small)) return fr_mul_wave(d, fr_r2(), pv);
+                    if (wave_any(!small)) return lazy_mul_wave<LAZY>(d, fr_r2(), pv);
                     return u256_select(d.v[0] != 0u, fr_one(), fr_zero());
                 };
                 if (h & (HDR_BIT_ALL_SHR | HDR_BIT_ALL_BAND)) {
@@ -998,7 +1036,8 @@
                 break;
             }
             case C_IDIVMOD: {
-                const Fr x = (h & HDR_A_CANON) ? a_op : fr_from_mont(a_op), y = (h & HDR_B_CANON) ? b_op : fr_from_mont(b_op);
+                const Fr ac = lazy_canon<LAZY>(a_op), bc = lazy_canon<LAZY>(b_op);
+                const Fr x = (h & HDR_A_CANON) ? ac : fr_from_mont(ac), y = (h & HDR_B_CANON) ? bc : fr_from_mont(bc);
                 const bool yz = u256_is_zero(y);
                 Fr ys = y;
                 ys.v[0] |= yz ? 1u : 0u;
@@ -1026,14 +1065,14 @@
                     u256_divrem_digits(q, rem, x, ys, dig, ly);
                 }
                 const Fr d = u256_select(yz, fr_zero(), u256_select(sub == SUB_IDIV, q, rem));
-                r = (h & HDR_OUT_CANON) ? d : fr_mul_wave(d, fr_r2(), pv);
+                r = (h & HDR_OUT_CANON) ? d : lazy_mul_wave<LAZY>(d, fr_r2(), pv);
                 break;
             }
             case C_TERN: {
                 const uint32_t cr = crefs[(size_t)cref_row * G + j];
                 ++cref_row;
-                const Fr y = ld(cr + t16);
-                r = u256_select(u256_is_zero(a_op), y, b_op);
+                const Fr y = lazy_canon<LAZY>(ld(cr + t16));
+                r = u256_select(u256_is_zero(lazy_canon<LAZY>(a_op)), y, lazy_canon<LAZY>(b_op));
                 break;
             }
             case C_SYNC: {
@@ -1105,8 +1144,8 @@
 
 template <bool MONT>
 __device__ __forceinline__ Fr pack_form(const Fr& v, bool canon) {
-    if (MONT) return canon ? fr_mul(v, fr_r2()) : v;
-    return canon ? v : fr_from_mont(v);
+    if (MONT) return canon ? fr_mul(v, fr_r2()) : fr_canon(v);
+    return canon ? fr_canon(v) : fr_from_mont(v);
 }
 
 template <bool MONT, int TT>
@@ -1345,13 +1384,11 @@
     if (a.v[0] == 0x1234567u && b.v[3] == 7u) sink[0] = a.v[1];
 }
 __global__ __launch_bounds__(512) void modmul_block_ubench_kernel(uint32_t* sink, uint32_t iters) {
-    Fr a = fr_r2(), b = fr_one(), pv = fr_p();
-#pragma unroll
-    for (int i = 0; i < 8; ++i) asm volatile("" : "+v"(pv.v[i]));
+    Fr a = fr_r2(), b = fr_one();
     a.v[0] ^= threadIdx.x + blockIdx.x * 977u;
     for (uint32_t it = 0; it < iters; ++it) {
-        a = fr_mul_wave(a, b, pv);
-        b = fr_mul_wave(b, a, pv);
+        a = fr_mul_wave_lazy(a, b);
+        b = fr_mul_wave_lazy(b, a);
     }
     if (a.v[0] == 0x1234567u && b.v[3] == 7u) sink[0] = a.v[1];
 }
```

Result: slower. 93390 (-1.0%).
